# omerbt/Splice

Measured on AMD Instinct MI355X. Metric: opt_steps_per_sec, higher is better.
Workload: dtype bf16

## Files before the change

include/splice_hip.h:

```cpp
#ifndef SPLICE_HIP_H
#define SPLICE_HIP_H
#include <stddef.h>
#include <stdint.h>

#ifdef __cplusplus
extern "C" {
#endif

typedef uint16_t splice_bf16;
typedef void* splice_stream_t;

#define SPLICE_OK 0
#define SPLICE_ERR_ARG -1
#define SPLICE_ERR_HIP -2
#define SPLICE_ERR_STATE -3
#define SPLICE_ERR_NOMEM -4

int splice_version(void);
int splice_dev_switches(void);
const char* splice_last_error(void);

typedef struct splice_gemm_epilogue {
    const float* bias;
    const float* resid;
    int ldr, resid_mod;
    float* out_f32;
    int ldo;
    splice_bf16* out_bf;
    int ldbf;
    splice_bf16* out_bf_t;
    int ldt;
    splice_bf16* out_pre;
    int ldp, pre_row_lo;
    const splice_bf16* aux;
    int ldaux;
    float* out_f32_cols;
    int ld_cols, col_lo, col_hi;
    float alpha;
    int ksplit;
    long long slab_stride;
    const splice_bf16* rd_other;
    int ld_rd, rd_rows;
    float* rowdot;
    const float* row_scale;
    const float* col_scale;
    uint8_t* out_f8;
    int ld8;
    uint8_t* out_f8_t;
    int ldt8;
} splice_gemm_epilogue;

enum {
    SPLICE_EPI_BIAS = 1, SPLICE_EPI_RESID = 2, SPLICE_EPI_OUT_F32 = 4, SPLICE_EPI_OUT_BF = 8,
    SPLICE_EPI_OUT_T = 16, SPLICE_EPI_GELU = 32, SPLICE_EPI_GELU_GRAD = 64,
    SPLICE_EPI_COLS_F32 = 128, SPLICE_EPI_ALPHA = 256, SPLICE_EPI_ROWDOT = 512, SPLICE_EPI_SCALE_RC = 1024, SPLICE_EPI_OUT_F8 = 2048,
    SPLICE_EPI_OUT_F8T = 4096
};

int splice_gemm_nt_bf16(unsigned flags, const splice_bf16* A, int lda, const splice_bf16* B, int ldb,
                        int M, int N, int K, const splice_gemm_epilogue* epi, splice_stream_t stream);

int splice_gemm_nt_fp8(unsigned flags, const uint8_t* A, int lda, const uint8_t* B, int ldb, int M, int N, int K,
                       const splice_gemm_epilogue* epi, splice_stream_t stream);
int splice_quantize_rows_fp8(const float* x, int ldx, uint8_t* q, int ldq, float* scale, int rows, int cols, splice_stream_t stream);
int splice_gemm_splitk_slabs(int M, int ksplit);
int splice_gemm_force_tile(int tile);
int splice_attention_variant(int variant);
int splice_attention_qfold(int on);
int splice_attention_bwd_variant(int variant);

int splice_layernorm_fwd(const float* x, const float* gamma, const float* beta, splice_bf16* y,
                         float* mean, float* rstd, int rows, int D, float eps, splice_stream_t stream);
int splice_layernorm_bwd(const float* dy, const float* x, const float* gamma, const float* mean,
                         const float* rstd, const float* g_in, float* g_out, splice_bf16* g_out_bf,
                         int rows, int D, splice_stream_t stream);

int splice_attention_fwd(const splice_bf16* qkv, const splice_bf16* qkvT, int ldt, int B, int T, int Tld,
                         int D, int H, float scale, splice_bf16* out, float* lse, splice_stream_t stream);
int splice_attention_fwd_fp8(const uint8_t* qkv8, const uint8_t* qkvT8, int ldt8, int B, int T, int Tld, int D, int H, float scale,
                             splice_bf16* out, float* lse, splice_stream_t stream);
int splice_attention_bwd(const splice_bf16* qkv, const splice_bf16* qkvT, int ldt, int B, int T, int Tld,
                         int D, int H, float scale, const splice_bf16* out, const float* lse,
                         const splice_bf16* dout, const splice_bf16* doutT, float* delta,
                         splice_bf16* dqkv, splice_stream_t stream);
int splice_attention_probs(const splice_bf16* qkv, int B, int T, int Tld, int D, int H, float scale,
                           const float* lse, float* probs, splice_stream_t stream);

int splice_augment_structure(const float* img, float* out, float* scratch, int H, int W, int flip, int n_ops, const int* order,
                             const float* factors, float blur_sigma, splice_stream_t stream);

size_t splice_keys_selfsim_ws_bytes(int T, int D);
int splice_keys_selfsim_fwd(const float* K, int ldk, int T, int D, float eps, float* S, void* ws,
                            splice_stream_t stream);
int splice_keys_selfsim_bwd(const float* dS, const float* S, int T, int D, float eps, float* dK, int lddk,
                            int accumulate, void* ws, splice_stream_t stream);

int splice_mse(const float* a, int lda, const float* b, int ldb, int rows, int cols, float weight,
               float* loss_accum, float* grad, int ldg, splice_stream_t stream);

int splice_patchify(const float* img, splice_bf16* patches, int B, int H, int W, int p, int Tld,
                    int normalize, splice_stream_t stream);
int splice_unpatchify(const float* dpatches, float* dimg, int B, int H, int W, int p, int Tld,
                      int normalize, splice_stream_t stream);
int splice_cast_f32_bf16(const float* x, splice_bf16* y, size_t n, splice_stream_t stream);
int splice_cast_bf16_f32(const splice_bf16* x, float* y, size_t n, splice_stream_t stream);
int splice_transpose_f32_bf16(const float* x, splice_bf16* y, int rows, int cols, int ldy, splice_stream_t stream);
int splice_resize_bilinear_fwd(const float* in, float* out, int planes, int h, int w, int oh, int ow, splice_stream_t stream);
int splice_resize_bilinear_bwd(const float* dout, float* din, int planes, int h, int w, int oh, int ow, splice_stream_t stream);

int splice_vit_create(int patch, int dim, int depth, int heads, void** out_handle);
void splice_vit_destroy(void* vit);
int splice_vit_set_param(void* vit, const char* name, const float* data, long long numel, splice_stream_t stream);
float splice_vit_qscale(void* vit);
int splice_vit_params_complete(void* vit);
int splice_vit_enable_fp8(void* vit, splice_stream_t stream);
int splice_vit_ctx_create(void* vit, int B, int H, int W, const float* pos_TD, int need_grad,
                          splice_stream_t stream, void** out_ctx);
void splice_vit_ctx_destroy(void* ctx);
int splice_vit_ctx_info(void* ctx, int* T, int* Tld, int* rows);
int splice_vit_ctx_set_top_cls_only(void* ctx, int on);
int splice_vit_ctx_set_fp8(void* ctx, int mode);
int splice_vit_forward(void* ctx, const float* img, int normalize, splice_stream_t stream);
int splice_vit_forward_ex(void* ctx, const float* img, int normalize, int grad_pass_begin, splice_stream_t stream);
int splice_vit_forward_passes(void* ctx, const float* img, int normalize, int grad_pass_begin, int pass_begin, int pass_end,
                              splice_stream_t stream);
int splice_vit_get_tensor(void* ctx, int kind, int layer, void** out_ptr);
int splice_vit_read_tensor(void* ctx, int kind, int layer, void* dst, size_t bytes, splice_stream_t stream);
int splice_vit_backward(void* ctx, int pass_begin, int pass_end, const float* const* d_block,
                        const float* const* d_qkv, const float* const* d_keys, float* d_img,
                        int normalize, splice_stream_t stream);

int splice_gen_create(void** out_handle);
#define SPLICE_GEN_MAX_SCALES 6
typedef struct splice_gen_arch {
    int n_scales, in_channels, out_channels;
    int down[SPLICE_GEN_MAX_SCALES], up[SPLICE_GEN_MAX_SCALES], skip[SPLICE_GEN_MAX_SCALES];
    int filter_down[SPLICE_GEN_MAX_SCALES], filter_up[SPLICE_GEN_MAX_SCALES];
    int filter_skip;
    int reflect;
} splice_gen_arch;
int splice_gen_create_arch(const splice_gen_arch* arch, void** out_handle);
void splice_gen_destroy(void* gen);
long long splice_gen_param_count(void* gen);
int splice_gen_num_tensors(void* gen);
int splice_gen_tensor_info(void* gen, int i, const char** name, long long* offset, long long* numel);
int splice_gen_plan_create(void* gen, int N, int H, int W, int need_grad, void** out_plan);
void splice_gen_plan_destroy(void* plan);
int splice_gen_forward(void* plan, const float* params, const float* x, float* y, splice_stream_t stream);
int splice_gen_forward_borrowed(void* plan, const float* params, const float* x, float* y, splice_stream_t stream);
int splice_gen_backward(void* plan, const float* params, const float* dy, float* grads, int accumulate,
                        splice_stream_t stream);
long long splice_gen_buffer_count(void* gen);
int splice_gen_num_buffers(void* gen);
int splice_gen_buffer_info(void* gen, int i, const char** name, long long* offset, long long* numel);
int splice_gen_running_stats_update(void* const* plans, int n_plans, float* running, long long running_stride, float momentum,
                                    splice_stream_t stream);
int splice_adam_step(float* params, float* grads, float* m, float* v, long long n, float lr, float beta1,
                     float beta2, float eps, int step, int zero_grad, splice_stream_t stream);
int splice_optim_step(int kind, float* params, float* grads, float* m, float* v, long long n, float lr, float hp0, float hp1,
                      float eps, int step, int zero_grad, splice_stream_t stream);
int splice_optim_step_ex(int kind, float* params, float* grads, const float* g2, float* m, float* v, long long n, float lr,
                         const float* lr_dev, float hp0, float hp1, float eps, int step, int zero_grad, splice_stream_t stream);
int splice_optim_step_pairs(int kind, float* params, float* grads, const float* g2, float* m, float* v, int n_pairs, long long stride,
                            long long n, const float* lr_dev, float hp0, float hp1, float eps, int step, int zero_grad,
                            splice_stream_t stream);
int splice_optim_step_ema(int kind, float* params, float* grads, const float* g2, float* m, float* v, float* ema, long long n, float lr,
                          const float* lr_dev, float hp0, float hp1, float eps, int step, int zero_grad, float ema_decay, int ema_start,
                          splice_stream_t stream);

typedef struct splice_optim_ext {
    float weight_decay;
    float momentum;
    float dampening;
    int nesterov;
    int decoupled;
    int amsgrad;
    int centered;
} splice_optim_ext;
int splice_optim_step_ext(int kind, float* params, float* grads, const float* g2, float* m, float* v, float* w, long long n, float lr,
                          const float* lr_dev, float hp0, float hp1, float eps, int step, int zero_grad, const splice_optim_ext* options,
                          splice_stream_t stream);

int splice_prof_begin(int which);
int splice_prof_end(float* total_ms, int* launches);
int splice_prof_end_ex(float* total_ms, int* calls, int* kernels);
int splice_prof_end_detail(float* total_ms, int* calls, int* kernels, char* detail, int detail_len);
int splice_prof_active(void);
int splice_vit_ctx_dims(void* ctx, int* B, int* H, int* W, int* D, int* depth, int* heads, int* patch);
int splice_gen_plan_dims(void* plan, int* N, int* H, int* W, long long* nparams);
int splice_gen_plan_set_arena_stride(void* plan, long long stride);
int splice_gen_plan_set_batch_stats(void* plan, int on);
int splice_gen_plan_set_groups(void* plan, int images_per_group);
int splice_gen_plan_resize(void* plan, int H, int W);

typedef struct splice_step_config {
    int crop_h, crop_w;
    int vit_h, vit_w;
    int ent_h, ent_w;
    int ent_vit_h, ent_vit_w;
    float lambda_global_cls, lambda_global_ssim, lambda_global_identity, lambda_entire_cls, lambda_entire_ssim;
    int entire_every, cls_warmup;
    float lr, beta1, beta2, eps;
    int pairs;
    long long arena_stride;
    int fp8_selfsim;
    int top_cls_only;
    int n_crops;
    int n_crops_b;
} splice_step_config;
#define SPLICE_STEP_MAX_PAIR_CFGS 32
#define SPLICE_STEP_MAX_GROUP_IMAGES 32
int splice_step_create(const splice_step_config* cfg, void* vit_ctx_global, void* vit_ctx_entire, void* gen_plan_a, void* gen_plan_b,
                       void* gen_plan_entire, void** out_handle);
void splice_step_destroy(void* step);
int splice_step_run(void* step, float* params, float* grads, float* m, float* v, const float* A_crop, const float* B_crop,
                    const float* A_entire, int step_idx, float* losses_out, splice_stream_t stream);
int splice_step_output(void* step, int which, float** out_ptr);
int splice_step_graph_stats(void* step, long long* out);
int splice_step_use_graph(void* step, int on);
int splice_step_use_overlap(void* step, int on);
int splice_step_set_crops(void* step, int a_h, int a_w, int b_h, int b_w);
int splice_step_set_mode(void* step, int skip_adam, int accumulate);
int splice_step_set_optimizer(void* step, int kind, float hp0, float hp1, float eps);
int splice_step_set_lr(void* step, float lr);
int splice_step_set_pair_weights(void* step, const float* lambdas);
int splice_step_set_pair_lr(void* step, const float* lr);
int splice_step_set_phases(void* step, int phases, void* leader);
int splice_step_set_running_stats(void* step, float* running, long long stride);

typedef struct splice_stop_state {
    float sum;
    int count;
    int windows;
    float best;
    int bad;
    int stop_step;
} splice_stop_state;
int splice_step_set_stop_rule(void* step, int window, float rel, int patience, int min_steps);
int splice_step_stop_state(void* step, splice_stop_state* out, splice_stream_t stream);
int splice_step_restore(void* step, int next_step_idx, const splice_stop_state* stop, splice_stream_t stream);
int splice_step_set_input_rows(void* step, int pairs_in, const int* rows);
int splice_plateau_update(splice_stop_state* state, const float* losses8, int pairs, int window, float rel, int patience, int min_steps,
                          int step_idx, int counted, splice_stream_t stream);

int splice_step_set_ema(void* step, float* ema, float decay, int start);
int splice_optim_step_pairs_ema(int kind, float* params, float* grads, const float* g2, float* m, float* v, float* ema, int n_pairs,
                                long long stride, long long n, const float* lr_dev, float hp0, float hp1, float eps, const int* step_dev,
                                const splice_stop_state* stop, int zero_grad, float ema_decay, int ema_start, splice_stream_t stream);

#define SPLICE_CLIP_CHUNK 4096
typedef struct splice_clip_state {
    float sumsq;
    float norm;
    float coef;
    int skip;
    int clipped;
    int skipped;
} splice_clip_state;
int splice_grad_norm_pairs(const float* grads, const float* g2, int n_pairs, long long stride, long long n, float max_norm, float* partials,
                           splice_clip_state* state, const splice_stop_state* stop, const int* step_dev, splice_stream_t stream);
int splice_optim_step_pairs_clip(int kind, float* params, float* grads, const float* g2, float* m, float* v, float* ema, int n_pairs,
                                 long long stride, long long n, const float* lr_dev, float hp0, float hp1, float eps, const int* step_dev,
                                 const splice_stop_state* stop, int zero_grad, float ema_decay, int ema_start, const splice_clip_state* clip,
                                 splice_stream_t stream);
int splice_optim_step_clip(int kind, float* params, float* grads, const float* g2, float* m, float* v, float* ema, long long n, float lr,
                           const float* lr_dev, float hp0, float hp1, float eps, int step, int zero_grad, float ema_decay, int ema_start,
                           const splice_clip_state* clip, splice_stream_t stream);
int splice_step_set_grad_clip(void* step, float max_norm, splice_clip_state* state);

typedef struct splice_clip_auto_state {
    float ref[2];
    int count[2];
    float thr;
    int regime;
} splice_clip_auto_state;
int splice_grad_norm_pairs_auto(const float* grads, const float* g2, int n_pairs, long long stride, long long n, float max_norm, float k,
                                float beta, int warmup, int regime, float* partials, splice_clip_state* state,
                                splice_clip_auto_state* auto_state, const splice_stop_state* stop, const int* step_dev,
                                splice_stream_t stream);
int splice_step_set_grad_clip_auto(void* step, float max_norm, float k, float beta, int warmup, splice_clip_state* state,
                                   splice_clip_auto_state* auto_state);

#define SPLICE_STOP_HISTORY 64
typedef struct splice_best_state {
    int best_step;
    int best_window;
} splice_best_state;
int splice_plateau_update_best(splice_stop_state* state, splice_best_state* best, float* means, const float* losses8, int pairs, int window,
                               float rel, int patience, int min_steps, int step_idx, int counted, splice_stream_t stream);
int splice_optim_step_pairs_best(int kind, float* params, float* grads, const float* g2, float* m, float* v, float* ema, int n_pairs,
                                 long long stride, long long n, const float* lr_dev, float hp0, float hp1, float eps, const int* step_dev,
                                 const splice_stop_state* stop, int zero_grad, float ema_decay, int ema_start, const splice_clip_state* clip,
                                 const splice_best_state* best, float* best_params, float* best_ema, splice_stream_t stream);
int splice_optim_step_pairs_ext(int kind, float* params, float* grads, const float* g2, float* m, float* v, float* w, float* ema, int n_pairs,
                                long long stride, long long n, const float* lr_dev, float hp0, float hp1, float eps, int step,
                                const int* step_dev, const splice_stop_state* stop, int zero_grad, float ema_decay, int ema_start,
                                const splice_clip_state* clip, const splice_best_state* best, float* best_params, float* best_ema,
                                const splice_optim_ext* options, splice_stream_t stream);
int splice_step_set_optimizer_ext(void* step, const splice_optim_ext* options, float* w);
int splice_step_set_keep_best(void* step, float* best_params, float* best_ema, splice_best_state* state, float* means);

int splice_step_set_loss_trace(void* step, float* trace, int capacity);

typedef struct splice_lr_state {
    float scale;
    int bad;
    int cuts;
    int last_cut_step;
} splice_lr_state;
int splice_step_set_lr_plateau(void* step, float factor, int patience, float min_scale, splice_lr_state* state, int* cut_steps);
int splice_plateau_update_lr(splice_stop_state* state, splice_lr_state* lr_state, int* cut_steps, const float* losses8, const float* lr_in,
                             int per_pair, float* lr_eff, int pairs, int window, float rel, int patience, int min_steps, float factor,
                             int lr_patience, float min_scale, int step_idx, int counted, splice_stream_t stream);

size_t splice_selfsim_loss_pairs_ws_bytes(int T, int D, int pairs);
int splice_selfsim_loss_pairs(const splice_bf16* k_tgt, const splice_bf16* k_x, int ldk, size_t k_pstride, const splice_bf16* kT_x, int ldt,
                              size_t kT_pstride, int T, int D, int pairs, float lambda, const float* e_scale_tab, int fp8, float eps,
                              float* loss_part, size_t part_pstride, float* dk, int lddk, size_t dk_pstride, void* ws, splice_stream_t stream);
int splice_mse_pairs(const float* a, int lda, size_t a_ps, const float* b, int ldb, size_t b_ps, int rows, int cols, float loss_weight,
                     float grad_weight, float* part, size_t part_ps, float* grad, int ldg, size_t g_ps, int pairs, const float* grad_tab,
                     splice_stream_t stream);
int splice_total_loss_pairs(float* lbase, size_t lstride, int lp, float w_ssim, float w_essim, float w_ecls, float w_cls, float w_id,
                            float* out8, int pairs, int n_a, int n_b, int n_c, int n_e, const float* wtab, int ssim_on, int entire,
                            splice_stream_t stream);
int splice_step_set_image_terms(void* step, float lambda_tv, float lambda_pix);
#define SPLICE_IMAGE_TERMS_CHUNK 4096
int splice_image_terms_value(const float* x, int n_x, int xh, int xw, const float* y, const float* b, int n_y, int yh, int yw, float* lbase,
                             size_t lstride, int lp, splice_stream_t stream);
int splice_image_terms_grad_add(const float* x, const float* b, float* d, int n_img, int h, int w, float lambda, splice_stream_t stream);
int splice_total_loss_pairs_img(float* lbase, size_t lstride, int lp, float w_ssim, float w_essim, float w_ecls, float w_cls, float w_id,
                                float* out8, int pairs, int n_a, int n_b, int n_c, int n_e, const float* wtab, int ssim_on, int entire,
                                float w_tv, float w_pix, splice_stream_t stream);
int splice_total_loss_pairs_trace(float* lbase, size_t lstride, int lp, float w_ssim, float w_essim, float w_ecls, float w_cls, float w_id,
                                  float* out8, int pairs, int n_a, int n_b, int n_c, int n_e, const float* wtab, int ssim_on, int entire,
                                  splice_stop_state* stop, int window, float rel, int patience, int min_steps, const int* dev_t,
                                  float* trace, int capacity, splice_stream_t stream);

int splice_attn_cls_fwd(const splice_bf16* qkv, const splice_bf16* qkvT, int ldt, int B, int T, int Tld, int D, int H, float scale, splice_bf16* out,
                        float* probs, splice_stream_t stream);
int splice_attn_cls_bwd(const splice_bf16* qkv, const splice_bf16* qkvT, int ldt, int B, int T, int Tld, int D, int H, float scale, const float* probs,
                        const float* dout_slabs, int n_slabs, size_t slab_stride, splice_bf16* dqkv, splice_stream_t stream);
int splice_ln_rows_fwd(float* x, size_t xs, const float* gamma, const float* beta, splice_bf16* y, size_t ys, float* mean, float* rstd, size_t ss,
                       int rows, int D, float eps, const float* slabs, int n_slabs, size_t slab_stride, const float* bias, const float* resid, size_t rs,
                       splice_stream_t stream);
int splice_ln_rows_bwd(float* dy, size_t dys, const float* x, size_t xs, const float* gamma, const float* mean, const float* rstd, size_t ss, float* g,
                       splice_bf16* g_bf, int rows, int D, int n_slabs, size_t slab_stride, splice_stream_t stream);
int splice_rows_finish(int mode, const float* slabs, int n_slabs, size_t slab_stride, int rows, int N, const float* bias, const float* resid, size_t rs,
                       float* out_f32, size_t os, splice_bf16* out_bf, splice_bf16* pre_bf, const splice_bf16* aux, size_t ps, int pre_lo,
                       splice_stream_t stream);

typedef struct splice_gen_conv_args {
    const float* in;
    const float* w;
    const float* bias;
    float* out;
    size_t in_nstride, in_cstride, out_nstride, out_cstride, w_jstride, w_cstride, p_nstride;
    int N, Cin, Hi, Wi, Cout, Ho, Wo, ks, stride, pad;
    int reflect, act, transposed, accumulate;
    float* ws;
    size_t ws_floats;
    int p_group, defer_reduce;
} splice_gen_conv_args;
#define SPLICE_GEN_CONV_FORM_INTS 5
int splice_gen_conv(const splice_gen_conv_args* args, int* form_out, splice_stream_t stream);
int splice_gen_conv_pair(const splice_gen_conv_args* a, const splice_gen_conv_args* b, int* forms_out, splice_stream_t stream);
int splice_gen_conv_reflect_dgrad(const splice_gen_conv_args* args, float* pad_scratch, size_t scratch_floats, splice_stream_t stream);

typedef struct splice_gen_wgrad_args {
    const float* x;
    const float* dy;
    float* ws;
    size_t ws_floats;
// ... 71 lines not shown
```

splice_amd/_lib.py:

```python
import ctypes as C
import os

_HERE = os.path.dirname(os.path.abspath(__file__))
LIB_PATH = os.path.join(_HERE, "libsplice_hip.so")

_lib = None


class GemmEpilogue(C.Structure):
    _fields_ = [
        ("bias", C.c_void_p), ("resid", C.c_void_p), ("ldr", C.c_int), ("resid_mod", C.c_int),
        ("out_f32", C.c_void_p), ("ldo", C.c_int),
        ("out_bf", C.c_void_p), ("ldbf", C.c_int),
        ("out_bf_t", C.c_void_p), ("ldt", C.c_int),
        ("out_pre", C.c_void_p), ("ldp", C.c_int), ("pre_row_lo", C.c_int),
        ("aux", C.c_void_p), ("ldaux", C.c_int),
        ("out_f32_cols", C.c_void_p), ("ld_cols", C.c_int), ("col_lo", C.c_int), ("col_hi", C.c_int),
        ("alpha", C.c_float), ("ksplit", C.c_int), ("slab_stride", C.c_longlong),
        ("rd_other", C.c_void_p), ("ld_rd", C.c_int), ("rd_rows", C.c_int), ("rowdot", C.c_void_p),
        ("row_scale", C.c_void_p), ("col_scale", C.c_void_p),
        ("out_f8", C.c_void_p), ("ld8", C.c_int),
        ("out_f8_t", C.c_void_p), ("ldt8", C.c_int),
    ]


class GenArch(C.Structure):
    _fields_ = [("n_scales", C.c_int), ("in_channels", C.c_int), ("out_channels", C.c_int),
                ("down", C.c_int * 6), ("up", C.c_int * 6), ("skip", C.c_int * 6),
                ("filter_down", C.c_int * 6), ("filter_up", C.c_int * 6), ("filter_skip", C.c_int), ("reflect", C.c_int)]


class StepConfig(C.Structure):
    _fields_ = [
        ("crop_h", C.c_int), ("crop_w", C.c_int), ("vit_h", C.c_int), ("vit_w", C.c_int),
        ("ent_h", C.c_int), ("ent_w", C.c_int), ("ent_vit_h", C.c_int), ("ent_vit_w", C.c_int),
        ("lambda_global_cls", C.c_float), ("lambda_global_ssim", C.c_float), ("lambda_global_identity", C.c_float),
        ("lambda_entire_cls", C.c_float), ("lambda_entire_ssim", C.c_float),
        ("entire_every", C.c_int), ("cls_warmup", C.c_int),
        ("lr", C.c_float), ("beta1", C.c_float), ("beta2", C.c_float), ("eps", C.c_float),
        ("pairs", C.c_int), ("arena_stride", C.c_longlong), ("fp8_selfsim", C.c_int), ("top_cls_only", C.c_int), ("n_crops", C.c_int), ("n_crops_b", C.c_int),
    ]


class StopState(C.Structure):
    _fields_ = [("sum", C.c_float), ("count", C.c_int), ("windows", C.c_int), ("best", C.c_float), ("bad", C.c_int), ("stop_step", C.c_int)]


class ClipState(C.Structure):
    _fields_ = [("sumsq", C.c_float), ("norm", C.c_float), ("coef", C.c_float), ("skip", C.c_int), ("clipped", C.c_int), ("skipped", C.c_int)]


class ClipAutoState(C.Structure):
    _fields_ = [("ref", C.c_float * 2), ("count", C.c_int * 2), ("thr", C.c_float), ("regime", C.c_int)]


class BestState(C.Structure):
    _fields_ = [("best_step", C.c_int), ("best_window", C.c_int)]


class LrState(C.Structure):
    _fields_ = [("scale", C.c_float), ("bad", C.c_int), ("cuts", C.c_int), ("last_cut_step", C.c_int)]


class OptimExt(C.Structure):
    _fields_ = [("weight_decay", C.c_float), ("momentum", C.c_float), ("dampening", C.c_float), ("nesterov", C.c_int), ("decoupled", C.c_int),
                ("amsgrad", C.c_int), ("centered", C.c_int)]


def optim_ext(options):
    if isinstance(options, OptimExt):
        return options
    return OptimExt(float(options.get("weight_decay", 0.0)), float(options.get("momentum", 0.0)), float(options.get("dampening", 0.0)),
                    int(bool(options.get("nesterov", False))), int(bool(options.get("decoupled", False))), int(bool(options.get("amsgrad", False))),
                    int(bool(options.get("centered", False))))


class GenConvArgs(C.Structure):
    _fields_ = [("in", C.c_void_p), ("w", C.c_void_p), ("bias", C.c_void_p), ("out", C.c_void_p)] + \
               [(n, C.c_size_t) for n in ("in_nstride", "in_cstride", "out_nstride", "out_cstride", "w_jstride", "w_cstride", "p_nstride")] + \
               [(n, C.c_int) for n in ("N", "Cin", "Hi", "Wi", "Cout", "Ho", "Wo", "ks", "stride", "pad", "reflect", "act", "transposed", "accumulate")] + \
               [("ws", C.c_void_p), ("ws_floats", C.c_size_t), ("p_group", C.c_int), ("defer_reduce", C.c_int)]


class GenWgradArgs(C.Structure):
    _fields_ = [("x", C.c_void_p), ("dy", C.c_void_p), ("ws", C.c_void_p), ("ws_floats", C.c_size_t)] + \
               [(n, C.c_size_t) for n in ("x_nstride", "x_cstride", "dy_nstride", "dy_cstride")] + \
               [(n, C.c_int) for n in ("N", "Cin", "Hi", "Wi", "Cout", "Ho", "Wo", "ks", "stride", "pad", "reflect")]


class GenBnArgs(C.Structure):
    _fields_ = [("y", C.c_void_p), ("out", C.c_void_p), ("y_nstride", C.c_size_t), ("out_nstride", C.c_size_t),
                ("N", C.c_int), ("C", C.c_int), ("HW", C.c_int), ("batch", C.c_int),
                ("gamma", C.c_void_p), ("beta", C.c_void_p), ("eps", C.c_float), ("slope", C.c_float), ("p_nstride", C.c_size_t),
                ("part", C.c_void_p), ("part_floats", C.c_size_t), ("mean", C.c_void_p), ("rstd", C.c_void_p),
                ("up_src", C.c_void_p), ("up_d_src", C.c_void_p), ("up_src_ns", C.c_size_t), ("up_d_src_ns", C.c_size_t),
                ("up_c0", C.c_int), ("up_h", C.c_int), ("up_w", C.c_int), ("up_Ho", C.c_int), ("up_Wo", C.c_int),
                ("slabs", C.c_void_p), ("bias", C.c_void_p), ("ksplit", C.c_int),
                ("da", C.c_void_p), ("dy", C.c_void_p), ("da_nstride", C.c_size_t), ("dy_nstride", C.c_size_t),
                ("dgamma", C.c_void_p), ("dbeta", C.c_void_p), ("accumulate", C.c_int),
                ("da_slabs", C.c_void_p), ("da_ksplit", C.c_int), ("da_accumulate", C.c_int),
                ("pre_y", C.c_void_p), ("pre_y_ns", C.c_size_t), ("pre_slabs", C.c_void_p), ("pre_bias", C.c_void_p),
                ("pre_ksplit", C.c_int), ("pre_C", C.c_int), ("pre_gamma", C.c_void_p), ("pre_beta", C.c_void_p),
                ("pre_mean", C.c_void_p), ("pre_rstd", C.c_void_p), ("pre_slope", C.c_float),
                ("pre_dy", C.c_void_p), ("pre_dgamma", C.c_void_p), ("pre_dbeta", C.c_void_p)]


GEN_CONV_FORM_INTS, GEN_WGRAD_FORM_INTS, GEN_BN_FORM_INTS = 5, 6, 7

STOP_HISTORY = 64

EPI_BIAS, EPI_RESID, EPI_OUT_F32, EPI_OUT_BF, EPI_OUT_T = 1, 2, 4, 8, 16
EPI_GELU, EPI_GELU_GRAD, EPI_COLS_F32, EPI_ALPHA, EPI_ROWDOT, EPI_SCALE_RC, EPI_OUT_F8, EPI_OUT_F8T = 32, 64, 128, 256, 512, 1024, 2048, 4096

_vp, _i, _f, _sz, _u = C.c_void_p, C.c_int, C.c_float, C.c_size_t, C.c_uint

_SIGNATURES = {
    "splice_version": ([], C.c_int),
    "splice_dev_switches": ([], C.c_int),
    "splice_last_error": ([], C.c_char_p),
    "splice_gemm_nt_bf16": ([_u, _vp, _i, _vp, _i, _i, _i, _i, C.POINTER(GemmEpilogue), _vp], _i),
    "splice_gemm_nt_fp8": ([_u, _vp, _i, _vp, _i, _i, _i, _i, C.POINTER(GemmEpilogue), _vp], _i),
    "splice_quantize_rows_fp8": ([_vp, _i, _vp, _i, _vp, _i, _i, _vp], _i),
    "splice_gemm_splitk_slabs": ([_i, _i], _i),
    "splice_gemm_force_tile": ([_i], _i),
    "splice_attention_variant": ([_i], _i),
    "splice_attention_qfold": ([_i], _i),
    "splice_attention_bwd_variant": ([_i], _i),
    "splice_layernorm_fwd": ([_vp, _vp, _vp, _vp, _vp, _vp, _i, _i, _f, _vp], _i),
    "splice_layernorm_bwd": ([_vp, _vp, _vp, _vp, _vp, _vp, _vp, _vp, _i, _i, _vp], _i),
    "splice_attention_fwd": ([_vp, _vp, _i, _i, _i, _i, _i, _i, _f, _vp, _vp, _vp], _i),
    "splice_attention_fwd_fp8": ([_vp, _vp, _i, _i, _i, _i, _i, _i, _f, _vp, _vp, _vp], _i),
    "splice_attention_bwd": ([_vp, _vp, _i, _i, _i, _i, _i, _i, _f, _vp, _vp, _vp, _vp, _vp, _vp, _vp], _i),
    "splice_attention_probs": ([_vp, _i, _i, _i, _i, _i, _f, _vp, _vp, _vp], _i),
    "splice_augment_structure": ([_vp, _vp, _vp, _i, _i, _i, _i, C.POINTER(C.c_int), C.POINTER(C.c_float), _f, _vp], _i),
    "splice_keys_selfsim_ws_bytes": ([_i, _i], _sz),
    "splice_keys_selfsim_fwd": ([_vp, _i, _i, _i, _f, _vp, _vp, _vp], _i),
    "splice_keys_selfsim_bwd": ([_vp, _vp, _i, _i, _f, _vp, _i, _i, _vp, _vp], _i),
    "splice_mse": ([_vp, _i, _vp, _i, _i, _i, _f, _vp, _vp, _i, _vp], _i),
    "splice_selfsim_loss_pairs_ws_bytes": ([_i, _i, _i], _sz),
    "splice_selfsim_loss_pairs": ([_vp, _vp, _i, _sz, _vp, _i, _sz, _i, _i, _i, _f, _vp, _i, _f, _vp, _sz, _vp, _i, _sz, _vp, _vp], _i),
    "splice_mse_pairs": ([_vp, _i, _sz, _vp, _i, _sz, _i, _i, _f, _f, _vp, _sz, _vp, _i, _sz, _i, _vp, _vp], _i),
    "splice_total_loss_pairs": ([_vp, _sz, _i, _f, _f, _f, _f, _f, _vp, _i, _i, _i, _i, _i, _vp, _i, _i, _vp], _i),
    "splice_attn_cls_fwd": ([_vp, _vp, _i, _i, _i, _i, _i, _i, _f, _vp, _vp, _vp], _i),
    "splice_attn_cls_bwd": ([_vp, _vp, _i, _i, _i, _i, _i, _i, _f, _vp, _vp, _i, _sz, _vp, _vp], _i),
    "splice_ln_rows_fwd": ([_vp, _sz, _vp, _vp, _vp, _sz, _vp, _vp, _sz, _i, _i, _f, _vp, _i, _sz, _vp, _vp, _sz, _vp], _i),
    "splice_ln_rows_bwd": ([_vp, _sz, _vp, _sz, _vp, _vp, _vp, _sz, _vp, _vp, _i, _i, _i, _sz, _vp], _i),
    "splice_rows_finish": ([_i, _vp, _i, _sz, _i, _i, _vp, _vp, _sz, _vp, _sz, _vp, _vp, _vp, _sz, _i, _vp], _i),
    "splice_gen_conv": ([C.POINTER(GenConvArgs), C.POINTER(_i), _vp], _i),
    "splice_gen_conv_pair": ([C.POINTER(GenConvArgs), C.POINTER(GenConvArgs), C.POINTER(_i), _vp], _i),
    "splice_gen_conv_reflect_dgrad": ([C.POINTER(GenConvArgs), _vp, _sz, _vp], _i),
    "splice_gen_conv_wgrad_ws_floats": ([_i, _i, _i, _i, _i, _i], _sz),
    "splice_gen_conv_wgrad": ([C.POINTER(GenWgradArgs), _vp, _i, _i, _sz, C.POINTER(_i), _vp], _i),
    "splice_gen_wgrad_reduce": ([_vp, _i, _i, _vp, _i, _i, _sz, _vp], _i),
    "splice_gen_bn_small_instance": ([_i], _i),
    "splice_gen_bn_form": ([_i, _i, _sz, _i, C.POINTER(_i)], _i),
    "splice_gen_bn_part_floats": ([_i, _i], _sz),
    "splice_gen_bn_fwd": ([C.POINTER(GenBnArgs), _vp], _i),
    "splice_gen_bn_bwd": ([C.POINTER(GenBnArgs), _vp], _i),
    "splice_gen_upsample2x_fwd": ([_vp, _sz, _vp, _sz, _i, _i, _i, _i, _i, _i, _vp], _i),
    "splice_gen_upsample2x_bwd": ([_vp, _sz, _vp, _sz, _i, _i, _i, _i, _i, _i, _vp], _i),
    "splice_gen_sigmoid_bias_part_floats": ([_i, _i], _sz),
    "splice_gen_sigmoid_bwd_bias": ([_vp, _vp, _vp, _i, _i, _i, _vp, _sz, _sz, _i, C.POINTER(_i), _vp], _i),
    "splice_patchify": ([_vp, _vp, _i, _i, _i, _i, _i, _i, _vp], _i),
    "splice_unpatchify": ([_vp, _vp, _i, _i, _i, _i, _i, _i, _vp], _i),
    "splice_cast_f32_bf16": ([_vp, _vp, _sz, _vp], _i),
    "splice_cast_bf16_f32": ([_vp, _vp, _sz, _vp], _i),
    "splice_transpose_f32_bf16": ([_vp, _vp, _i, _i, _i, _vp], _i),
    "splice_resize_bilinear_fwd": ([_vp, _vp, _i, _i, _i, _i, _i, _vp], _i),
    "splice_resize_bilinear_bwd": ([_vp, _vp, _i, _i, _i, _i, _i, _vp], _i),
    "splice_vit_create": ([_i, _i, _i, _i, C.POINTER(_vp)], _i),
    "splice_vit_destroy": ([_vp], None),
    "splice_vit_set_param": ([_vp, C.c_char_p, _vp, C.c_longlong, _vp], _i),
    "splice_vit_params_complete": ([_vp], _i),
    "splice_vit_enable_fp8": ([_vp, _vp], _i),
    "splice_vit_ctx_create": ([_vp, _i, _i, _i, _vp, _i, _vp, C.POINTER(_vp)], _i),
    "splice_vit_ctx_destroy": ([_vp], None),
    "splice_vit_ctx_info": ([_vp, C.POINTER(_i), C.POINTER(_i), C.POINTER(_i)], _i),
    "splice_vit_ctx_set_top_cls_only": ([_vp, _i], _i),
    "splice_vit_ctx_set_fp8": ([_vp, _i], _i),
    "splice_vit_forward": ([_vp, _vp, _i, _vp], _i),
    "splice_vit_forward_ex": ([_vp, _vp, _i, _i, _vp], _i),
    "splice_vit_forward_passes": ([_vp, _vp, _i, _i, _i, _i, _vp], _i),
    "splice_vit_get_tensor": ([_vp, _i, _i, C.POINTER(_vp)], _i),
    "splice_vit_qscale": ([_vp], C.c_float),
    "splice_vit_read_tensor": ([_vp, _i, _i, _vp, _sz, _vp], _i),
    "splice_vit_backward": ([_vp, _i, _i, C.POINTER(_vp), C.POINTER(_vp), C.POINTER(_vp), _vp, _i, _vp], _i),
    "splice_gen_create": ([C.POINTER(_vp)], _i),
    "splice_gen_create_arch": ([C.POINTER(GenArch), C.POINTER(_vp)], _i),
    "splice_gen_destroy": ([_vp], None),
    "splice_gen_param_count": ([_vp], C.c_longlong),
    "splice_gen_num_tensors": ([_vp], _i),
    "splice_gen_tensor_info": ([_vp, _i, C.POINTER(C.c_char_p), C.POINTER(C.c_longlong), C.POINTER(C.c_longlong)], _i),
    "splice_gen_plan_create": ([_vp, _i, _i, _i, _i, C.POINTER(_vp)], _i),
    "splice_gen_plan_destroy": ([_vp], None),
    "splice_gen_forward": ([_vp, _vp, _vp, _vp, _vp], _i),
    "splice_gen_forward_borrowed": ([_vp, _vp, _vp, _vp, _vp], _i),
    "splice_gen_backward": ([_vp, _vp, _vp, _vp, _i, _vp], _i),
    "splice_adam_step": ([_vp, _vp, _vp, _vp, C.c_longlong, _f, _f, _f, _f, _i, _i, _vp], _i),
    "splice_optim_step": ([_i, _vp, _vp, _vp, _vp, C.c_longlong, _f, _f, _f, _f, _i, _i, _vp], _i),
    "splice_optim_step_ex": ([_i, _vp, _vp, _vp, _vp, _vp, C.c_longlong, _f, _vp, _f, _f, _f, _i, _i, _vp], _i),
    "splice_optim_step_pairs": ([_i, _vp, _vp, _vp, _vp, _vp, _i, C.c_longlong, C.c_longlong, _vp, _f, _f, _f, _i, _i, _vp], _i),
    "splice_optim_step_ema": ([_i, _vp, _vp, _vp, _vp, _vp, _vp, C.c_longlong, _f, _vp, _f, _f, _f, _i, _i, _f, _i, _vp], _i),
    "splice_optim_step_pairs_ema": ([_i, _vp, _vp, _vp, _vp, _vp, _vp, _i, C.c_longlong, C.c_longlong, _vp, _f, _f, _f, _vp, _vp, _i, _f, _i, _vp], _i),
    "splice_step_set_ema": ([_vp, _vp, _f, _i], _i),
    "splice_grad_norm_pairs": ([_vp, _vp, _i, C.c_longlong, C.c_longlong, _f, _vp, _vp, _vp, _vp, _vp], _i),
    "splice_optim_step_pairs_clip": ([_i, _vp, _vp, _vp, _vp, _vp, _vp, _i, C.c_longlong, C.c_longlong, _vp, _f, _f, _f, _vp, _vp, _i, _f, _i, _vp, _vp], _i),
    "splice_optim_step_clip": ([_i, _vp, _vp, _vp, _vp, _vp, _vp, C.c_longlong, _f, _vp, _f, _f, _f, _i, _i, _f, _i, _vp, _vp], _i),
    "splice_step_set_grad_clip": ([_vp, _f, _vp], _i),
    "splice_grad_norm_pairs_auto": ([_vp, _vp, _i, C.c_longlong, C.c_longlong, _f, _f, _f, _i, _i, _vp, _vp, _vp, _vp, _vp, _vp], _i),
    "splice_step_set_grad_clip_auto": ([_vp, _f, _f, _f, _i, _vp, _vp], _i),
    "splice_plateau_update_best": ([_vp, _vp, _vp, _vp, _i, _i, _f, _i, _i, _i, _i, _vp], _i),
    "splice_optim_step_pairs_best": ([_i, _vp, _vp, _vp, _vp, _vp, _vp, _i, C.c_longlong, C.c_longlong, _vp, _f, _f, _f, _vp, _vp, _i, _f, _i, _vp, _vp, _vp, _vp, _vp], _i),
    "splice_step_set_keep_best": ([_vp, _vp, _vp, _vp, _vp], _i),
    "splice_step_set_loss_trace": ([_vp, _vp, _i], _i),
    "splice_total_loss_pairs_trace": ([_vp, _sz, _i, _f, _f, _f, _f, _f, _vp, _i, _i, _i, _i, _i, _vp, _i, _i, _vp, _i, _f, _i, _i, _vp, _vp, _i, _vp], _i),
    "splice_step_set_lr_plateau": ([_vp, _f, _i, _f, _vp, _vp], _i),
    "splice_plateau_update_lr": ([_vp, _vp, _vp, _vp, _vp, _i, _vp, _i, _i, _f, _i, _i, _f, _i, _f, _i, _i, _vp], _i),
    "splice_optim_step_ext": ([_i, _vp, _vp, _vp, _vp, _vp, _vp, C.c_longlong, _f, _vp, _f, _f, _f, _i, _i, C.POINTER(OptimExt), _vp], _i),
    "splice_optim_step_pairs_ext": ([_i, _vp, _vp, _vp, _vp, _vp, _vp, _vp, _i, C.c_longlong, C.c_longlong, _vp, _f, _f, _f, _i, _vp, _vp, _i, _f, _i, _vp, _vp,
                                     _vp, _vp, C.POINTER(OptimExt), _vp], _i),
    "splice_step_set_optimizer_ext": ([_vp, C.POINTER(OptimExt), _vp], _i),
    "splice_step_set_image_terms": ([_vp, _f, _f], _i),
    "splice_image_terms_value": ([_vp, _i, _i, _i, _vp, _vp, _i, _i, _i, _vp, _sz, _i, _vp], _i),
    "splice_image_terms_grad_add": ([_vp, _vp, _vp, _i, _i, _i, _f, _vp], _i),
    "splice_total_loss_pairs_img": ([_vp, _sz, _i, _f, _f, _f, _f, _f, _vp, _i, _i, _i, _i, _i, _vp, _i, _i, _f, _f, _vp], _i),
    "splice_prof_begin": ([_i], _i),
    "splice_prof_end": ([C.POINTER(_f), C.POINTER(_i)], _i),
    "splice_prof_end_ex": ([C.POINTER(_f), C.POINTER(_i), C.POINTER(_i)], _i),
    "splice_prof_end_detail": ([C.POINTER(_f), C.POINTER(_i), C.POINTER(_i), C.c_char_p, _i], _i),
    "splice_prof_active": ([], _i),
    "splice_step_use_graph": ([_vp, _i], _i),
    "splice_step_graph_stats": ([_vp, C.POINTER(C.c_longlong)], _i),
    "splice_step_use_overlap": ([_vp, _i], _i),
    "splice_vit_ctx_dims": ([_vp] + [C.POINTER(_i)] * 7, _i),
    "splice_gen_plan_dims": ([_vp, C.POINTER(_i), C.POINTER(_i), C.POINTER(_i), C.POINTER(C.c_longlong)], _i),
    "splice_step_create": ([C.POINTER(StepConfig), _vp, _vp, _vp, _vp, _vp, C.POINTER(_vp)], _i),
    "splice_step_destroy": ([_vp], None),
    "splice_step_run": ([_vp, _vp, _vp, _vp, _vp, _vp, _vp, _vp, _i, _vp, _vp], _i),
    "splice_step_output": ([_vp, _i, C.POINTER(_vp)], _i),
    "splice_step_set_crops": ([_vp, _i, _i, _i, _i], _i),
    "splice_step_set_running_stats": ([_vp, _vp, C.c_longlong], _i),
    "splice_step_set_mode": ([_vp, _i, _i], _i),
    "splice_step_set_optimizer": ([_vp, _i, _f, _f, _f], _i),
    "splice_step_set_lr": ([_vp, _f], _i),
    "splice_step_set_pair_weights": ([_vp, _vp], _i),
    "splice_step_set_pair_lr": ([_vp, _vp], _i),
    "splice_step_set_phases": ([_vp, _i, _vp], _i),
    "splice_step_set_stop_rule": ([_vp, _i, _f, _i, _i], _i),
    "splice_step_stop_state": ([_vp, _vp, _vp], _i),
    "splice_plateau_update": ([_vp, _vp, _i, _i, _f, _i, _i, _i, _i, _vp], _i),
    "splice_step_restore": ([_vp, _i, _vp, _vp], _i),
    "splice_step_set_input_rows": ([_vp, _i, _vp], _i),
    "splice_gen_buffer_count": ([_vp], C.c_longlong),
    "splice_gen_num_buffers": ([_vp], _i),
    "splice_gen_buffer_info": ([_vp, _i, C.POINTER(C.c_char_p), C.POINTER(C.c_longlong), C.POINTER(C.c_longlong)], _i),
    "splice_gen_running_stats_update": ([C.POINTER(_vp), _i, _vp, C.c_longlong, _f, _vp], _i),
    "splice_gen_plan_resize": ([_vp, _i, _i], _i),
    "splice_gen_plan_set_arena_stride": ([_vp, C.c_longlong], _i),
    "splice_gen_plan_set_batch_stats": ([_vp, _i], _i),
    "splice_gen_plan_set_groups": ([_vp, _i], _i),
}


def exported_symbols():
    return sorted(_SIGNATURES)


def register(name, argtypes, restype):
    _SIGNATURES[name] = (argtypes, restype)


def lib():
    global _lib
    if _lib is None:
        if not os.path.exists(LIB_PATH):
            raise RuntimeError(
                f"{LIB_PATH} not found: the HIP extension is not built "
                "(run __graft_entry__.build() or `make -C splice_amd/csrc`). There is no CPU fallback.")
        _lib = C.CDLL(LIB_PATH)
        for name, (argtypes, restype) in _SIGNATURES.items():
            fn = getattr(_lib, name)
            fn.argtypes = argtypes
            fn.restype = restype
    return _lib


def check(rc, what=""):
    if rc != 0:
        msg = lib().splice_last_error().decode(errors="replace")
        raise RuntimeError(f"libsplice_hip {what} failed (rc={rc}): {msg}")


def ptr(t):
    return None if t is None else C.c_void_p(t.data_ptr())


def current_stream():
    import torch
    return C.c_void_p(torch.cuda.current_stream().cuda_stream)
```

splice_amd/csrc/attention.hip:

```cpp
#include "kernels.h"
#include <cstdlib>


#define NEG_BIG (-1.0e30f)
#define LOG2E 1.4426950408889634f
#define LN2 0.6931471805599453f

__device__ __forceinline__ u32x4 ld16v(const bf16_t* p) { return *reinterpret_cast<const u32x4*>(p); }
__device__ __forceinline__ u32x4 pack8v(const f32x4& a, const f32x4& b) {
    return u32x4{pack2bf(a[0], a[1]), pack2bf(a[2], a[3]), pack2bf(b[0], b[1]), pack2bf(b[2], b[3])};
}
__device__ __forceinline__ void st4bf(bf16_t* p, const f32x4& v, float s) {
    *reinterpret_cast<uint2*>(p) = uint2{pack2bf(v[0] * s, v[1] * s), pack2bf(v[2] * s, v[3] * s)};
}
__device__ __forceinline__ float group4_max(float v) {
    v = fmaxf(v, __shfl_xor(v, 16, 64));
    return fmaxf(v, __shfl_xor(v, 32, 64));
}
__device__ __forceinline__ float group4_sum(float v) {
    v += __shfl_xor(v, 16, 64);
    return v + __shfl_xor(v, 32, 64);
}

typedef __attribute__((address_space(3))) void lds_void;
// ... 320 lines not shown
        }
        __syncthreads();
        if (grp == 1) return;
#pragma unroll
        for (int qb = 0; qb < QB; ++qb) {
            const float* e = ex + ((dma.wave * QB + qb) * 18) * 64 + lane;
            const float m1 = e[0], l1 = e[64];
            const float mn = fmaxf(m[qb], m1);
            const float a0 = __builtin_amdgcn_exp2f(m[qb] - mn), a1 = __builtin_amdgcn_exp2f(m1 - mn);
            m[qb] = mn;
            l[qb] = merge2(l[qb], a0, l1, a1);
#pragma unroll
            for (int nd = 0; nd < 4; ++nd)
#pragma unroll
                for (int r = 0; r < 4; ++r) o[qb][nd][r] = merge2(o[qb][nd][r], a0, e[(2 + nd * 4 + r) * 64], a1);
        }
    }
    if (!active) return;
#pragma unroll
    for (int qb = 0; qb < QB; ++qb) {
        const float lt = group4_sum(l[qb]);
        const int q = qidx[qb];
        if (q < a.Tld) {
            const float inv = 1.0f / lt;
            bf16_t* op = a.out + ((size_t)b * a.Tld + q) * a.D + h * 64 + g * 4;
#pragma unroll
            for (int nd = 0; nd < 4; ++nd) st4bf(op + nd * 16, o[qb][nd], inv);
            if (g == 0) a.lse[((size_t)b * a.H + h) * a.Tld + q] = m[qb] + __builtin_amdgcn_logf(lt);
        }
    }
}

template <int NSUB, bool MASK>
__device__ __forceinline__ void attn_bwd_q_tile(const bf16_t* Ks, const bf16_t* Vs, const FragAddr& fa,
                                                const u32x4 (&qf)[2], const u32x4 (&dof)[2], float lse_q, float del_q, f32x4 (&dq)[4],
                                                float c2, int kt, int T, int g) {
    f32x4 s[NSUB * 2], dp[NSUB * 2];
#pragma unroll
    for (int nb = 0; nb < NSUB * 2; ++nb) {
        const int off = (nb >> 1) * 2048 + (nb & 1) * 256;
        s[nb] = mfma16(lds16(Ks + fa.tok[0] + off), qf[0], f32x4{0.f, 0.f, 0.f, 0.f});
        dp[nb] = mfma16(lds16(Vs + fa.tok[0] + off), dof[0], f32x4{0.f, 0.f, 0.f, 0.f});
        s[nb] = mfma16(lds16(Ks + fa.tok[1] + off), qf[1], s[nb]);
        dp[nb] = mfma16(lds16(Vs + fa.tok[1] + off), dof[1], dp[nb]);
    }
#pragma unroll
    for (int nb = 0; nb < NSUB * 2; ++nb)
#pragma unroll
        for (int r = 0; r < 4; ++r) {
            float p = __builtin_amdgcn_exp2f(__builtin_fmaf(s[nb][r], c2, -lse_q));
            if (MASK) p = kt + (nb >> 1) * 32 + g * 8 + (nb & 1) * 4 + r < T ? p : 0.f;
            dp[nb][r] = p * (dp[nb][r] - del_q);
        }
#pragma unroll
    for (int sub = 0; sub < NSUB; ++sub) {
        const u32x4 dsb = pack8v(dp[sub * 2], dp[sub * 2 + 1]);
#pragma unroll
        for (int nd = 0; nd < 4; ++nd) dq[nd] = mfma16(lds_tr16(Ks, fa.tr[nd] + sub * 2048), dsb, dq[nd]);
    }
}

__device__ __forceinline__ float dot8bf(const u32x4& x, const u32x4& y) {
    float acc = 0.f;
#pragma unroll
    for (int j = 0; j < 4; ++j) {
        acc = __builtin_fmaf(__uint_as_float(x[j] << 16), __uint_as_float(y[j] << 16), acc);
        acc = __builtin_fmaf(__uint_as_float(x[j] & 0xFFFF0000u), __uint_as_float(y[j] & 0xFFFF0000u), acc);
    }
    return acc;
}

constexpr int Q_STAGE = 2 * 4096;
template <int NW = 4>
__device__ __forceinline__ void attn_bwd_q_body(const AttnArgs& a, int xb, int h, int b, bf16_t* smem ) {
    const int lane = threadIdx.x & 63;
    const int g = lane >> 4, c = lane & 15;
    const int ld = 3 * a.D;
    const TileDmaT<NW> dma;
    const FragAddr fa(g, c);
    const int qbase = xb * (16 * NW) + dma.wave * 16;
    const bool active = qbase < a.Tld;
    const int q = qbase + c;
    const int qc = q < a.Tld ? q : a.Tld - 1;
    const bf16_t* qkv_b = a.qkv + (size_t)b * a.Tld * ld;
    u32x4 qf[2], dof[2];
    {
        const bf16_t* pq = qkv_b + (size_t)qc * ld + h * 64 + g * 8;
        const bf16_t* pd = a.dout + ((size_t)b * a.Tld + qc) * a.D + h * 64 + g * 8;
        qf[0] = ld16v(pq); qf[1] = ld16v(pq + 32);
        dof[0] = ld16v(pd); dof[1] = ld16v(pd + 32);
    }
    const float lse_q = a.lse[((size_t)b * a.H + h) * a.Tld + qc];
    const float del_q = a.delta[((size_t)b * a.H + h) * a.Tld + qc];
    const bf16_t* krow = qkv_b + a.D + h * 64;
    const bf16_t* vrow = qkv_b + 2 * a.D + h * 64;
    const uint32_t koff = dma.token_off(ld);
    auto issue = [&](int kt, bf16_t* st) {
        if (kt + 64 <= a.Tld) {
            dma.fast_tile(krow + (size_t)kt * ld, koff, ld, st);
            dma.fast_tile(vrow + (size_t)kt * ld, koff, ld, st + 4096);
        } else {
            dma.token_tile(krow, ld, kt, a.Tld - 1, st);
            dma.token_tile(vrow, ld, kt, a.Tld - 1, st + 4096);
        }
    };
    issue(0, smem);
    f32x4 dq[4];
#pragma unroll
    for (int nd = 0; nd < 4; ++nd) dq[nd] = f32x4{0.f, 0.f, 0.f, 0.f};
    const float c2 = a.scale * LOG2E;
    const int nfull = a.T / 64;
    for (int it = 0; it < nfull; ++it) {
        dma_wait_barrier();
        const int kn = it * 64 + 64;
        if (kn < a.Tld) issue(kn, smem + ((it + 1) & 1) * Q_STAGE);
        if (active) {
            const bf16_t* cur = smem + (it & 1) * Q_STAGE;
            attn_bwd_q_tile<2, false>(cur, cur + 4096, fa, qf, dof, lse_q, del_q, dq, c2, it * 64, a.T, g);
        }
    }
    if (nfull * 64 < a.T) {
        dma_wait_barrier();
        const int kt = nfull * 64;
        if (active) {
            const bf16_t* cur = smem + (nfull & 1) * Q_STAGE;
            if (kt + 32 < a.T) attn_bwd_q_tile<2, true>(cur, cur + 4096, fa, qf, dof, lse_q, del_q, dq, c2, kt, a.T, g);
            else attn_bwd_q_tile<1, true>(cur, cur + 4096, fa, qf, dof, lse_q, del_q, dq, c2, kt, a.T, g);
        }
    }
    if (active && q < a.Tld) {
        bf16_t* p = a.dqkv + ((size_t)b * a.Tld + q) * ld + h * 64 + g * 4;
#pragma unroll
        for (int nd = 0; nd < 4; ++nd) st4bf(p + nd * 16, dq[nd], a.scale);
    }
}

#define KV_STAGE (2 * 4096 + 256)
template <int NSUB>
__device__ __forceinline__ void attn_bwd_kv_tile(const bf16_t* st, const FragAddr& fa, const u32x4 (&kf)[2], const u32x4 (&vf)[2],
                                                 f32x4 (&dk)[4], f32x4 (&dv)[4], float c2, int g) {
    const bf16_t *Qs = st, *Ds = st + 4096;
    const float* Ls = reinterpret_cast<const float*>(st + 8192);
    const float* Es = Ls + 64;
    f32x4 s[NSUB * 2], dp[NSUB * 2];
#pragma unroll
    for (int nb = 0; nb < NSUB * 2; ++nb) {
        const int off = (nb >> 1) * 2048 + (nb & 1) * 256;
        s[nb] = mfma16(lds16(Qs + fa.tok[0] + off), kf[0], f32x4{0.f, 0.f, 0.f, 0.f});
        dp[nb] = mfma16(lds16(Ds + fa.tok[0] + off), vf[0], f32x4{0.f, 0.f, 0.f, 0.f});
        s[nb] = mfma16(lds16(Qs + fa.tok[1] + off), kf[1], s[nb]);
        dp[nb] = mfma16(lds16(Ds + fa.tok[1] + off), vf[1], dp[nb]);
    }
#pragma unroll
    for (int nb = 0; nb < NSUB * 2; ++nb) {
        const f32x4 ls = *reinterpret_cast<const f32x4*>(Ls + (nb >> 1) * 32 + g * 8 + (nb & 1) * 4);
        const f32x4 de = *reinterpret_cast<const f32x4*>(Es + (nb >> 1) * 32 + g * 8 + (nb & 1) * 4);
#pragma unroll
        for (int r = 0; r < 4; ++r) {
            const float p = __builtin_amdgcn_exp2f(__builtin_fmaf(s[nb][r], c2, -ls[r]));
            s[nb][r] = p;
            dp[nb][r] = p * (dp[nb][r] - de[r]);
        }
    }
#pragma unroll
    for (int sub = 0; sub < NSUB; ++sub) {
        const u32x4 pb = pack8v(s[sub * 2], s[sub * 2 + 1]), dsb = pack8v(dp[sub * 2], dp[sub * 2 + 1]);
#pragma unroll
        for (int nd = 0; nd < 4; ++nd) {
            dv[nd] = mfma16(lds_tr16(Ds, fa.tr[nd] + sub * 2048), pb, dv[nd]);
            dk[nd] = mfma16(lds_tr16(Qs, fa.tr[nd] + sub * 2048), dsb, dk[nd]);
        }
    }
}

template <int NW = 4>
__device__ __forceinline__ void attn_bwd_kv_body(const AttnArgs& a, int xb, int h, int b, bf16_t* smem ) {
    const int lane = threadIdx.x & 63;
    const int g = lane >> 4, c = lane & 15;
    const int ld = 3 * a.D;
    const TileDmaT<NW> dma;
    const FragAddr fa(g, c);
    const int kbase = xb * (16 * NW) + dma.wave * 16;
    const bool active = kbase < a.Tld;
    const int key = kbase + c;
    const int keyc = key < a.Tld ? key : a.Tld - 1;
    const bf16_t* qkv_b = a.qkv + (size_t)b * a.Tld * ld;
    u32x4 kf[2], vf[2];
    {
        const bf16_t* pk = qkv_b + (size_t)keyc * ld + a.D + h * 64 + g * 8;
        const bf16_t* pv = qkv_b + (size_t)keyc * ld + 2 * a.D + h * 64 + g * 8;
        kf[0] = ld16v(pk); kf[1] = ld16v(pk + 32);
        vf[0] = ld16v(pv); vf[1] = ld16v(pv + 32);
    }
    const bf16_t* qrow = qkv_b + h * 64;
    const bf16_t* dorow = a.dout + (size_t)b * a.Tld * a.D + h * 64;
    const float* lse = a.lse + ((size_t)b * a.H + h) * a.Tld;
    const float* dl = a.delta + ((size_t)b * a.H + h) * a.Tld;
    const uint32_t qoff = dma.token_off(ld), dooff = dma.token_off(a.D);
    auto issue = [&](int qt, bf16_t* st) {
        if (qt + 64 <= a.Tld) {
            dma.fast_tile(qrow + (size_t)qt * ld, qoff, ld, st);
            dma.fast_tile(dorow + (size_t)qt * a.D, dooff, a.D, st + 4096);
        } else {
            dma.token_tile(qrow, ld, qt, a.Tld - 1, st);
            dma.token_tile(dorow, a.D, qt, a.Tld - 1, st + 4096);
        }
        if (dma.wave < 2) {
            const int qq = qt + lane < a.Tld ? qt + lane : a.Tld - 1;
            const float* src = (dma.wave == 0 ? lse : dl) + qq;
            __builtin_amdgcn_global_load_lds((glb_void*)src, (lds_void*)(st + 8192 + dma.wave * 128), 4, 0, 0);
        }
    };
    issue(0, smem);
    f32x4 dk[4], dv[4];
#pragma unroll
    for (int nd = 0; nd < 4; ++nd) { dk[nd] = f32x4{0.f, 0.f, 0.f, 0.f}; dv[nd] = f32x4{0.f, 0.f, 0.f, 0.f}; }
    const float c2 = a.scale * LOG2E;
    const int nfull = a.Tld / 64;
    for (int it = 0; it < nfull; ++it) {
        dma_wait_barrier();
        const int qn = it * 64 + 64;
        if (qn < a.Tld) issue(qn, smem + ((it + 1) & 1) * KV_STAGE);
        if (active) attn_bwd_kv_tile<2>(smem + (it & 1) * KV_STAGE, fa, kf, vf, dk, dv, c2, g);
    }
    if (nfull * 64 < a.Tld) {
        dma_wait_barrier();
        if (active) attn_bwd_kv_tile<1>(smem + (nfull & 1) * KV_STAGE, fa, kf, vf, dk, dv, c2, g);
    }
    if (active && key < a.Tld) {
        const float sk = key < a.T ? a.scale : 0.f, sv = key < a.T ? 1.0f : 0.f;
        bf16_t* pk = a.dqkv + ((size_t)b * a.Tld + key) * ld + a.D + h * 64 + g * 4;
        bf16_t* pv = a.dqkv + ((size_t)b * a.Tld + key) * ld + 2 * a.D + h * 64 + g * 4;
#pragma unroll
        for (int nd = 0; nd < 4; ++nd) {
            st4bf(pk + nd * 16, dk[nd], sk);
            st4bf(pv + nd * 16, dv[nd], sv);
        }
    }
}

__global__ __launch_bounds__(256) void attn_bwd_kernel(AttnArgs a, int nx) {
    __shared__ __attribute__((aligned(16))) bf16_t smem[2 * KV_STAGE];
    const int n = nx * a.H * a.B;
    const int lid = xcd_remap(blockIdx.x, 2 * n);
    const int pair = lid >> 1;
    const int xb = pair % nx, bh = pair / nx;
    const int h = bh % a.H, b = bh / a.H;
    if (lid & 1) attn_bwd_kv_body(a, xb, h, b, smem);
    else attn_bwd_q_body(a, xb, h, b, smem);
}

template <int NW>
__global__ __launch_bounds__(64 * NW) void attn_bwd_q_kernel(AttnArgs a, int nx) {
    __shared__ __attribute__((aligned(16))) bf16_t smem[2 * Q_STAGE];
    int xb, h, b;
    attn_block_coords(nx, a.H, a.B, xb, h, b);
    attn_bwd_q_body<NW>(a, xb, h, b, smem);
}
template <int NW>
__global__ __launch_bounds__(64 * NW) void attn_bwd_kv_kernel(AttnArgs a, int nx) {
    __shared__ __attribute__((aligned(16))) bf16_t smem[2 * KV_STAGE];
    int xb, h, b;
    attn_block_coords(nx, a.H, a.B, xb, h, b);
    attn_bwd_kv_body<NW>(a, xb, h, b, smem);
}

__global__ void attn_delta_kernel(AttnArgs a) {
    const int idx = blockIdx.x * blockDim.x + threadIdx.x;
    if (idx >= a.B * a.Tld * a.H) return;
    const int h = idx % a.H, row = idx / a.H;
    const int b = row / a.Tld, q = row % a.Tld;
    const bf16_t* po = a.out + (size_t)row * a.D + h * 64;
    const bf16_t* pd = a.dout + (size_t)row * a.D + h * 64;
    float acc = 0.f;
#pragma unroll
    for (int i = 0; i < 8; ++i) acc += dot8bf(ld16v(po + i * 8), ld16v(pd + i * 8));
    a.delta[((size_t)b * a.H + h) * a.Tld + q] = acc;
}

__global__ void attn_probs_kernel(AttnArgs a, float* probs) {
    const int q = blockIdx.x, h = blockIdx.y, b = blockIdx.z;
    const int ld = 3 * a.D;
    const bf16_t* qkv_b = a.qkv + (size_t)b * a.Tld * ld;
    const bf16_t* pq = qkv_b + (size_t)q * ld + h * 64;
    const float lse = a.lse[((size_t)b * a.H + h) * a.Tld + q];
    float qv[64];
#pragma unroll
    for (int d = 0; d < 64; ++d) qv[d] = bf2f(pq[d]);
    float* out = probs + (((size_t)b * a.H + h) * a.T + q) * a.T;
    for (int key = threadIdx.x; key < a.T; key += blockDim.x) {
        const bf16_t* pk = qkv_b + (size_t)key * ld + a.D + h * 64;
        float s = 0.f;
#pragma unroll
        for (int d = 0; d < 64; ++d) s += qv[d] * bf2f(pk[d]);
        out[key] = __builtin_amdgcn_exp2f(s * a.scale * LOG2E - lse);
    }
}

static int g_attn_variant = 0;
void attn_set_variant(int v) { g_attn_variant = v; }
static int g_attn_qfold = 0;
void attn_set_qfold(int on) { g_attn_qfold = on; }
int attn_qfold_hook() { return g_attn_qfold; }

struct AttrOnce {
    bool done[64] = {};
    void set(const void* fn, int bytes) {
        int dev = 0;
        (void)hipGetDevice(&dev);
        if (dev < 0 || dev >= 64) { (void)hipFuncSetAttribute(fn, hipFuncAttributeMaxDynamicSharedMemorySize, bytes); return; }
        if (!done[dev]) { (void)hipFuncSetAttribute(fn, hipFuncAttributeMaxDynamicSharedMemorySize, bytes); done[dev] = true; }
    }
};

template <int NW, bool FOLD>
static void attn_fwd_x32_go(const AttnArgs* a, hipStream_t s) {
    static AttrOnce attr;
    attr.set((const void*)attn_fwd_x32_kernel<NW, FOLD>, X32<NW>::LDS_BYTES);
    const int nx = cdiv(a->Tld, 32 * NW);
    SPLICE_LAUNCH((attn_fwd_x32_kernel<NW, FOLD>), dim3(nx * a->H * a->B), dim3(64 * NW), X32<NW>::LDS_BYTES, s, *a, nx);
}

int attn_fwd_launch(const AttnArgs* a, hipStream_t s) {
    if (a->Tld % 32 || a->D % 64 || a->D / 64 != a->H) return SPLICE_ERR_ARG;
    if (!a->qkv8) {
        const int nwv = g_attn_variant / 10 == 4 ? g_attn_variant % 10 : 4;
        if (a->qfold) { if (nwv == 2) attn_fwd_x32_go<2, true>(a, s); else if (nwv == 8) attn_fwd_x32_go<8, true>(a, s); else attn_fwd_x32_go<4, true>(a, s); }
        else { if (nwv == 2) attn_fwd_x32_go<2, false>(a, s); else if (nwv == 8) attn_fwd_x32_go<8, false>(a, s); else attn_fwd_x32_go<4, false>(a, s); }
        return SPLICE_OK;
    }
    if (!a->qkvT8 || a->ldt8 % 16 || a->D % 16) return SPLICE_ERR_ARG;
    const long tasks = (long)a->B * a->H * cdiv(a->Tld, 16);
    const int qb = g_attn_variant ? g_attn_variant % 10 : (tasks > 60000 ? 2 : 1);
    const long wgs = (long)cdiv(a->Tld, 64 * qb) * a->H * a->B;
    const int ks = g_attn_variant ? (g_attn_variant / 10 == 1 ? 2 : 1) : ((wgs > 512 && a->T <= 2048) ? 1 : 2);
    const int nx = cdiv(a->Tld, 64 * qb);
    const dim3 grid(nx * a->H * a->B);
    if (ks == 2) {
        if (qb == 2) SPLICE_LAUNCH((attn_fwd8_kernel<2, 2>), grid, dim3(512), 0, s, *a, nx);
        else SPLICE_LAUNCH((attn_fwd8_kernel<1, 2>), grid, dim3(512), 0, s, *a, nx);
    } else {
        if (qb == 2) SPLICE_LAUNCH((attn_fwd8_kernel<2, 1>), grid, dim3(256), 0, s, *a, nx);
        else SPLICE_LAUNCH((attn_fwd8_kernel<1, 1>), grid, dim3(256), 0, s, *a, nx);
    }
    return SPLICE_OK;
}

static int g_attn_bwd_variant = 0;
void attn_set_bwd_variant(int v) { g_attn_bwd_variant = v; }
static const int kAttnBwdMergeMaxX32 = 1400;
static const int kAttnBwdMergeMax16 = 768;

int attn_bwd_launch(const AttnArgs* a, hipStream_t s) {
    if (a->Tld % 32 || a->D % 64 || a->D / 64 != a->H) return SPLICE_ERR_ARG;
    const int nx = cdiv(a->Tld, 64);
    if (!a->delta_ready) SPLICE_LAUNCH(attn_delta_kernel, dim3(cdiv(a->B * a->Tld * a->H, 256)), dim3(256), 0, s, *a);
    if (a->qfold && g_attn_bwd_variant != 1) {
        static AttrOnce at_m, at_q, at_kv, at_m2;
        at_m.set((const void*)attn_bwd_x32_kernel<4>, BX_KV_LDS);
        at_q.set((const void*)attn_bwd_q_x32_kernel<4>, BX_Q_LDS);
        at_kv.set((const void*)attn_bwd_kv_x32_kernel<4>, BX_KV_LDS);
        if (g_attn_bwd_variant == 4) {
            at_m2.set((const void*)attn_bwd_x32_kernel<2>, BX_KV_LDS);
            const int nx2 = cdiv(a->Tld, 64), n2 = nx2 * a->H * a->B;
            SPLICE_LAUNCH((attn_bwd_x32_kernel<2>), dim3(2 * n2), dim3(128), BX_KV_LDS, s, *a, nx2);
            return SPLICE_OK;
        }
        const int nx4 = cdiv(a->Tld, 128), n4 = nx4 * a->H * a->B;
        if (g_attn_bwd_variant == 3 || (g_attn_bwd_variant != 2 && 2 * n4 > kAttnBwdMergeMaxX32)) {
            SPLICE_LAUNCH((attn_bwd_q_x32_kernel<4>), dim3(n4), dim3(256), BX_Q_LDS, s, *a, nx4);
            SPLICE_LAUNCH((attn_bwd_kv_x32_kernel<4>), dim3(n4), dim3(256), BX_KV_LDS, s, *a, nx4);
        } else SPLICE_LAUNCH((attn_bwd_x32_kernel<4>), dim3(2 * n4), dim3(256), BX_KV_LDS, s, *a, nx4);
        return SPLICE_OK;
    }
    const int n = nx * a->H * a->B;
    if (2 * n <= kAttnBwdMergeMax16) {
        SPLICE_LAUNCH(attn_bwd_kernel, dim3(2 * n), dim3(256), 0, s, *a, nx);
    } else {
        SPLICE_LAUNCH(attn_bwd_q_kernel<4>, dim3(n), dim3(256), 0, s, *a, nx);
        SPLICE_LAUNCH(attn_bwd_kv_kernel<4>, dim3(n), dim3(256), 0, s, *a, nx);
    }
    return SPLICE_OK;
}

int attn_probs_launch(const AttnArgs* a, float* probs, hipStream_t s) {
    dim3 grid(a->T, a->H, a->B);
    SPLICE_LAUNCH(attn_probs_kernel, grid, dim3(128), 0, s, *a, probs);
    return SPLICE_OK;
}
```

splice_amd/csrc/attn_bwd_x32.h:

```cpp
#pragma once

constexpr int BX_SLOTS = 4;
constexpr int BX_Q_LDS = BX_SLOTS * 2 * 8192;
constexpr int BX_KV_LDS = BX_SLOTS * (2 * 8192 + 512);

__device__ __forceinline__ int bx_swz(int row) { return (((row >> 1) & 1) << 2) | (((row >> 3) & 1) << 1) | ((row >> 2) & 1); }

struct BxFrag {
    int rowa[4];
    int tra[2][2];
    __device__ __forceinline__ BxFrag(int lane) {
        const int q32 = lane & 31, hi = lane >> 5;
#pragma unroll
        for (int ks = 0; ks < 4; ++ks) rowa[ks] = q32 * 64 + (((2 * ks + hi) ^ bx_swz(q32)) << 3);
        const int m = lane & 15, dg = (lane >> 4) & 1;
#pragma unroll
        for (int db = 0; db < 2; ++db)
#pragma unroll
            for (int sec = 0; sec < 2; ++sec) {
                const int row = 8 * sec + 4 * hi + (m >> 2);
                tra[db][sec] = row * 64 + (((4 * db + 2 * dg + ((m >> 1) & 1)) ^ bx_swz(row)) << 3) + (m & 1) * 4;
            }
    }
};
__device__ __forceinline__ u32x4 bx_tr(const bf16_t* tile, const BxFrag& f, int db, int off) {
    typedef __attribute__((address_space(3))) tr_v4s lds_v4s;
    const tr_v4s lo = __builtin_amdgcn_ds_read_tr16_b64_v4i16((lds_v4s*)(tile + f.tra[db][0] + off));
    const tr_v4s hh = __builtin_amdgcn_ds_read_tr16_b64_v4i16((lds_v4s*)(tile + f.tra[db][1] + off));
    const uint2 x = __builtin_bit_cast(uint2, lo), y = __builtin_bit_cast(uint2, hh);
    return u32x4{x.x, x.y, y.x, y.y};
}
__device__ __forceinline__ void bx_mfma_seed(f32x16_t& d, const u32x4& a, const u32x4& b, const f32x16_t& c) {
    asm volatile("v_mfma_f32_32x32x16_bf16 %0, %1, %2, %3" : "=&v"(d) : "v"(a), "v"(b), "v"(c));
}
#define BX_SB __builtin_amdgcn_sched_barrier(0)

template <int NW>
struct BxDma {
    static constexpr int PIECES = 8 / NW;
    int wave, lr, chunk;
    uint32_t off[PIECES];
    __device__ __forceinline__ BxDma(int lane, int wave_, int ld, int coldelta) : wave(wave_) {
        lr = lane >> 3;
        const int pos = lane & 7;
        chunk = pos ^ ((((lr >> 1) & 1) << 2) | ((wave & 1) << 1) | ((lr >> 2) & 1));
#pragma unroll
        for (int i = 0; i < PIECES; ++i) off[i] = (uint32_t)((((wave + NW * i) * 8 + lr) * ld + chunk * 8 + coldelta) * 2);
    }
    __device__ __forceinline__ void tile(const bf16_t* base, int ld, int coldelta, int row0, int rows_total, uint32_t dst) const {
        if (row0 + 64 <= rows_total) {
            const bf16_t* tb = base + (size_t)row0 * ld;
#pragma unroll
            for (int i = 0; i < PIECES; ++i) pp_dma16(dst + i * (NW * 1024), off[i], tb);
        } else {
#pragma unroll
            for (int i = 0; i < PIECES; ++i) {
                int t = row0 + (wave + NW * i) * 8 + lr;
                t = t < rows_total ? t : rows_total - 1;
                pp_dma16(dst + i * (NW * 1024), (uint32_t)((t * ld + chunk * 8 + coldelta) * 2), base);
            }
        }
    }
};

template <int NW, bool FOLD>
__device__ __forceinline__ void attn_bwd_q_x32_body(const AttnArgs& a, int xb, int h, int b, bf16_t* bx_smem ) {
    constexpr int NL = 2 * (8 / NW);
    const int lane = threadIdx.x & 63, q32 = lane & 31, hi = lane >> 5;
    const int wave = __builtin_amdgcn_readfirstlane(threadIdx.x >> 6);
    const int ld = 3 * a.D;
    const int qbase = xb * (32 * NW) + wave * 32;
    const bool active = qbase < a.Tld;
    const bf16_t* pbase = a.qkv + (size_t)b * a.Tld * ld + h * 64;
    const int nt = (a.T + 63) / 64;
    const BxDma<NW> dk_(lane, wave, ld, a.D), dv_(lane, wave, ld, 2 * a.D);
    const BxFrag fr(lane);
    const uint32_t lds0 = (uint32_t)(size_t)(__attribute__((address_space(3))) bf16_t*)bx_smem + (uint32_t)wave * 1024u;
    auto issue = [&](int tile, int slot) __attribute__((always_inline)) {
        const uint32_t dst = __builtin_amdgcn_readfirstlane(lds0 + (uint32_t)slot * 16384u);
        dk_.tile(pbase, ld, a.D, tile * 64, a.Tld, dst);
        dv_.tile(pbase, ld, 2 * a.D, tile * 64, a.Tld, dst + 8192u);
    };
    issue(0, 0);
    if (nt > 1) issue(1, 1);
    if (nt > 2) issue(2, 2);

    const int qidx = qbase + q32;
    const int qc = qidx < a.Tld ? qidx : a.Tld - 1;
    u32x4 qf[4], dof[4];
    {
        const bf16_t* pq = pbase + (size_t)qc * ld + hi * 8;
        const bf16_t* pd = a.dout + ((size_t)b * a.Tld + qc) * a.D + h * 64 + hi * 8;
#pragma unroll
        for (int ks = 0; ks < 4; ++ks) { qf[ks] = ld16v(pq + ks * 16); dof[ks] = ld16v(pd + ks * 16); }
    }
    const float lse_q = a.lse[((size_t)b * a.H + h) * a.Tld + qc];
    const float del_q = a.delta[((size_t)b * a.H + h) * a.Tld + qc];
    const float c2 = a.scale * LOG2E;
    f32x16_t negl, negd, dq[2], s[2], dp[2];
    const f32x16_t zero16 = {0.f, 0.f, 0.f, 0.f, 0.f, 0.f, 0.f, 0.f, 0.f, 0.f, 0.f, 0.f, 0.f, 0.f, 0.f, 0.f};
#pragma unroll
    for (int r = 0; r < 16; ++r) { negl[r] = -lse_q; negd[r] = -del_q; dq[0][r] = dq[1][r] = 0.f; s[0][r] = s[1][r] = dp[0][r] = dp[1][r] = 0.f; }
    u32x4 kf[4], vf[4];
    auto read_rows = [&](const bf16_t* K, int blk) __attribute__((always_inline)) {
#pragma unroll
        for (int ks = 0; ks < 4; ++ks) { kf[ks] = lds16(K + fr.rowa[ks] + blk * 2048); vf[ks] = lds16(K + 4096 + fr.rowa[ks] + blk * 2048); }
    };
    auto sdp = [&](f32x16_t& sx, f32x16_t& dx, int ks) __attribute__((always_inline)) {
        if (ks == 0) {
            if (FOLD) bx_mfma_seed(sx, kf[0], qf[0], negl); else sx = mfma32(kf[0], qf[0], zero16);
            bx_mfma_seed(dx, vf[0], dof[0], negd);
        } else { sx = mfma32(kf[ks], qf[ks], sx); dx = mfma32(vf[ks], dof[ks], dx); }
    };
    pp_wait_dma<0>();
    asm volatile("" : "+v"(qf[0]), "+v"(qf[1]), "+v"(qf[2]), "+v"(qf[3]), "+v"(dof[0]), "+v"(dof[1]), "+v"(dof[2]), "+v"(dof[3]));
    pp_barrier();
    if (active) {
        read_rows(bx_smem, 0);
#pragma unroll
        for (int ks = 0; ks < 4; ++ks) sdp(s[0], dp[0], ks);
        read_rows(bx_smem, 1);
    }
    int slot = 0;
    auto body = [&](auto TAILC, int t) __attribute__((always_inline)) {
        constexpr bool TAIL = decltype(TAILC)::value;
        const int s1 = (slot + 1) & 3, s3 = (slot + 3) & 3;
        if (!TAIL || t + 2 < nt) pp_wait_dma<NL>(); else pp_wait_dma<0>();
        asm volatile("s_waitcnt lgkmcnt(0)" ::: "memory");
        pp_barrier();
        if (!TAIL || t + 3 < nt) issue(t + 3, s3);
        if (active) {
            const bf16_t* Kt = bx_smem + slot * 8192;
            const bf16_t* Kn = bx_smem + s1 * 8192;
#pragma unroll
            for (int blk = 0; blk < 2; ++blk) {
                f32x16_t& sc = s[blk];
                f32x16_t& dc = dp[blk];
                f32x16_t& sn = s[blk ^ 1];
                f32x16_t& dn = dp[blk ^ 1];
                if (TAIL && t * 64 + 64 > a.T) {
#pragma unroll
                    for (int r = 0; r < 16; ++r) sc[r] = t * 64 + 32 * blk + 8 * (r >> 2) + 4 * hi + (r & 3) < a.T ? sc[r] : NEG_BIG;
                }
                float g[16];
                u32x4 dsb[2], ktf[2][2];
                auto va = [&](int r0, int n) __attribute__((always_inline)) {
#pragma unroll
                    for (int r = r0; r < r0 + n; ++r) {
                        const float p = FOLD ? __builtin_amdgcn_exp2f(sc[r]) : __builtin_amdgcn_exp2f(__builtin_fmaf(sc[r], c2, -lse_q));
                        g[r] = p * dc[r];
                    }
                    asm volatile("" : "+v"(g[r0]), "+v"(g[r0 + n - 1]));
                };
                auto cv = [&](int kk) __attribute__((always_inline)) {
                    const float* pp = &g[kk * 8];
                    dsb[kk] = u32x4{pack2bf(pp[0], pp[1]), pack2bf(pp[2], pp[3]), pack2bf(pp[4], pp[5]), pack2bf(pp[6], pp[7])};
                    pp_opaque(dsb[kk]);
                };
                auto rt = [&](int kk, int db) __attribute__((always_inline)) {
                    ktf[kk][db] = bx_tr(Kt, fr, db, blk * 2048 + kk * 1024);
                };
                BX_SB;
                sdp(sn, dn, 0); BX_SB; va(0, 4); rt(0, 0); BX_SB;
                sdp(sn, dn, 1); BX_SB; va(4, 4); cv(0); rt(0, 1); BX_SB;
                sdp(sn, dn, 2); BX_SB; va(8, 4); rt(1, 0); BX_SB;
                sdp(sn, dn, 3); BX_SB; va(12, 4); cv(1); rt(1, 1); BX_SB;
                const bf16_t* Kr = blk == 0 ? Kn : Kn;
#pragma unroll
                for (int kk = 0; kk < 2; ++kk)
#pragma unroll
                    for (int db = 0; db < 2; ++db) {
                        dq[db] = mfma32(ktf[kk][db], dsb[kk], dq[db]);
                        BX_SB;
                        const int ks = kk * 2 + db;
                        kf[ks] = lds16(Kr + fr.rowa[ks] + blk * 2048); vf[ks] = lds16(Kr + 4096 + fr.rowa[ks] + blk * 2048);
                        BX_SB;
                    }
            }
        }
        slot = s1;
    };
    {
        std::false_type MAIN; std::true_type TAILT;
        int t = 0;
        for (; t + 4 < nt; ++t) body(MAIN, t);
        for (; t < nt; ++t) body(TAILT, t);
    }
    if (!active || qidx >= a.Tld) return;
    bf16_t* op = a.dqkv + ((size_t)b * a.Tld + qidx) * ld + h * 64 + hi * 4;
#pragma unroll
    for (int db = 0; db < 2; ++db)
#pragma unroll
        for (int j = 0; j < 4; ++j)
            *reinterpret_cast<uint2*>(op + db * 32 + j * 8) = uint2{pack2bf(dq[db][4 * j] * a.scale, dq[db][4 * j + 1] * a.scale),
                                                                    pack2bf(dq[db][4 * j + 2] * a.scale, dq[db][4 * j + 3] * a.scale)};
}

template <int NW>
__device__ __forceinline__ void attn_bwd_kv_x32_body(const AttnArgs& a, int xb, int h, int b, bf16_t* bx_smem ) {
    constexpr int SLOT = 2 * 4096 + 256;
    static_assert(NW >= 2, "waves 0 and 1 move the lse / delta rows");
    const int lane = threadIdx.x & 63, k32 = lane & 31, hi = lane >> 5;
    const int wave = __builtin_amdgcn_readfirstlane(threadIdx.x >> 6);
    const int ld = 3 * a.D;
    const int kbase = xb * (32 * NW) + wave * 32;
    const bool active = kbase < a.Tld;
    const bf16_t* pbase = a.qkv + (size_t)b * a.Tld * ld + h * 64;
    const bf16_t* dobase = a.dout + (size_t)b * a.Tld * a.D + h * 64;
    const float* lse = a.lse + ((size_t)b * a.H + h) * a.Tld;
    const float* dl = a.delta + ((size_t)b * a.H + h) * a.Tld;
    const int nblk = a.Tld / 32, nt = (nblk + 1) / 2;
    const BxDma<NW> dq_(lane, wave, ld, 0), dd_(lane, wave, a.D, 0);
    const BxFrag fr(lane);
    const uint32_t ldsb = (uint32_t)(size_t)(__attribute__((address_space(3))) bf16_t*)bx_smem;
    const uint32_t lds0 = ldsb + (uint32_t)wave * 1024u;
    auto issue = [&](int tile, int slot) __attribute__((always_inline)) {
        const uint32_t dst = __builtin_amdgcn_readfirstlane(lds0 + (uint32_t)slot * (SLOT * 2));
        dq_.tile(pbase, ld, 0, tile * 64, a.Tld, dst);
        dd_.tile(dobase, a.D, 0, tile * 64, a.Tld, dst + 8192u);
        if (wave < 2) {
            const int r = tile * 64 + lane;
            const uint32_t voff = (uint32_t)((r < a.Tld ? r : a.Tld - 1) * 4);
            const uint32_t d2 = __builtin_amdgcn_readfirstlane(ldsb + (uint32_t)slot * (SLOT * 2) + 16384u + (uint32_t)wave * 256u);
            const float* src = wave == 0 ? lse : dl;
            asm volatile("s_mov_b32 m0, %0\n\ts_nop 0\n\tglobal_load_lds_dword %1, %2" ::"s"(d2), "v"(voff), "s"(src) : "memory");
        }
    };
    issue(0, 0);
    if (nt > 1) issue(1, 1);
    if (nt > 2) issue(2, 2);

    const int kidx = kbase + k32;
    const int kc = kidx < a.Tld ? kidx : a.Tld - 1;
    u32x4 kn[4], vn[4];
    {
        const bf16_t* pk = pbase + (size_t)kc * ld + a.D + hi * 8;
        const bf16_t* pv = pbase + (size_t)kc * ld + 2 * a.D + hi * 8;
#pragma unroll
        for (int ks = 0; ks < 4; ++ks) {
            kn[ks] = ld16v(pk + ks * 16); vn[ks] = ld16v(pv + ks * 16);
#pragma unroll
            for (int j = 0; j < 4; ++j) { kn[ks][j] ^= 0x80008000u; vn[ks][j] ^= 0x80008000u; }
        }
    }
    f32x16_t dkn[2], dv[2];
#pragma unroll
    for (int r = 0; r < 16; ++r) { dkn[0][r] = dkn[1][r] = dv[0][r] = dv[1][r] = 0.f; }
    u32x4 qr[4], dr[4];
    f32x16_t sx, dx;
    auto seeds = [&](const bf16_t* st, int blk) __attribute__((always_inline)) {
        const float* Ls = reinterpret_cast<const float*>(st + 8192);
#pragma unroll
        for (int j = 0; j < 4; ++j) {
            const f32x4 lv = *reinterpret_cast<const f32x4*>(Ls + 32 * blk + 8 * j + 4 * hi);
            const f32x4 ev = *reinterpret_cast<const f32x4*>(Ls + 64 + 32 * blk + 8 * j + 4 * hi);
#pragma unroll
            for (int i = 0; i < 4; ++i) { sx[4 * j + i] = lv[i]; dx[4 * j + i] = ev[i]; }
        }
    };
    auto rows = [&](const bf16_t* st, int blk) __attribute__((always_inline)) {
#pragma unroll
        for (int ks = 0; ks < 4; ++ks) { qr[ks] = lds16(st + fr.rowa[ks] + blk * 2048); dr[ks] = lds16(st + 4096 + fr.rowa[ks] + blk * 2048); }
    };
    pp_wait_dma<0>();
    asm volatile("" : "+v"(kn[0]), "+v"(kn[1]), "+v"(kn[2]), "+v"(kn[3]), "+v"(vn[0]), "+v"(vn[1]), "+v"(vn[2]), "+v"(vn[3]));
    pp_barrier();
    if (active) { rows(bx_smem, 0); seeds(bx_smem, 0); }
    int slot = 0;
    auto body = [&](auto TAILC, int t) __attribute__((always_inline)) {
        constexpr bool TAIL = decltype(TAILC)::value;
        const int s1 = (slot + 1) & 3, s3 = (slot + 3) & 3;
        if (!TAIL || t + 2 < nt) { if (wave < 2) pp_wait_dma<2 * (8 / NW) + 1>(); else pp_wait_dma<2 * (8 / NW)>(); } else pp_wait_dma<0>();
        asm volatile("s_waitcnt lgkmcnt(0)" ::: "memory");
        pp_barrier();
        if (!TAIL || t + 3 < nt) issue(t + 3, s3);
        if (active) {
            const bf16_t* st = bx_smem + slot * SLOT;
            const bf16_t* sn = bx_smem + s1 * SLOT;
#pragma unroll
            for (int blk = 0; blk < 2; ++blk) {
                if (TAIL && 2 * t + blk >= nblk) break;
                u32x4 dot[2][2], qt[2][2], pb[2], gb[2];
                float p[16], g[16];
#pragma unroll
                for (int ks = 0; ks < 4; ++ks) {
                    sx = mfma32(qr[ks], kn[ks], sx);
                    BX_SB;
                    {
                        if (ks < 2) { dot[ks][0] = bx_tr(st + 4096, fr, 0, blk * 2048 + ks * 1024); dot[ks][1] = bx_tr(st + 4096, fr, 1, blk * 2048 + ks * 1024); }
                        else { qt[ks - 2][0] = bx_tr(st, fr, 0, blk * 2048 + (ks - 2) * 1024); qt[ks - 2][1] = bx_tr(st, fr, 1, blk * 2048 + (ks - 2) * 1024); }
                    }
                    BX_SB;
                }
#pragma unroll
                for (int ks = 0; ks < 4; ++ks) {
                    dx = mfma32(dr[ks], vn[ks], dx);
                    BX_SB;
                    {
#pragma unroll
                        for (int r = 4 * ks; r < 4 * ks + 4; ++r) p[r] = __builtin_amdgcn_exp2f(-sx[r]);
                        if (ks & 1) {
                            const float* pp = &p[(ks >> 1) * 8];
                            pb[ks >> 1] = u32x4{pack2bf(pp[0], pp[1]), pack2bf(pp[2], pp[3]), pack2bf(pp[4], pp[5]), pack2bf(pp[6], pp[7])};
                            pp_opaque(pb[ks >> 1]);
                        } else asm volatile("" : "+v"(p[4 * ks]), "+v"(p[4 * ks + 3]));
                    }
                    BX_SB;
                }
#pragma unroll
                for (int i4 = 0; i4 < 4; ++i4) {
                    const int kk = i4 >> 1, db = i4 & 1;
                    dv[db] = mfma32(dot[kk][db], pb[kk], dv[db]);
                    BX_SB;
                    {
#pragma unroll
                        for (int r = 4 * i4; r < 4 * i4 + 4; ++r) g[r] = p[r] * dx[r];
                        if (i4 & 1) {
                            const float* pp = &g[(i4 >> 1) * 8];
                            gb[i4 >> 1] = u32x4{pack2bf(pp[0], pp[1]), pack2bf(pp[2], pp[3]), pack2bf(pp[4], pp[5]), pack2bf(pp[6], pp[7])};
                            pp_opaque(gb[i4 >> 1]);
                        } else asm volatile("" : "+v"(g[4 * i4]), "+v"(g[4 * i4 + 3]));
                    }
                    BX_SB;
                }
                const bf16_t* nx_st = blk == 0 ? st : sn;
                const int nx_blk = blk ^ 1;
#pragma unroll
                for (int i4 = 0; i4 < 4; ++i4) {
                    const int kk = i4 >> 1, db = i4 & 1;
                    dkn[db] = mfma32(qt[kk][db], gb[kk], dkn[db]);
                    BX_SB;
                    {
                        const float* Ls = reinterpret_cast<const float*>(nx_st + 8192);
                        qr[i4] = lds16(nx_st + fr.rowa[i4] + nx_blk * 2048);
                        dr[i4] = lds16(nx_st + 4096 + fr.rowa[i4] + nx_blk * 2048);
                        const f32x4 lv = *reinterpret_cast<const f32x4*>(Ls + 32 * nx_blk + 8 * i4 + 4 * hi);
                        const f32x4 ev = *reinterpret_cast<const f32x4*>(Ls + 64 + 32 * nx_blk + 8 * i4 + 4 * hi);
#pragma unroll
                        for (int i = 0; i < 4; ++i) { sx[4 * i4 + i] = lv[i]; dx[4 * i4 + i] = ev[i]; }
                    }
                    BX_SB;
                }
            }
        }
        slot = s1;
    };
    {
        std::false_type MAIN; std::true_type TAILT;
        int t = 0;
        for (; t + 4 < nt; ++t) body(MAIN, t);
        for (; t < nt; ++t) body(TAILT, t);
    }
    if (!active || kidx >= a.Tld) return;
    const float sk = kidx < a.T ? -a.scale : 0.f, sv = kidx < a.T ? 1.0f : 0.f;
    bf16_t* pk = a.dqkv + ((size_t)b * a.Tld + kidx) * ld + a.D + h * 64 + hi * 4;
    bf16_t* pv = a.dqkv + ((size_t)b * a.Tld + kidx) * ld + 2 * a.D + h * 64 + hi * 4;
#pragma unroll
    for (int db = 0; db < 2; ++db)
#pragma unroll
        for (int j = 0; j < 4; ++j) {
            *reinterpret_cast<uint2*>(pk + db * 32 + j * 8) = uint2{pack2bf(dkn[db][4 * j] * sk, dkn[db][4 * j + 1] * sk), pack2bf(dkn[db][4 * j + 2] * sk, dkn[db][4 * j + 3] * sk)};
            *reinterpret_cast<uint2*>(pv + db * 32 + j * 8) = uint2{pack2bf(dv[db][4 * j] * sv, dv[db][4 * j + 1] * sv), pack2bf(dv[db][4 * j + 2] * sv, dv[db][4 * j + 3] * sv)};
        }
}
#undef BX_SB

template <int NW>
__global__ __launch_bounds__(64 * NW) void attn_bwd_x32_kernel(AttnArgs a, int nx) {
    extern __shared__ __attribute__((aligned(16))) bf16_t bx_smem[];
    const int n = nx * a.H * a.B;
    const int lid = xcd_remap(blockIdx.x, 2 * n);
    const int pair = lid >> 1;
    const int xb = pair % nx, bh = pair / nx;
    const int h = bh % a.H, b = bh / a.H;
    if (lid & 1) attn_bwd_kv_x32_body<NW>(a, xb, h, b, bx_smem);
    else attn_bwd_q_x32_body<NW, true>(a, xb, h, b, bx_smem);
}
template <int NW>
__global__ __launch_bounds__(64 * NW) void attn_bwd_q_x32_kernel(AttnArgs a, int nx) {
    extern __shared__ __attribute__((aligned(16))) bf16_t bx_smem[];
    int xb, h, b;
    attn_block_coords(nx, a.H, a.B, xb, h, b);
    attn_bwd_q_x32_body<NW, true>(a, xb, h, b, bx_smem);
}
template <int NW>
__global__ __launch_bounds__(64 * NW) void attn_bwd_kv_x32_kernel(AttnArgs a, int nx) {
    extern __shared__ __attribute__((aligned(16))) bf16_t bx_smem[];
    int xb, h, b;
    attn_block_coords(nx, a.H, a.B, xb, h, b);
    attn_bwd_kv_x32_body<NW>(a, xb, h, b, bx_smem);
}
```

splice_amd/csrc/attn_x32.h:

```cpp
#pragma once
#include <type_traits>

template <int NW>
struct X32 {
    static constexpr int PIECES = 8 / NW;
    static constexpr int NL = 2 * PIECES;
    static constexpr int LDS_BYTES = 6 * 8192;
};

__device__ __forceinline__ void pp_dma16(uint32_t lds_byte, uint32_t voff, const void* sbase) {
    asm volatile("s_mov_b32 m0, %0\n\ts_nop 0\n\tglobal_load_lds_dwordx4 %1, %2" ::"s"(lds_byte), "v"(voff), "s"(sbase) : "memory");
}
template <int N>
__device__ __forceinline__ void pp_wait_dma() { asm volatile("s_waitcnt vmcnt(%0)" ::"n"(N) : "memory"); }
__device__ __forceinline__ void pp_barrier() {
    __builtin_amdgcn_sched_barrier(0);
    __builtin_amdgcn_s_barrier();
    __builtin_amdgcn_sched_barrier(0);
}
template <class V> __device__ __forceinline__ void pp_opaque(V& v) { asm volatile("" : "+v"(v)); }

typedef __attribute__((ext_vector_type(16))) float f32x16_t;
__device__ __forceinline__ f32x16_t mfma32(const u32x4& a, const u32x4& b, const f32x16_t& c) {
    return __builtin_amdgcn_mfma_f32_32x32x16_bf16(__builtin_bit_cast(bf16x8, a), __builtin_bit_cast(bf16x8, b), c, 0, 0, 0);
}
__device__ __forceinline__ float half2_max(float v) { return fmaxf(v, __shfl_xor(v, 32, 64)); }

__device__ __forceinline__ void x32_exact_rows(const AttnArgs& a, const bf16_t* pbase, int b, int h, int qidx, int hi, float c2) {
    const int ld = 3 * a.D;
    const int qc = qidx < a.Tld ? qidx : a.Tld - 1;
    float q[64], o[64];
    {
        const bf16_t* p = pbase + (size_t)qc * ld;
#pragma unroll
        for (int i = 0; i < 8; ++i) {
            const u32x4 v = ld16v(p + i * 8);
#pragma unroll
            for (int j = 0; j < 4; ++j) { q[i * 8 + 2 * j] = __uint_as_float(v[j] << 16) * c2; q[i * 8 + 2 * j + 1] = __uint_as_float(v[j] & 0xFFFF0000u) * c2; }
        }
    }
#pragma unroll
    for (int d = 0; d < 64; ++d) o[d] = 0.f;
    float m = NEG_BIG, l = 0.f;
    for (int key = hi; key < a.T; key += 2) {
        const bf16_t* kp = pbase + (size_t)key * ld + a.D;
        float sc = 0.f;
#pragma unroll
        for (int i = 0; i < 8; ++i) {
            const u32x4 v = ld16v(kp + i * 8);
#pragma unroll
            for (int j = 0; j < 4; ++j) {
                sc = __builtin_fmaf(q[i * 8 + 2 * j], __uint_as_float(v[j] << 16), sc);
                sc = __builtin_fmaf(q[i * 8 + 2 * j + 1], __uint_as_float(v[j] & 0xFFFF0000u), sc);
            }
        }
        const float mn = fmaxf(m, sc);
        const float alpha = __builtin_amdgcn_exp2f(m - mn), pk = __builtin_amdgcn_exp2f(sc - mn);
        m = mn;
        l = l * alpha + pk;
        const bf16_t* vp = pbase + (size_t)key * ld + 2 * a.D;
#pragma unroll
        for (int i = 0; i < 8; ++i) {
            const u32x4 v = ld16v(vp + i * 8);
#pragma unroll
            for (int j = 0; j < 4; ++j) {
                o[i * 8 + 2 * j] = __builtin_fmaf(pk, __uint_as_float(v[j] << 16), o[i * 8 + 2 * j] * alpha);
                o[i * 8 + 2 * j + 1] = __builtin_fmaf(pk, __uint_as_float(v[j] & 0xFFFF0000u), o[i * 8 + 2 * j + 1] * alpha);
            }
        }
    }
    const float m1 = __shfl_xor(m, 32, 64), l1 = __shfl_xor(l, 32, 64);
    const float mn = fmaxf(m, m1);
    const float a0 = __builtin_amdgcn_exp2f(m - mn), a1 = __builtin_amdgcn_exp2f(m1 - mn);
    const float lt = l * a0 + l1 * a1, inv = 1.0f / lt;
    bf16_t* op = a.out + ((size_t)b * a.Tld + qc) * a.D + h * 64;
#pragma unroll
    for (int d = 0; d < 64; ++d) {
        const float od = (o[d] * a0 + __shfl_xor(o[d], 32, 64) * a1) * inv;
        if (hi == (d >> 5) && qidx < a.Tld) op[d] = f2bf(od);
    }
    if (hi == 0 && qidx < a.Tld) a.lse[((size_t)b * a.H + h) * a.Tld + qidx] = mn + __builtin_amdgcn_logf(lt);
}

template <int NW, bool FOLD>
__global__ __launch_bounds__(64 * NW) void attn_fwd_x32_kernel(AttnArgs a, int nx) {
    extern __shared__ __attribute__((aligned(16))) bf16_t x32_smem[];
    constexpr int PIECES = X32<NW>::PIECES, NL = X32<NW>::NL;
    const int lane = threadIdx.x & 63;
    const int q32 = lane & 31, hi = lane >> 5;
    const int wave = __builtin_amdgcn_readfirstlane(threadIdx.x >> 6);
    int xb, h, b;
    attn_block_coords(nx, a.H, a.B, xb, h, b);
    const int ld = 3 * a.D;
    const int qbase = xb * (32 * NW) + wave * 32;
    const bool active = qbase < a.Tld;
    const bf16_t* pbase = a.qkv + (size_t)b * a.Tld * ld + h * 64;
    const int nt = (a.T + 63) / 64;

    const int lr = lane >> 3, pos = lane & 7;
    const int kchunk = pos ^ (((wave & 1) << 2) | (lr >> 1));
    const int vchunk = pos ^ (((lr >> 1) & 1) << 2);
    uint32_t koffs[PIECES], voffs[PIECES];
#pragma unroll
    for (int i = 0; i < PIECES; ++i) {
        const int row = (wave + NW * i) * 8 + lr;
        koffs[i] = (uint32_t)((row * ld + kchunk * 8 + a.D) * 2);
        voffs[i] = (uint32_t)((row * ld + vchunk * 8 + 2 * a.D) * 2);
    }
    const uint32_t lds0 = (uint32_t)(size_t)(__attribute__((address_space(3))) bf16_t*)x32_smem + (uint32_t)wave * 1024u;
    auto issue_tile = [&](const uint32_t (&offs)[PIECES], int chunk, int coldelta, int tile, uint32_t dst) __attribute__((always_inline)) {
        const int kt = tile * 64;
        if (kt + 64 <= a.Tld) {
            const bf16_t* tb = pbase + (size_t)kt * ld;
#pragma unroll
            for (int i = 0; i < PIECES; ++i) pp_dma16(dst + i * (NW * 1024), offs[i], tb);
        } else {
#pragma unroll
            for (int i = 0; i < PIECES; ++i) {
                int t = kt + (wave + NW * i) * 8 + lr;
                t = t < a.Tld ? t : a.Tld - 1;
                pp_dma16(dst + i * (NW * 1024), (uint32_t)((t * ld + chunk * 8 + coldelta) * 2), pbase);
            }
        }
    };
    auto issue_k = [&](int tile, int slot) __attribute__((always_inline)) { issue_tile(koffs, kchunk, a.D, tile, __builtin_amdgcn_readfirstlane(lds0 + (uint32_t)slot * 8192u)); };
    auto issue_v = [&](int tile, int slot) __attribute__((always_inline)) { issue_tile(voffs, vchunk, 2 * a.D, tile, __builtin_amdgcn_readfirstlane(lds0 + 3 * 8192u + (uint32_t)slot * 8192u)); };
    const char* kptr = reinterpret_cast<const char*>(pbase) + (size_t)4 * 64 * ld * 2;
    const char* vptr = reinterpret_cast<const char*>(pbase) + (size_t)2 * 64 * ld * 2;
    const size_t tile_bytes = (size_t)64 * ld * 2;
    auto issue_fast = [&](int s1, int s2) __attribute__((always_inline)) {
        const uint32_t kd = __builtin_amdgcn_readfirstlane(lds0 + (uint32_t)s1 * 8192u), vd = __builtin_amdgcn_readfirstlane(lds0 + 3 * 8192u + (uint32_t)s2 * 8192u);
#pragma unroll
        for (int i = 0; i < PIECES; ++i) pp_dma16(kd + i * (NW * 1024), koffs[i], kptr);
#pragma unroll
        for (int i = 0; i < PIECES; ++i) pp_dma16(vd + i * (NW * 1024), voffs[i], vptr);
    };
    issue_k(0, 0);
    issue_v(0, 0);
    if (nt > 1) { issue_k(1, 1); issue_v(1, 1); }
    if (nt > 2) issue_k(2, 2);

    u32x4 qf[4];
    const int qidx = qbase + q32;
    {
        const int qc = qidx < a.Tld ? qidx : a.Tld - 1;
        const bf16_t* p = pbase + (size_t)qc * ld + hi * 8;
#pragma unroll
        for (int ks = 0; ks < 4; ++ks) qf[ks] = ld16v(p + ks * 16);
    }
    int ka[4];
#pragma unroll
    for (int ks = 0; ks < 4; ++ks) ka[ks] = q32 * 64 + (((2 * ks + hi) ^ ((q32 >> 1) & 7)) << 3);
    int va[2];
    {
        const int m = lane & 15, dg = (lane >> 4) & 1;
#pragma unroll
        for (int db = 0; db < 2; ++db)
            va[db] = (4 * hi + (m >> 2)) * 64 + (((4 * db + 2 * dg + ((m >> 1) & 1)) ^ (((m >> 3) & 1) << 2)) << 3) + (m & 1) * 4;
    }
    float m_ref = 0.f, l = 0.f;
    f32x16_t o[2], sb[2][2], negm;
#pragma unroll
    for (int r = 0; r < 16; ++r) { o[0][r] = 0.f; o[1][r] = 0.f; sb[0][0][r] = sb[0][1][r] = sb[1][0][r] = sb[1][1][r] = 0.f; negm[r] = 0.f; }
    const float c2 = a.scale * LOG2E;
    const f32x16_t zero16 = {0.f, 0.f, 0.f, 0.f, 0.f, 0.f, 0.f, 0.f, 0.f, 0.f, 0.f, 0.f, 0.f, 0.f, 0.f, 0.f};
    u32x4 kf[2][4];
    auto read_k = [&](const bf16_t* Ks) __attribute__((always_inline)) {
#pragma unroll
        for (int kb = 0; kb < 2; ++kb)
#pragma unroll
            for (int ks = 0; ks < 4; ++ks) kf[kb][ks] = lds16(Ks + ka[ks] + kb * 2048);
    };
    auto scores = [&](f32x16_t (&s)[2], const f32x16_t& seed) __attribute__((always_inline)) {
#pragma unroll
        for (int kb = 0; kb < 2; ++kb) s[kb] = mfma32(kf[kb][0], qf[0], seed);
#pragma unroll
        for (int ks = 1; ks < 4; ++ks)
#pragma unroll
            for (int kb = 0; kb < 2; ++kb) s[kb] = mfma32(kf[kb][ks], qf[ks], s[kb]);
    };
    const bf16_t* Kring = x32_smem;
    const bf16_t* Vring = x32_smem + 3 * 4096;

    pp_wait_dma<0>();
    asm volatile("" : "+v"(qf[0]), "+v"(qf[1]), "+v"(qf[2]), "+v"(qf[3]));
    pp_barrier();
    if (active) {
        read_k(Kring);
        scores(sb[0], zero16);
        float mx = NEG_BIG;
#pragma unroll
        for (int kb = 0; kb < 2; ++kb)
#pragma unroll
            for (int r = 0; r < 16; ++r) {
                const bool valid = 32 * kb + 8 * (r >> 2) + 4 * hi + (r & 3) < a.T;
                mx = fmaxf(mx, valid ? sb[0][kb][r] : NEG_BIG);
            }
        m_ref = half2_max(mx) * (FOLD ? 1.0f : c2);
#pragma unroll
        for (int r = 0; r < 16; ++r) negm[r] = -m_ref;
        if (FOLD) scores(sb[0], negm);
        if (nt > 1) read_k(Kring + 4096);
    }
    asm volatile("s_waitcnt lgkmcnt(0)" ::: "memory");
    pp_barrier();
    if (nt > 3) issue_k(3, 0);

    int slot = 0;
#define X32_SB __builtin_amdgcn_sched_barrier(0)
    auto body = [&](auto PARC, auto TAILC, int t) __attribute__((always_inline)) {
        constexpr int PAR = decltype(PARC)::value;
        constexpr bool TAIL = decltype(TAILC)::value;
        f32x16_t (&s)[2] = sb[PAR];
        f32x16_t (&sn)[2] = sb[PAR ^ 1];
        const int s1 = slot == 2 ? 0 : slot + 1, s2 = slot == 0 ? 2 : slot - 1;
        if (!TAIL || t + 3 < nt) pp_wait_dma<NL>(); else pp_wait_dma<0>();
        asm volatile("s_waitcnt lgkmcnt(0)" ::: "memory");
        pp_barrier();
        if (!TAIL) issue_fast(s1, s2);
        else {
            if (t + 4 < nt) issue_k(t + 4, s1);
            if (t + 2 < nt) issue_v(t + 2, s2);
        }
        kptr += tile_bytes;
        vptr += tile_bytes;
        if (active) {
            const bf16_t* Vs = Vring + slot * 4096;
            const bf16_t* Kn = Kring + s2 * 4096;
            u32x4 vf[4][2], pb[4];
            float p[2][16];
            float pa[4] = {0.f, 0.f, 0.f, 0.f};
            const int kt = t * 64;
            if (TAIL && kt + 64 > a.T) {
#pragma unroll
                for (int kb = 0; kb < 2; ++kb)
#pragma unroll
                    for (int r = 0; r < 16; ++r) s[kb][r] = kt + 32 * kb + 8 * (r >> 2) + 4 * hi + (r & 3) < a.T ? s[kb][r] : NEG_BIG;
            }
            auto ex = [&](int kb, int r0, int n) __attribute__((always_inline)) {
#pragma unroll
                for (int r = r0; r < r0 + n; ++r) {
                    p[kb][r] = FOLD ? __builtin_amdgcn_exp2f(s[kb][r]) : __builtin_amdgcn_exp2f(__builtin_fmaf(s[kb][r], c2, -m_ref));
                    pa[r & 3] += p[kb][r];
                }
                asm volatile("" : "+v"(pa[0]), "+v"(pa[1]), "+v"(pa[2]), "+v"(pa[3]));
            };
            auto cv = [&](int kk) __attribute__((always_inline)) {
                const float* pp = &p[kk >> 1][(kk & 1) * 8];
                pb[kk] = u32x4{pack2bf(pp[0], pp[1]), pack2bf(pp[2], pp[3]), pack2bf(pp[4], pp[5]), pack2bf(pp[6], pp[7])};
                pp_opaque(pb[kk]);
            };
            auto rv = [&](int kk, int db) __attribute__((always_inline)) {
                typedef __attribute__((address_space(3))) tr_v4s lds_v4s;
                const tr_v4s lo = __builtin_amdgcn_ds_read_tr16_b64_v4i16((lds_v4s*)(Vs + va[db] + kk * 1024));
                const tr_v4s hh = __builtin_amdgcn_ds_read_tr16_b64_v4i16((lds_v4s*)(Vs + va[db] + kk * 1024 + 512));
                const uint2 x = __builtin_bit_cast(uint2, lo), y = __builtin_bit_cast(uint2, hh);
                vf[kk][db] = u32x4{x.x, x.y, y.x, y.y};
            };
            auto rk = [&](int kb, int ks) __attribute__((always_inline)) {
                kf[kb][ks] = lds16(Kn + ka[ks] + kb * 2048);
            };
            auto qk = [&](int kb, int ks) __attribute__((always_inline)) {
                if (ks == 0 && FOLD) asm volatile("v_mfma_f32_32x32x16_bf16 %0, %1, %2, %3" : "=&v"(sn[kb]) : "v"(kf[kb][0]), "v"(qf[0]), "v"(negm));
                else sn[kb] = mfma32(kf[kb][ks], qf[ks], ks == 0 ? zero16 : sn[kb]);
            };
            auto pv = [&](int kk, int db) __attribute__((always_inline)) {
                o[db] = mfma32(vf[kk][db], pb[kk], o[db]);
            };
            X32_SB;
            qk(0, 0); X32_SB; ex(0, 0, 3); rv(0, 0); X32_SB;
            qk(1, 0); X32_SB; ex(0, 3, 3); rv(0, 1); X32_SB;
            qk(0, 1); X32_SB; ex(0, 6, 2); cv(0); rv(1, 0); X32_SB;
            qk(1, 1); X32_SB; ex(0, 8, 3); rv(1, 1); X32_SB;
            qk(0, 2); X32_SB; ex(0, 11, 3); rv(2, 0); X32_SB;
            qk(1, 2); X32_SB; ex(0, 14, 2); cv(1); rv(2, 1); X32_SB;
            qk(0, 3); X32_SB; ex(1, 0, 3); rv(3, 0); X32_SB;
            qk(1, 3); X32_SB; ex(1, 3, 3); rv(3, 1); X32_SB;
            pv(0, 0); X32_SB; ex(1, 6, 2); cv(2); rk(0, 0); X32_SB;
            pv(0, 1); X32_SB; ex(1, 8, 3); rk(1, 0); X32_SB;
            pv(1, 0); X32_SB; ex(1, 11, 3); rk(0, 1); X32_SB;
            pv(1, 1); X32_SB; ex(1, 14, 2); cv(3); rk(1, 1); X32_SB;
            pv(2, 0); X32_SB; rk(0, 2); X32_SB;
            pv(2, 1); X32_SB; rk(1, 2); X32_SB;
            pv(3, 0); X32_SB; rk(0, 3); X32_SB;
            pv(3, 1); X32_SB; rk(1, 3); X32_SB;
            const float ps = (pa[0] + pa[1]) + (pa[2] + pa[3]);
            l += ps;
            if (__builtin_expect(__any(!(ps < ATTN_RESCALE_LIMIT)), 0)) {
                const bool mine = half2_max(!(ps < ATTN_RESCALE_LIMIT) ? 1.0f : 0.0f) > 0.f;
                const float lq = l + __shfl_xor(l, 32, 64);
                const float shift = mine ? __builtin_amdgcn_logf(lq) : 0.f;
                const float alpha = __builtin_amdgcn_exp2f(-shift);
                m_ref += shift;
                l *= alpha;
#pragma unroll
                for (int r = 0; r < 16; ++r) {
                    negm[r] = -m_ref; o[0][r] *= alpha; o[1][r] *= alpha;
                    if (FOLD) { sn[0][r] -= shift; sn[1][r] -= shift; }
                }
            }
        }
        slot = s1;
    };
    {
        std::integral_constant<int, 0> P0; std::integral_constant<int, 1> P1;
        std::false_type MAIN; std::true_type TAILT;
        int t = 0;
        for (; t + 6 < nt; t += 2) {
            body(P0, MAIN, t);
            body(P1, MAIN, t + 1);
        }
        for (; t < nt; t += 2) {
            body(P0, TAILT, t);
            if (t + 1 < nt) body(P1, TAILT, t + 1);
        }
    }
#undef X32_SB
    if (!active) return;
    const float lt = l + __shfl_xor(l, 32, 64);
    if (__builtin_expect(__any(!(lt > 0.25f && lt < 1.0e37f)), 0)) {
        x32_exact_rows(a, pbase, b, h, qidx, hi, FOLD ? 1.0f : c2);
        return;
    }
    if (qidx < a.Tld) {
        const float inv = 1.0f / lt;
        bf16_t* op = a.out + ((size_t)b * a.Tld + qidx) * a.D + h * 64 + hi * 4;
#pragma unroll
        for (int db = 0; db < 2; ++db)
#pragma unroll
            for (int j = 0; j < 4; ++j)
                *reinterpret_cast<uint2*>(op + db * 32 + j * 8) =
                    uint2{pack2bf(o[db][4 * j] * inv, o[db][4 * j + 1] * inv), pack2bf(o[db][4 * j + 2] * inv, o[db][4 * j + 3] * inv)};
        if (hi == 0) a.lse[((size_t)b * a.H + h) * a.Tld + qidx] = m_ref + __builtin_amdgcn_logf(lt);
    }
}
```

splice_amd/csrc/capi.hip:

```cpp
#include <stdarg.h>
#include <stdio.h>

#include "gen_kernels.h"
#include "kernels.h"

static thread_local char g_err[512] = "";

void splice_set_error(const char* fmt, ...) {
    va_list ap;
    va_start(ap, fmt);
    vsnprintf(g_err, sizeof(g_err), fmt, ap);
    va_end(ap);
}

static int finish(int rc, const char* what) {
    if (rc != SPLICE_OK) {
        splice_set_error("%s: invalid argument", what);
        return rc;
    }
    const hipError_t e = hipGetLastError();
    if (e != hipSuccess) {
        splice_set_error("%s: HIP error %d (%s)", what, (int)e, hipGetErrorString(e));
        return SPLICE_ERR_HIP;
    }
    return SPLICE_OK;
}

#define ST(s) ((hipStream_t)(s))

extern "C" {

int splice_version(void) { return 100; }
int splice_dev_switches(void) {
#ifdef SPLICE_DEV_SWITCHES
    return 1;
#else
    return 0;
#endif
}
const char* splice_last_error(void) { return g_err; }

int splice_gemm_nt_bf16(unsigned flags, const splice_bf16* A, int lda, const splice_bf16* B, int ldb, int M, int N, int K,
                        const splice_gemm_epilogue* epi, splice_stream_t stream) {
    if (!A || !B || !epi) return finish(SPLICE_ERR_ARG, "splice_gemm_nt_bf16");
    return finish(gemm_nt_launch(flags, A, lda, B, ldb, M, N, K, *epi, ST(stream)), "splice_gemm_nt_bf16");
}

int splice_gemm_nt_fp8(unsigned flags, const uint8_t* A, int lda, const uint8_t* B, int ldb, int M, int N, int K,
                       const splice_gemm_epilogue* epi, splice_stream_t stream) {
    if (!A || !B || !epi) return finish(SPLICE_ERR_ARG, "splice_gemm_nt_fp8");
    return finish(gemm_nt_fp8_launch(flags, A, lda, B, ldb, M, N, K, *epi, ST(stream)), "splice_gemm_nt_fp8");
}
int splice_quantize_rows_fp8(const float* x, int ldx, uint8_t* q, int ldq, float* scale, int rows, int cols, splice_stream_t stream) {
    if (!x || !q || !scale) return finish(SPLICE_ERR_ARG, "splice_quantize_rows_fp8");
    return finish(quantize_rows_fp8_launch(x, ldx, q, ldq, scale, rows, cols, ST(stream)), "splice_quantize_rows_fp8");
}

int splice_gemm_splitk_slabs(int M, int ksplit) { return gemm_splitk_slabs(M, ksplit); }

int splice_gemm_force_tile(int tile) { gemm_force_tile(tile); return SPLICE_OK; }
int splice_attention_variant(int variant) { attn_set_variant(variant); return SPLICE_OK; }
int splice_attention_qfold(int on) { attn_set_qfold(on); return SPLICE_OK; }
int splice_attention_bwd_variant(int variant) { attn_set_bwd_variant(variant); return SPLICE_OK; }

int splice_layernorm_fwd(const float* x, const float* gamma, const float* beta, splice_bf16* y, float* mean, float* rstd,
                         int rows, int D, float eps, splice_stream_t stream) {
    return finish(layernorm_fwd_launch(x, gamma, beta, y, mean, rstd, rows, D, eps, ST(stream)), "splice_layernorm_fwd");
}
int splice_layernorm_bwd(const float* dy, const float* x, const float* gamma, const float* mean, const float* rstd,
                         const float* g_in, float* g_out, splice_bf16* g_out_bf, int rows, int D, splice_stream_t stream) {
    return finish(layernorm_bwd_launch(dy, x, gamma, mean, rstd, g_in, g_out, g_out_bf, rows, D, ST(stream)), "splice_layernorm_bwd");
}

int splice_attention_fwd(const splice_bf16* qkv, const splice_bf16* qkvT, int ldt, int B, int T, int Tld, int D, int H,
                         float scale, splice_bf16* out, float* lse, splice_stream_t stream) {
    AttnArgs a = {};
    a.qkv = qkv; a.qkvT = qkvT; a.ldt = ldt; a.B = B; a.T = T; a.Tld = Tld; a.D = D; a.H = H; a.scale = scale;
    a.out = out; a.lse = lse; a.qfold = attn_qfold_hook();
    return finish(attn_fwd_launch(&a, ST(stream)), "splice_attention_fwd");
}
int splice_attention_fwd_fp8(const uint8_t* qkv8, const uint8_t* qkvT8, int ldt8, int B, int T, int Tld, int D, int H, float scale,
                             splice_bf16* out, float* lse, splice_stream_t stream) {
    if (!qkv8 || !qkvT8 || !out || !lse) return finish(SPLICE_ERR_ARG, "splice_attention_fwd_fp8");
    AttnArgs a = {};
    a.qkv8 = qkv8; a.qkvT8 = qkvT8; a.ldt8 = ldt8; a.ldt = 4; a.B = B; a.T = T; a.Tld = Tld; a.D = D; a.H = H; a.scale = scale;
    a.out = out; a.lse = lse;
    return finish(attn_fwd_launch(&a, ST(stream)), "splice_attention_fwd_fp8");
}
int splice_attention_bwd(const splice_bf16* qkv, const splice_bf16* qkvT, int ldt, int B, int T, int Tld, int D, int H,
                         float scale, const splice_bf16* out, const float* lse, const splice_bf16* dout,
                         const splice_bf16* doutT, float* delta, splice_bf16* dqkv, splice_stream_t stream) {
    AttnArgs a = {};
    a.qkv = qkv; a.qkvT = qkvT; a.ldt = ldt; a.B = B; a.T = T; a.Tld = Tld; a.D = D; a.H = H; a.scale = scale;
    a.out = const_cast<splice_bf16*>(out); a.lse = const_cast<float*>(lse);
    a.dout = dout; a.doutT = doutT; a.delta = delta; a.dqkv = dqkv; a.qfold = attn_qfold_hook();
    return finish(attn_bwd_launch(&a, ST(stream)), "splice_attention_bwd");
}
int splice_attention_probs(const splice_bf16* qkv, int B, int T, int Tld, int D, int H, float scale, const float* lse,
                           float* probs, splice_stream_t stream) {
    AttnArgs a = {};
    a.qkv = qkv; a.B = B; a.T = T; a.Tld = Tld; a.D = D; a.H = H; a.scale = scale; a.lse = const_cast<float*>(lse);
    return finish(attn_probs_launch(&a, probs, ST(stream)), "splice_attention_probs");
}

int splice_augment_structure(const float* img, float* out, float* scratch, int H, int W, int flip, int n_ops, const int* order,
                             const float* factors, float blur_sigma, splice_stream_t stream) {
    return finish(augment_structure_launch(img, out, scratch, H, W, flip, n_ops, order, factors, blur_sigma, ST(stream)), "splice_augment_structure");
}

size_t splice_keys_selfsim_ws_bytes(int T, int D) { return selfsim_ws_bytes(T, D); }
int splice_keys_selfsim_fwd(const float* K, int ldk, int T, int D, float eps, float* S, void* ws, splice_stream_t stream) {
    SelfSimWs w;
    selfsim_ws_carve(ws, T, D, &w);
    return finish(selfsim_fwd_launch(K, ldk, T, D, eps, S, w, ST(stream)), "splice_keys_selfsim_fwd");
}
int splice_keys_selfsim_bwd(const float* dS, const float* S, int T, int D, float eps, float* dK, int lddk, int accumulate,
                            void* ws, splice_stream_t stream) {
    SelfSimWs w;
    selfsim_ws_carve(ws, T, D, &w);
    return finish(selfsim_bwd_launch(dS, S, T, D, eps, dK, lddk, accumulate, w, ST(stream)), "splice_keys_selfsim_bwd");
}
int splice_mse(const float* a, int lda, const float* b, int ldb, int rows, int cols, float weight, float* loss_accum,
               float* grad, int ldg, splice_stream_t stream) {
    return finish(mse_launch(a, lda, b, ldb, rows, cols, weight, loss_accum, grad, ldg, ST(stream)), "splice_mse");
}

size_t splice_selfsim_loss_pairs_ws_bytes(int T, int D, int pairs) { return selfsim_batch_ws_bytes(T, D, pairs); }
int splice_selfsim_loss_pairs(const splice_bf16* k_tgt, const splice_bf16* k_x, int ldk, size_t k_pstride, const splice_bf16* kT_x, int ldt,
                              size_t kT_pstride, int T, int D, int pairs, float lambda, const float* e_scale_tab, int fp8, float eps,
                              float* loss_part, size_t part_pstride, float* dk, int lddk, size_t dk_pstride, void* ws, splice_stream_t stream) {
    const char* who = "splice_selfsim_loss_pairs";
    if (!k_tgt || !k_x || !kT_x || !loss_part || !dk || !ws || T < 1 || pairs < 1 || D < 64 || D % 64 || ldk < D || ldk % 8 || ldt % 8 ||
        k_pstride % 8 || kT_pstride % 8 || lddk < D)
        return finish(SPLICE_ERR_ARG, who);
    const int nt = (T + 63) / 64;
    if ((fp8 && D % 128) || (size_t)(nt * (nt + 1) / 2) > part_pstride) return finish(SPLICE_ERR_ARG, who);
    SelfSimBatch b = {};
    selfsim_batch_carve(ws, T, D, pairs, &b);
    b.ldk = ldk; b.ldt = ldt; b.k_pstride = k_pstride; b.kT_pstride = kT_pstride;
    b.k_tgt = k_tgt; b.k_x = k_x; b.kT_x = kT_x;
    b.loss_part = loss_part; b.part_pstride = part_pstride;
    b.dk = dk; b.dk_pstride = dk_pstride; b.lddk = lddk;
    b.eps = eps;
    b.fp8 = fp8 != 0;
    b.loss_scale = 1.0f / ((float)T * (float)T);
    b.e_scale = 4.0f * lambda * b.loss_scale;
    b.e_scale_tab = e_scale_tab;
    const int rc = selfsim_target_launch(b, ST(stream));
    if (rc != SPLICE_OK) return finish(rc, who);
    return finish(selfsim_loss_launch(b, ST(stream)), who);
}
int splice_mse_pairs(const float* a, int lda, size_t a_ps, const float* b, int ldb, size_t b_ps, int rows, int cols, float loss_weight,
                     float grad_weight, float* part, size_t part_ps, float* grad, int ldg, size_t g_ps, int pairs, const float* grad_tab,
                     splice_stream_t stream) {
    if (!a || !b || rows < 1 || cols < 1) return finish(SPLICE_ERR_ARG, "splice_mse_pairs");
    return finish(mse_batched_launch(a, lda, a_ps, b, ldb, b_ps, rows, cols, loss_weight, grad_weight, part, part_ps, grad, ldg, g_ps, pairs,
                                     ST(stream), grad_tab),
                  "splice_mse_pairs");
}

static_assert(SPLICE_IMAGE_TERMS_CHUNK == IMAGE_TERMS_CHUNK, "the header states the value kernel's chunk");
int splice_image_terms_value(const float* x, int n_x, int xh, int xw, const float* y, const float* b, int n_y, int yh, int yw, float* lbase,
                             size_t lstride, int lp, splice_stream_t stream) {
    const char* who = "splice_image_terms_value";
    if (!lbase || lp < 1 || lstride < 8 + (size_t)8 * lp || (!x && !y) || (y && !b)) return finish(SPLICE_ERR_ARG, who);
    const int rc = image_terms_value_launch(x, n_x, xh, xw, lbase + 8 + (size_t)6 * lp, y, b, n_y, yh, yw, lbase + 8 + (size_t)7 * lp, lstride, (size_t)lp,
                                            ST(stream));
    if (rc != SPLICE_OK) return rc;
    return finish(rc, who);
}
int splice_image_terms_grad_add(const float* x, const float* b, float* d, int n_img, int h, int w, float lambda, splice_stream_t stream) {
    if (!(lambda <= 3.402823466e+38f)) return finish(SPLICE_ERR_ARG, "splice_image_terms_grad_add");
    const int rc = b ? image_pix_grad_add_launch(x, b, d, n_img, h, w, lambda, ST(stream)) : image_tv_grad_add_launch(x, d, n_img, h, w, lambda, ST(stream));
    if (rc != SPLICE_OK) return rc;
    return finish(rc, "splice_image_terms_grad_add");
}

static bool attn_cls_args_ok(const void* qkv, const void* qkvT, int ldt, int B, int T, int Tld, int D, int H, size_t lds) {
    if (!qkv || !qkvT || B < 1 || T < 1 || T > Tld || Tld % 32 || ldt % 8 || (long long)ldt < (long long)B * Tld || D < 64 || D % 64 || H != D / 64)
        return false;
    int dev = 0, lim = 0;
    if (hipGetDevice(&dev) != hipSuccess || hipDeviceGetAttribute(&lim, hipDeviceAttributeMaxSharedMemoryPerBlock, dev) != hipSuccess) return false;
    return lds <= (size_t)(lim < 65536 ? lim : 65536);
}
int splice_attn_cls_fwd(const splice_bf16* qkv, const splice_bf16* qkvT, int ldt, int B, int T, int Tld, int D, int H, float scale, splice_bf16* out,
                        float* probs, splice_stream_t stream) {
    const char* who = "splice_attn_cls_fwd";
    if (!out || !probs || !attn_cls_args_ok(qkv, qkvT, ldt, B, T, Tld, D, H, ((size_t)Tld + Tld / 2 + 256 + 8) * sizeof(float)))
        return finish(SPLICE_ERR_ARG, who);
    return finish(attn_cls_fwd_launch(qkv, qkvT, ldt, B, T, Tld, D, H, scale, out, probs, ST(stream)), who);
}
int splice_attn_cls_bwd(const splice_bf16* qkv, const splice_bf16* qkvT, int ldt, int B, int T, int Tld, int D, int H, float scale, const float* probs,
                        const float* dout_slabs, int n_slabs, size_t slab_stride, splice_bf16* dqkv, splice_stream_t stream) {
    const char* who = "splice_attn_cls_bwd";
    if (!probs || !dout_slabs || !dqkv || n_slabs < 1 || n_slabs > 16 ||
        !attn_cls_args_ok(qkv, qkvT, ldt, B, T, Tld, D, H, ((size_t)Tld + Tld / 2 + 64 + 64 + 32 + 256 + 8) * sizeof(float)))
        return finish(SPLICE_ERR_ARG, who);
    return finish(attn_cls_bwd_launch(qkv, qkvT, ldt, B, T, Tld, D, H, scale, probs, dout_slabs, n_slabs, slab_stride, dqkv, ST(stream)), who);
}
int splice_ln_rows_fwd(float* x, size_t xs, const float* gamma, const float* beta, splice_bf16* y, size_t ys, float* mean, float* rstd, size_t ss,
                       int rows, int D, float eps, const float* slabs, int n_slabs, size_t slab_stride, const float* bias, const float* resid, size_t rs,
                       splice_stream_t stream) {
    const char* who = "splice_ln_rows_fwd";
    if (!x || !gamma || !beta || !y || !mean || !rstd || (slabs && (n_slabs < 1 || !bias || !resid))) return finish(SPLICE_ERR_ARG, who);
    return finish(ln_rows_fwd_launch(x, xs, gamma, beta, y, ys, mean, rstd, ss, rows, D, eps, slabs, n_slabs, slab_stride, bias, resid, rs, ST(stream)), who);
}
int splice_ln_rows_bwd(float* dy, size_t dys, const float* x, size_t xs, const float* gamma, const float* mean, const float* rstd, size_t ss, float* g,
                       splice_bf16* g_bf, int rows, int D, int n_slabs, size_t slab_stride, splice_stream_t stream) {
    const char* who = "splice_ln_rows_bwd";
    if (!dy || !x || !gamma || !mean || !rstd || !g || !g_bf) return finish(SPLICE_ERR_ARG, who);
    return finish(ln_rows_bwd_launch(dy, dys, x, xs, gamma, mean, rstd, ss, g, g_bf, rows, D, n_slabs, slab_stride, ST(stream)), who);
}
int splice_rows_finish(int mode, const float* slabs, int n_slabs, size_t slab_stride, int rows, int N, const float* bias, const float* resid, size_t rs,
                       float* out_f32, size_t os, splice_bf16* out_bf, splice_bf16* pre_bf, const splice_bf16* aux, size_t ps, int pre_lo,
                       splice_stream_t stream) {
    const char* who = "splice_rows_finish";
    if (mode < 0 || mode > 2 || !slabs || n_slabs < 1 || rows < 1 || N < 1 || (long long)rows * N > 0x7fffffffLL) return finish(SPLICE_ERR_ARG, who);
    if ((mode == 0 && (!out_f32 || !resid)) || (mode != 0 && !out_bf) || (mode == 2 && !aux)) return finish(SPLICE_ERR_ARG, who);
    return finish(rows_finish_launch(mode, slabs, n_slabs, slab_stride, rows, N, bias, resid, rs, out_f32, os, out_bf, pre_bf, aux, ps, pre_lo, ST(stream)), who);
}

static bool gen_conv_args_ok(const splice_gen_conv_args* g, bool reflect_dgrad) {
    if (!g || !g->in || !g->w || !g->out) return false;
    if (g->N < 1 || g->Cin < 1 || g->Hi < 1 || g->Wi < 1 || g->Cout < 1 || g->Ho < 1 || g->Wo < 1 || g->pad < 0) return false;
    if (g->ks != 1 && g->ks != 3 && g->ks != 5 && g->ks != 7) return false;
    if (g->stride != 1 && g->stride != 2) return false;
    if ((g->act != 0 && g->act != 1) || (g->reflect && g->transposed && !reflect_dgrad)) return false;
    const long long HWi = (long long)g->Hi * g->Wi, HWo = (long long)g->Ho * g->Wo;
    if (HWi > 0x1fffffffLL || HWo > 0x1fffffffLL) return false;
    if (g->in_cstride < (size_t)HWi || g->out_cstride < (size_t)HWo) return false;
    if (g->N > 1 && (g->in_nstride < (size_t)g->Cin * g->in_cstride || g->out_nstride < (size_t)g->Cout * g->out_cstride)) return false;
    if ((size_t)g->Cin * g->in_cstride > 0x1fffffffULL) return false;
    if ((size_t)g->Cout * g->w_jstride + (size_t)g->Cin * g->w_cstride + (size_t)g->ks * g->ks > 0x1fffffffULL) return false;
    if ((size_t)g->Cout * g->out_cstride > 0x7fffffffULL) return false;
    if (g->w_jstride < 1 || g->w_cstride < 1) return false;
    if (g->p_group < 0 || (g->p_group > 1 && (!g->p_nstride || g->N % g->p_group))) return false;
    if (g->reflect && !reflect_dgrad && (g->pad >= g->Hi || g->pad >= g->Wi)) return false;
    if (reflect_dgrad && (g->pad >= g->Ho || g->pad >= g->Wo || g->act)) return false;
    if (g->ws && g->ws_floats < 1) return false;
    if (g->defer_reduce && !g->ws) return false;
    return true;
}
static ConvArgs gen_conv_fill(const splice_gen_conv_args* g) {
    ConvArgs a = {};
    a.in = g->in; a.w = g->w; a.bias = g->bias; a.out = g->out;
    a.in_nstride = g->in_nstride; a.in_cstride = g->in_cstride; a.out_nstride = g->out_nstride; a.out_cstride = g->out_cstride;
    a.w_jstride = g->w_jstride; a.w_cstride = g->w_cstride; a.p_nstride = g->p_nstride;
    a.N = g->N; a.Cin = g->Cin; a.Hi = g->Hi; a.Wi = g->Wi; a.Cout = g->Cout; a.Ho = g->Ho; a.Wo = g->Wo;
    a.ks = g->ks; a.stride = g->stride; a.pad = g->pad;
    a.reflect = g->reflect; a.act = g->act; a.transposed = g->transposed; a.accumulate = g->accumulate;
    a.ws = g->ws; a.ws_floats = g->ws_floats; a.p_group = g->p_group; a.defer_reduce = g->defer_reduce;
    return a;
}
int splice_gen_conv(const splice_gen_conv_args* args, int* form_out, splice_stream_t stream) {
    const char* who = "splice_gen_conv";
    if (!gen_conv_args_ok(args, false)) return finish(SPLICE_ERR_ARG, who);
    const ConvArgs a = gen_conv_fill(args);
    if (form_out) conv_form_report(a, form_out);
    return finish(conv_launch(a, ST(stream)), who);
}
int splice_gen_conv_pair(const splice_gen_conv_args* a_args, const splice_gen_conv_args* b_args, int* forms_out, splice_stream_t stream) {
    const char* who = "splice_gen_conv_pair";
    if (!gen_conv_args_ok(a_args, false) || !gen_conv_args_ok(b_args, false)) return finish(SPLICE_ERR_ARG, who);
    const ConvArgs a = gen_conv_fill(a_args), b = gen_conv_fill(b_args);
    if (forms_out) { conv_form_report(a, forms_out); conv_form_report(b, forms_out + SPLICE_GEN_CONV_FORM_INTS); }
    return finish(conv_pair_launch(a, b, ST(stream)), who);
}
int splice_gen_conv_reflect_dgrad(const splice_gen_conv_args* args, float* pad_scratch, size_t scratch_floats, splice_stream_t stream) {
    const char* who = "splice_gen_conv_reflect_dgrad";
    if (!gen_conv_args_ok(args, true) || !pad_scratch) return finish(SPLICE_ERR_ARG, who);
    const size_t Hp = (size_t)args->Ho + 2 * args->pad, Wp = (size_t)args->Wo + 2 * args->pad;
    if (scratch_floats < (size_t)args->N * args->Cout * Hp * Wp || (size_t)args->Cout * Hp * Wp > 0x7fffffffULL) return finish(SPLICE_ERR_ARG, who);
    return finish(conv_reflect_dgrad_launch(gen_conv_fill(args), pad_scratch, ST(stream)), who);
}

static bool gen_wgrad_args_ok(const splice_gen_wgrad_args* g) {
    if (!g || !g->x || !g->dy) return false;
    if (g->N < 1 || g->Cin < 1 || g->Hi < 1 || g->Wi < 1 || g->Cout < 1 || g->Ho < 1 || g->Wo < 1 || g->pad < 0 || g->pad > 255) return false;
    if (g->ks != 1 && g->ks != 3 && g->ks != 5 && g->ks != 7) return false;
    if ((g->stride != 1 && g->stride != 2) || g->Cout > 128) return false;
    if (g->Hi > 65535 || g->Wi > 65535 || g->Ho > 65535 || g->Wo > 65535 || g->Cin > 65535) return false;
    const long long HWi = (long long)g->Hi * g->Wi, HWo = (long long)g->Ho * g->Wo;
    if (HWo > (1LL << 22)) return false;
    if (g->x_cstride < (size_t)HWi || g->dy_cstride < (size_t)HWo) return false;
    if (g->N > 1 && (g->x_nstride < (size_t)g->Cin * g->x_cstride || g->dy_nstride < (size_t)g->Cout * g->dy_cstride)) return false;
    if ((size_t)g->Cin * g->x_cstride > 0x1fffffffULL || (size_t)g->Cout * g->dy_cstride > 0x1fffffffULL) return false;
    if (g->x_nstride > 0xffffffffULL || g->dy_nstride > 0xffffffffULL) return false;
    if (g->reflect && (g->pad >= g->Hi || g->pad >= g->Wi)) return false;
    return true;
}
size_t splice_gen_conv_wgrad_ws_floats(int N, int Cin, int Cout, int ks, int Ho, int Wo) {
    if (N < 1 || Cin < 1 || Cout < 1 || ks < 1 || Ho < 1 || Wo < 1) return 0;
    int ppc = 0, cpi = 0;
    return (size_t)wgrad_chunks(N, Ho, Wo, &ppc, &cpi) * Cout * Cin * ks * ks;
}
int splice_gen_conv_wgrad(const splice_gen_wgrad_args* args, float* dw, int accumulate, int n_img, size_t p_nstride, int* form_out, splice_stream_t stream) {
    const char* who = "splice_gen_conv_wgrad";
    if (!gen_wgrad_args_ok(args) || !dw || !args->ws) return finish(SPLICE_ERR_ARG, who);
    const size_t n = (size_t)args->Cout * args->Cin * args->ks * args->ks;
    if (n > 0x7fffffffULL || args->ws_floats < splice_gen_conv_wgrad_ws_floats(args->N, args->Cin, args->Cout, args->ks, args->Ho, args->Wo))
        return finish(SPLICE_ERR_ARG, who);
    if (p_nstride ? (n_img != args->N || p_nstride < n) : n_img != 1) return finish(SPLICE_ERR_ARG, who);
    WgradArgs a = {};
    a.x = args->x; a.dy = args->dy; a.ws = args->ws;
    a.x_nstride = args->x_nstride; a.x_cstride = args->x_cstride; a.dy_nstride = args->dy_nstride; a.dy_cstride = args->dy_cstride;
    a.N = args->N; a.Cin = args->Cin; a.Hi = args->Hi; a.Wi = args->Wi; a.Cout = args->Cout; a.Ho = args->Ho; a.Wo = args->Wo;
    a.ks = args->ks; a.stride = args->stride; a.pad = args->pad; a.reflect = args->reflect;
    WgradBatchPair pair = {};
    int chunks = 0;
    int rc = conv_wgrad_add(&pair, a, &chunks);
    if (rc != SPLICE_OK) return finish(rc, who);
    WgradReduceAll r = {};
    r.count = 1; r.n[0] = (int)n; r.chunks[0] = chunks; r.ws_off[0] = 0; r.dw_off[0] = 0;
    if (form_out) {
        const WgradBatch& b = pair.tile.count ? pair.tile : pair.big.count ? pair.big : pair.small;
        form_out[0] = pair.tile.count ? 2 : pair.big.count ? 1 : 0;
        form_out[1] = b.d[0].variant;
        form_out[2] = b.d[0].pix_per_chunk;
        form_out[3] = chunks;
        form_out[4] = !((reinterpret_cast<size_t>(args->ws) | reinterpret_cast<size_t>(dw)) & 15) && p_nstride % 4 == 0 && n % 4 == 0;
        form_out[5] = b.total_wgs;
    }
    rc = conv_wgrad_batched_launch(pair, ST(stream));
    if (rc != SPLICE_OK) return finish(rc, who);
    return finish(wgrad_reduce_all_launch(r, args->ws, dw, accumulate, ST(stream), n_img, p_nstride), who);
}

int splice_gen_wgrad_reduce(const float* partials, int n, int chunks, float* dw, int accumulate, int n_img, size_t p_nstride, splice_stream_t stream) {
    const char* who = "splice_gen_wgrad_reduce";
    if (!partials || !dw || n < 1 || chunks < 0 || n_img < 1 || n_img > 65535 || (long long)n * (chunks > 0 ? chunks : 1) > 0x7fffffffLL) return finish(SPLICE_ERR_ARG, who);
    if (p_nstride ? (chunks % n_img || p_nstride < (size_t)n) : n_img != 1) return finish(SPLICE_ERR_ARG, who);
    WgradReduceAll r = {};
    r.count = 1; r.n[0] = n; r.chunks[0] = chunks; r.ws_off[0] = 0; r.dw_off[0] = 0;
    return finish(wgrad_reduce_all_launch(r, partials, dw, accumulate, ST(stream), n_img, p_nstride), who);
}

int splice_gen_bn_small_instance(int mask) { return finish(bn_small_force_instance(mask), "splice_gen_bn_small_instance"); }
int splice_gen_bn_form(int HW, int N, size_t p_nstride, int batch, int* out) {
    if (HW < 1 || N < 1 || batch < 0 || !out) return finish(SPLICE_ERR_ARG, "splice_gen_bn_form");
    const BnForm f = bn_form(HW, N, p_nstride, batch);
    out[0] = (int)f.kind; out[1] = f.hosts_pre; out[2] = f.fwd_takes_slabs; out[3] = f.bwd_takes_slabs;
    out[4] = f.fwd_fuses_upsample; out[5] = f.bwd_fuses_upsample; out[6] = f.sign_from_y;
    return SPLICE_OK;
}
size_t splice_gen_bn_part_floats(int N, int C) { return N < 1 || C < 1 ? 0 : (size_t)bn_part_floats(N, C); }
static bool gen_bn_fill(const splice_gen_bn_args* g, bool bwd, BnArgs* a, BnUpsample* up, BnPre* pre, BnSlabs* sl) {
    if (!g || !g->y || !g->out || !g->gamma || !g->mean || !g->rstd) return false;
    if (g->N < 1 || g->C < 1 || g->HW < 1 || g->N > 65535 || g->C > 65535 || g->batch < 0 || g->batch > 8) return false;
    if (g->batch && (g->N % g->batch || (g->N != g->batch && !g->p_nstride))) return false;
    if (g->N > 1 && (g->y_nstride < (size_t)g->C * g->HW || g->out_nstride < (size_t)g->C * g->HW)) return false;
    const BnForm f = bn_form(g->HW, g->N, g->p_nstride, g->batch);
    const bool two_stage = f.kind == BnForm::TWO_STAGE || f.kind == BnForm::TWO_STAGE_VEC;
    if (two_stage && (!g->part || g->part_floats < (size_t)bn_part_floats(g->N, g->C))) return false;
    if (!bwd && !g->beta) return false;
    if (bwd && ((f.sign_from_y && !g->beta) || !g->da || !g->dy || !g->dgamma || !g->dbeta)) return false;
    if (bwd && g->N > 1 && (g->da_nstride < (size_t)g->C * g->HW || g->dy_nstride < (size_t)g->C * g->HW)) return false;
    a->y = g->y; a->y_nstride = g->y_nstride; a->out = g->out; a->out_nstride = g->out_nstride;
    a->N = g->N; a->C = g->C; a->HW = g->HW; a->gamma = g->gamma; a->beta = g->beta; a->eps = g->eps; a->slope = g->slope;
    a->p_nstride = g->p_nstride; a->batch = g->batch; a->part = g->part; a->mean = g->mean; a->rstd = g->rstd;
    if (g->up_src || g->up_d_src) {
        if (bwd ? !g->up_d_src : !g->up_src) return false;
        if (g->up_c0 < 0 || g->up_c0 >= g->C || g->up_h < 1 || g->up_w < 1 || g->up_Ho < 1 || g->up_Wo < 1) return false;
        if (g->up_Ho > 2 * g->up_h || g->up_Wo > 2 * g->up_w || (long long)g->up_Ho * g->up_Wo != g->HW) return false;
        const size_t src = (size_t)(g->C - g->up_c0) * g->up_h * g->up_w;
        if (g->N > 1 && (bwd ? g->up_d_src_ns : g->up_src_ns) < src) return false;
        up->src = g->up_src; up->src_ns = g->up_src_ns; up->d_src = g->up_d_src; up->d_src_ns = g->up_d_src_ns;
// ... 88 lines not shown
```

splice_amd/csrc/common.h:

```cpp
#pragma once
#include <hip/hip_runtime.h>
#include <hip/hip_ext.h>
#include <stdint.h>
#include "splice_hip.h"

typedef uint16_t bf16_t;

void splice_set_error(const char* fmt, ...);
#define RC(x)                                                                                     \
    do {                                                                                          \
        int rc_ = (x);                                                                            \
        if (rc_ != SPLICE_OK) {                                                                   \
            splice_set_error("%s:%d %s failed (%d)", __FILE__, __LINE__, #x, rc_);                \
            return rc_;                                                                           \
        }                                                                                         \
    } while (0)
#define HIPCHK(x)                                                                                 \
    do {                                                                                          \
        hipError_t e_ = (x);                                                                      \
        if (e_ != hipSuccess) {                                                                   \
            splice_set_error("%s:%d %s -> %s", __FILE__, __LINE__, #x, hipGetErrorString(e_));    \
            return SPLICE_ERR_HIP;                                                                \
        }                                                                                         \
    } while (0)

bool splice_prof_take(hipEvent_t* start, hipEvent_t* stop, const char* kernel_name);
void splice_prof_note(double flops, double bytes);
extern int g_splice_prof_open;
struct SpliceProfScope {
    bool on;
    explicit SpliceProfScope(int which);
    ~SpliceProfScope();
};
#ifdef SPLICE_DEV_SWITCHES
extern unsigned long long g_splice_dev_skip;
extern int g_splice_dev_region, g_splice_dev_steps;
struct SpliceDevRegion {
    int prev;
    explicit SpliceDevRegion(int id) : prev(g_splice_dev_region) { g_splice_dev_region = id; }
    ~SpliceDevRegion() { g_splice_dev_region = prev; }
};
#define SPLICE_DEV_REGION(id) SpliceDevRegion splice_dev_region_##id(id)
#define SPLICE_DEV_SKIPPED() (g_splice_dev_steps > 2 && ((g_splice_dev_skip >> g_splice_dev_region) & 1ull))
#else
#define SPLICE_DEV_REGION(id) do { } while (0)
#define SPLICE_DEV_SKIPPED() false
#endif
#define SPLICE_LAUNCH(kernel, grid, block, lds, stream, ...)                                                       \
    do {                                                                                                           \
        if (SPLICE_DEV_SKIPPED()) break;                                                                           \
        hipEvent_t pa_, pb_;                                                                                       \
        if (g_splice_prof_open > 0 && splice_prof_take(&pa_, &pb_, #kernel))                                             \
            hipExtLaunchKernelGGL(kernel, grid, block, lds, stream, pa_, pb_, 0, __VA_ARGS__);                     \
        else                                                                                                       \
            hipLaunchKernelGGL(kernel, grid, block, lds, stream, __VA_ARGS__);                                     \
    } while (0)
typedef __attribute__((ext_vector_type(8))) __bf16 bf16x8;
typedef __attribute__((ext_vector_type(4))) float f32x4;
typedef __attribute__((ext_vector_type(4))) unsigned int u32x4;
typedef __attribute__((ext_vector_type(16))) float f32x16;
typedef __attribute__((ext_vector_type(2))) unsigned int u32x2;

#ifndef WT_STORES
#define WT_STORES 1
#endif
template <class V>
__device__ __forceinline__ void st_out(V* p, const V& v) {
    static_assert(sizeof(V) == 16 || sizeof(V) == 8 || sizeof(V) == 4, "4-, 8- or 16-byte values");
#if WT_STORES
    if constexpr (sizeof(V) == 16) asm volatile("global_store_dwordx4 %0, %1, off sc0 sc1" ::"v"(p), "v"(__builtin_bit_cast(u32x4, v)) : "memory");
    else if constexpr (sizeof(V) == 8) asm volatile("global_store_dwordx2 %0, %1, off sc0 sc1" ::"v"(p), "v"(__builtin_bit_cast(u32x2, v)) : "memory");
    else asm volatile("global_store_dword %0, %1, off sc0 sc1" ::"v"(p), "v"(__builtin_bit_cast(unsigned int, v)) : "memory");
#else
    *p = v;
#endif
}


typedef __bf16 bf16x2_t __attribute__((ext_vector_type(2)));
__device__ __forceinline__ bf16_t f2bf(float f) {
    const __bf16 h = (__bf16)f;
    return __builtin_bit_cast(bf16_t, h);
}
__device__ __forceinline__ float bf2f(bf16_t h) { return __uint_as_float(((uint32_t)h) << 16); }
__device__ __forceinline__ uint32_t pack2bf(float lo, float hi) {
    const bf16x2_t v = {(__bf16)lo, (__bf16)hi};
    return __builtin_bit_cast(uint32_t, v);
}

__device__ __forceinline__ float wave_sum(float v) {
#pragma unroll
    for (int o = 32; o > 0; o >>= 1) v += __shfl_xor(v, o, 64);
    return v;
}
__device__ __forceinline__ float wave_max(float v) {
#pragma unroll
    for (int o = 32; o > 0; o >>= 1) v = fmaxf(v, __shfl_xor(v, o, 64));
    return v;
}

__device__ __forceinline__ float gelu_cdf_poly(float xc) {
    const float u = xc * xc;
    float p = 7.804400182e-11f;
    p = __builtin_fmaf(p, u, -6.827484800e-09f);
    p = __builtin_fmaf(p, u, 2.666929504e-07f);
    p = __builtin_fmaf(p, u, -6.221946023e-06f);
    p = __builtin_fmaf(p, u, 9.829076589e-05f);
    p = __builtin_fmaf(p, u, -1.130963792e-03f);
    p = __builtin_fmaf(p, u, 9.869961999e-03f);
    p = __builtin_fmaf(p, u, -6.640202552e-02f);
    p = __builtin_fmaf(p, u, 3.989198506e-01f);
    return __builtin_fmaf(xc, p, 0.5f);
}
__device__ __forceinline__ float gelu_f(float x) {
    const float m = fmaxf(x, -4.0f);
    return m * gelu_cdf_poly(fminf(m, 4.0f));
}
__device__ __forceinline__ float gelu_grad_f(float x) {
    const float xc = fminf(fmaxf(x, -4.0f), 4.0f), u = xc * xc;
    float p = -5.066447262e-11f;
    p = __builtin_fmaf(p, u, 4.789254326e-09f);
    p = __builtin_fmaf(p, u, -2.026289394e-07f);
    p = __builtin_fmaf(p, u, 5.107016932e-06f);
    p = __builtin_fmaf(p, u, -8.623141184e-05f);
    p = __builtin_fmaf(p, u, 1.038558665e-03f);
    p = __builtin_fmaf(p, u, -9.190188721e-03f);
    p = __builtin_fmaf(p, u, 5.937872082e-02f);
    p = __builtin_fmaf(p, u, -2.656380534e-01f);
    p = __builtin_fmaf(p, u, 7.978171706e-01f);
    const float d = __builtin_fmaf(xc, p, 0.5f);
    return x < -4.0f ? 0.0f : (x > 4.0f ? 0.99997f : d);
}

__device__ __forceinline__ f32x4 mfma16(const uint4& a, const uint4& b, f32x4 c) {
    return __builtin_amdgcn_mfma_f32_16x16x32_bf16(__builtin_bit_cast(bf16x8, a), __builtin_bit_cast(bf16x8, b), c, 0, 0, 0);
}
__device__ __forceinline__ f32x4 mfma16(const u32x4& a, const u32x4& b, f32x4 c) {
    return __builtin_amdgcn_mfma_f32_16x16x32_bf16(__builtin_bit_cast(bf16x8, a), __builtin_bit_cast(bf16x8, b), c, 0, 0, 0);
}

__device__ __forceinline__ int xcd_remap(int bid, int nwg) {
    const int q = nwg >> 3, r = nwg & 7, xcd = bid & 7, idx = bid >> 3;
    const int base = (xcd < r) ? xcd * (q + 1) : r * (q + 1) + (xcd - r) * q;
    return base + idx;
}

__device__ __forceinline__ void grouped_tile(int t, int tiles_m, int tiles_n, int gm, int& tm, int& tn) {
    const int width = gm * tiles_n;
    const int gid = t / width, first = gid * gm;
    const int gsz = (tiles_m - first) < gm ? (tiles_m - first) : gm;
    const int r = t - gid * width;
    tm = first + r % gsz;
    tn = r / gsz;
}

static inline int cdiv(int a, int b) { return (a + b - 1) / b; }
```

splice_amd/csrc/gen_conv.hip:

```cpp
#include "gen_device.h"
#ifndef CONV_KB
#define CONV_KB 6
#endif
#include <cstdlib>

template <int KS, int FN, int CK>
struct ConvTile {
    static constexpr int T = KS * KS, KT = CK * T, BM = 64;
    static constexpr int LDA = KS == 7 ? BM + 1 : BM + 16;
    static constexpr int LDW = KT + 2;
    static constexpr int A_FLOATS = KT * LDA, W_FLOATS = 16 * FN * LDW;
};
__device__ __forceinline__ size_t conv_arena(const ConvArgs& a, int img) { return (size_t)(a.p_group > 1 ? img / a.p_group : img) * a.p_nstride; }
template <int KS, bool TRANSPOSED, int FN, int CK, int NG>
__device__ __forceinline__ void conv_igemm_body(const ConvArgs& a, int bx, int by, int bz, float* As, float* Ws) {
    constexpr int T = KS * KS;
    constexpr int KT = CK * T;
    constexpr int BM = 64;
    constexpr int LDA = ConvTile<KS, FN, CK>::LDA;
    constexpr int LDW = ConvTile<KS, FN, CK>::LDW;
    constexpr int BN = 16 * FN;
    constexpr int NTH = 256 * NG;
    constexpr int NWV = 4 * NG;
    constexpr int NA = KT / NWV;
    constexpr int NW = (BN * KT + NTH - 1) / NTH;
    constexpr int KSTEPS = KT / 4 / NG;
    static_assert(KT % (4 * NG) == 0 && ((LDW / 2) & 1) == 1, "tile shape");
    static_assert(NG == 1 || KT * LDA >= FN * 4 * 256, "accumulator exchange reuses the A tile");
    const int tid = threadIdx.x, lane = tid & 63, wave = __builtin_amdgcn_readfirstlane(tid >> 6);
    const int pw = wave & 3, grp = wave >> 2;
    const int img = bz;
    const int m0 = bx * BM;
    const int HWo = a.Ho * a.Wo;
    const float* in = a.in + (size_t)img * a.in_nstride;
    const float* wgt = a.w + conv_arena(a, img);
    const float* bias = a.bias ? a.bias + conv_arena(a, img) : nullptr;
    const int pl = tid & 63;
    const int p = m0 + pl;
    const bool pvalid = p < HWo;
    const int oy = pvalid ? p / a.Wo : 0, ox = pvalid ? p % a.Wo : 0;
    const int ksplit = a.ksplit > 1 ? a.ksplit : 1;
    const int kslice = by % ksplit;
    const int n0 = (by / ksplit) * BN;
    const int cper = ((a.Cin + ksplit - 1) / ksplit + CK - 1) / CK * CK;
    const int cbeg = kslice * cper;
    const int Kc = min(a.Cin, cbeg + cper);
    int a_off[NA], a_cl[NA];
    unsigned long long a_ok = 0;
    static_assert(NA <= 64, "gather mask");
#pragma unroll
    for (int i = 0; i < NA; ++i) {
        const int k = wave + NWV * i;
        const int cl = k / T, tap = k % T;
        const int ky = tap / KS, kx = tap % KS;
        int sy, sx;
        bool ok;
        if (!TRANSPOSED) {
            sy = oy * a.stride + ky - a.pad;
            sx = ox * a.stride + kx - a.pad;
            if (a.reflect) {
                sy = sy < 0 ? -sy : (sy >= a.Hi ? 2 * (a.Hi - 1) - sy : sy);
                sx = sx < 0 ? -sx : (sx >= a.Wi ? 2 * (a.Wi - 1) - sx : sx);
            }
            ok = sy >= 0 && sy < a.Hi && sx >= 0 && sx < a.Wi;
        } else {
            const int ty = oy + a.pad - ky, tx = ox + a.pad - kx;
            ok = ty >= 0 && tx >= 0;
            if (a.stride == 2) {
                ok = ok && !(ty & 1) && !(tx & 1);
                sy = ty >> 1; sx = tx >> 1;
            } else {
                sy = ty; sx = tx;
            }
            ok = ok && sy < a.Hi && sx < a.Wi;
        }
        ok = ok && pvalid;
        a_cl[i] = cl;
        a_off[i] = ok ? (int)(cl * a.in_cstride) + sy * a.Wi + sx : 0;
        if (ok) a_ok |= 1ull << i;
    }
    static_assert(NW <= 64, "weight mask");
    int w_off[NW], w_cl[NW], w_lds[NW];
    unsigned long long w_ok = 0;
#pragma unroll
    for (int t = 0; t < NW; ++t) {
        const int e = tid + NTH * t;
        const int j = e / KT, k = e % KT;
        const int cl = k / T, tap = k % T;
        const bool ok = e < BN * KT && (n0 + j) < a.Cout;
        w_cl[t] = cl;
        w_off[t] = ok ? (int)((size_t)(n0 + j) * a.w_jstride + (size_t)cl * a.w_cstride + tap) : 0;
        w_lds[t] = e < BN * KT ? j * LDW + k : -1;
        if (ok) w_ok |= 1ull << t;
    }
    float av[NA], wv[NW];
    const __amdgpu_buffer_rsrc_t rin = __builtin_amdgcn_make_buffer_rsrc(const_cast<float*>(in), 0, 0x7FFFFFFF, 0x00020000);
    const __amdgpu_buffer_rsrc_t rw = __builtin_amdgcn_make_buffer_rsrc(const_cast<float*>(wgt), 0, 0x7FFFFFFF, 0x00020000);
    int a_vo[NA], w_vo[NW];
#pragma unroll
    for (int i = 0; i < NA; ++i) a_vo[i] = ((a_ok >> i) & 1ull) ? a_off[i] * 4 : (int)0x80000000;
#pragma unroll
    for (int t = 0; t < NW; ++t) w_vo[t] = ((w_ok >> t) & 1ull) ? w_off[t] * 4 : (int)0x80000000;
    auto fetch = [&](int c0) {
        if (c0 + CK <= Kc) {
            const int so_a = __builtin_amdgcn_readfirstlane(c0 * (int)a.in_cstride * 4), so_w = __builtin_amdgcn_readfirstlane(c0 * (int)a.w_cstride * 4);
#pragma unroll
            for (int i = 0; i < NA; ++i) av[i] = __builtin_bit_cast(float, __builtin_amdgcn_raw_buffer_load_b32(rin, a_vo[i], so_a, 0));
#pragma unroll
            for (int t = 0; t < NW; ++t) wv[t] = __builtin_bit_cast(float, __builtin_amdgcn_raw_buffer_load_b32(rw, w_vo[t], so_w, 0));
            return;
        }
        const float* inc = in + (size_t)c0 * a.in_cstride;
        const float* wc = wgt + (size_t)c0 * a.w_cstride;
#pragma unroll
        for (int i = 0; i < NA; ++i) av[i] = a_vo[i] >= 0 && (c0 + a_cl[i] < Kc) ? inc[a_vo[i] >> 2] : 0.f;
#pragma unroll
        for (int t = 0; t < NW; ++t) wv[t] = w_vo[t] >= 0 && (c0 + w_cl[t] < Kc) ? wc[w_vo[t] >> 2] : 0.f;
    };
    f32x4 acc[FN];
#pragma unroll
    for (int j = 0; j < FN; ++j) acc[j] = f32x4{0.f, 0.f, 0.f, 0.f};
    fetch(cbeg);
    int a_wr = wave * LDA + pl;
    int a_rd = (grp * KSTEPS * 4 + (lane >> 4)) * LDA + pw * 16 + (lane & 15);
    int w_rd = (lane & 15) * LDW + grp * KSTEPS * 4 + (lane >> 4);
    for (int c0 = cbeg; c0 < Kc; c0 += CK) {
        asm volatile("" : "+v"(a_wr), "+v"(a_rd), "+v"(w_rd));
        __syncthreads();
#pragma unroll
        for (int i = 0; i < NA; ++i) As[a_wr + NWV * i * LDA] = av[i];
#pragma unroll
        for (int t = 0; t < NW; ++t)
            if (w_lds[t] >= 0) Ws[w_lds[t]] = wv[t];
        __syncthreads();
        if (c0 + CK < Kc) fetch(c0 + CK);
        constexpr int KB0 = FN == 1 ? CONV_KB : 3;
        constexpr int KB = KB0 > 0 ? (KB0 < KSTEPS ? KB0 : KSTEPS) : KSTEPS;
        float af[2][KB], bf[2][FN][KB];
        auto frag = [&](int buf, int k0) __attribute__((always_inline)) {
#pragma unroll
            for (int t = 0; t < KB; ++t) {
                if (k0 + t >= KSTEPS) break;
                af[buf][t] = As[a_rd + (k0 + t) * 4 * LDA];
#pragma unroll
                for (int j = 0; j < FN; ++j) bf[buf][j][t] = Ws[w_rd + j * 16 * LDW + (k0 + t) * 4];
            }
        };
        frag(0, 0);
#pragma unroll
        for (int k0 = 0, cur = 0; k0 < KSTEPS; k0 += KB, cur ^= 1) {
            if (k0 + KB < KSTEPS) frag(cur ^ 1, k0 + KB);
            __builtin_amdgcn_sched_barrier(0);
#pragma unroll
            for (int t = 0; t < KB; ++t) {
                if (k0 + t >= KSTEPS) break;
#pragma unroll
                for (int j = 0; j < FN; ++j) {
                    acc[j] = mfma4(af[cur][t], bf[cur][j][t], acc[j]);
                }
            }
            __builtin_amdgcn_sched_barrier(0);
        }
    }
    if (NG == 2) {
        __syncthreads();
        if (grp == 1) {
#pragma unroll
            for (int j = 0; j < FN; ++j)
#pragma unroll
                for (int r = 0; r < 4; ++r) As[(j * 4 + r) * 256 + (tid & 255)] = acc[j][r];
        }
        __syncthreads();
        if (grp == 1) return;
#pragma unroll
        for (int j = 0; j < FN; ++j)
#pragma unroll
            for (int r = 0; r < 4; ++r) acc[j][r] += As[(j * 4 + r) * 256 + tid];
    }
    if (ksplit > 1) {
        float* wsp = a.ws + (((size_t)kslice * a.N + img) * a.Cout) * HWo;
#pragma unroll
        for (int j = 0; j < FN; ++j) {
            const int n = n0 + j * 16 + (lane & 15);
            if (n >= a.Cout) continue;
#pragma unroll
            for (int r = 0; r < 4; ++r) {
                const int pp = m0 + pw * 16 + (lane >> 4) * 4 + r;
                if (pp < HWo) wsp[(size_t)n * HWo + pp] = acc[j][r];
            }
        }
        return;
    }
    float* out = a.out + (size_t)img * a.out_nstride;
    float bj[FN], prev[FN][4];
#pragma unroll
    for (int j = 0; j < FN; ++j) {
        const int nc = min(n0 + j * 16 + (lane & 15), a.Cout - 1);
        bj[j] = bias ? bias[nc] : 0.f;
        if (a.accumulate) {
#pragma unroll
            for (int r = 0; r < 4; ++r) prev[j][r] = out[(size_t)nc * a.out_cstride + min(m0 + pw * 16 + (lane >> 4) * 4 + r, HWo - 1)];
        }
    }
#pragma unroll
    for (int j = 0; j < FN; ++j) {
        const int n = n0 + j * 16 + (lane & 15);
        if (n >= a.Cout) continue;
        const float b = bj[j];
#pragma unroll
        for (int r = 0; r < 4; ++r) {
            const int pp = m0 + pw * 16 + (lane >> 4) * 4 + r;
            if (pp < HWo) {
                float v = acc[j][r] + b;
                if (a.act == 1) v = 1.0f / (1.0f + __expf(-v));
                out[(size_t)n * a.out_cstride + pp] = a.accumulate ? prev[j][r] + v : v;
            }
        }
    }
}

template <int KS, bool TRANSPOSED, int FN, int CK, int NG>
__global__ __launch_bounds__(256 * NG) void conv_igemm_kernel(ConvArgs a) {
    __shared__ float As[ConvTile<KS, FN, CK>::A_FLOATS];
    __shared__ float Ws[ConvTile<KS, FN, CK>::W_FLOATS];
    conv_igemm_body<KS, TRANSPOSED, FN, CK, NG>(a, blockIdx.x, blockIdx.y, blockIdx.z, As, Ws);
}
template <int KSA, bool TRA, int FNA, int CKA, int NGA, int KSB, bool TRB, int FNB, int CKB, int NGB>
__global__ __launch_bounds__(256 * (NGA > NGB ? NGA : NGB)) void conv_pair_kernel(ConvArgs a, ConvArgs b, int na, int gxa, int gxb) {
    using TA = ConvTile<KSA, FNA, CKA>;
    using TB = ConvTile<KSB, FNB, CKB>;
    constexpr int AF = TA::A_FLOATS > TB::A_FLOATS ? TA::A_FLOATS : TB::A_FLOATS;
    constexpr int WF = TA::W_FLOATS > TB::W_FLOATS ? TA::W_FLOATS : TB::W_FLOATS;
    __shared__ float As[AF];
    __shared__ float Ws[WF];
    const int bid = blockIdx.x;
    if (bid < na) {
        if (NGA < NGB && threadIdx.x >= 256 * NGA) return;
        conv_igemm_body<KSA, TRA, FNA, CKA, NGA>(a, bid % gxa, bid / gxa, blockIdx.z, As, Ws);
    } else {
        if (NGB < NGA && threadIdx.x >= 256 * NGB) return;
        conv_igemm_body<KSB, TRB, FNB, CKB, NGB>(b, (bid - na) % gxb, (bid - na) / gxb, blockIdx.z, As, Ws);
    }
}

__global__ void conv_splitk_reduce_kernel(ConvArgs a, int ksplit) {
    const int HWo = a.Ho * a.Wo;
    const size_t per = (size_t)a.N * a.Cout * HWo;
    for (size_t i = (size_t)blockIdx.x * 256 + threadIdx.x; i < per; i += (size_t)gridDim.x * 256) {
        const int pp = i % HWo;
        const int n = (i / HWo) % a.Cout;
        const int img = i / ((size_t)HWo * a.Cout);
        float v = a.bias ? a.bias[conv_arena(a, img) + n] : 0.f;
        float* q = a.out + (size_t)img * a.out_nstride + (size_t)n * a.out_cstride + pp;
        const float prev = a.accumulate ? *q : 0.f;
        int k = 0;
        for (; k + 3 < ksplit; k += 4) {
            const float t0 = a.ws[(size_t)k * per + i], t1 = a.ws[(size_t)(k + 1) * per + i], t2 = a.ws[(size_t)(k + 2) * per + i],
                        t3 = a.ws[(size_t)(k + 3) * per + i];
            v += t0; v += t1; v += t2; v += t3;
        }
        for (; k < ksplit; ++k) v += a.ws[(size_t)k * per + i];
        if (a.act == 1) v = 1.0f / (1.0f + __expf(-v));
        *q = a.accumulate ? prev + v : v;
    }
}

struct ConvPolicy { int fn_run, ng, ksplit, mt, ny; };
static ConvPolicy conv_policy(const ConvArgs& a, int KS, int CK) {
    const int HWo = a.Ho * a.Wo;
    const int mt = cdiv(HWo, 64);
    const int fn = (KS < 5 && a.Cout > 16 && a.Cout <= 32) ? 2 : 1;
    const int nt = cdiv(a.Cout, 16 * fn);
    constexpr int batch_fn = 2;
    constexpr int batch_min = 4;
    int fn_run = (KS < 5 && fn == 1 && a.Cout >= 64 && a.N >= batch_min && (batch_fn == 2 || batch_fn == 4)) ? batch_fn : fn;
    static const int big_fn = getenv("SPLICE_CONV_BIG_FN") ? atoi(getenv("SPLICE_CONV_BIG_FN")) : 4;
    constexpr int big_mt = 512;
    if (KS < 5 && (big_fn == 2 || big_fn == 4) && mt >= big_mt && a.Cout > 16) {
        const int want = a.Cout > 32 ? big_fn : 2;
        if (want > fn_run) fn_run = want;
    }
    const int nt_run = cdiv(a.Cout, 16 * fn_run);
    const int npol = a.p_nstride ? (a.p_group > 1 ? a.p_group : 1) : a.N;
    const int wgs = mt * nt * npol;
    int ksplit = 1;
    const int ktiles = cdiv(a.Cin, CK);
    if (a.ws && wgs < 128 && ktiles >= 4 && (size_t)a.N * a.Cout * HWo * 16 <= a.ws_floats) {
        ksplit = cdiv(256, wgs);
        if (ksplit > ktiles) ksplit = ktiles;
        if (ksplit > 16) ksplit = 16;
        if (ksplit < 2) ksplit = 1;
    }
    const bool can8 = KS == 3 && CK == 8;
    const bool ng2 = can8 && (long)mt * nt * ksplit * npol <= 2048 && cdiv(a.Cin, CK) >= 2;
    ConvPolicy p;
    p.fn_run = KS >= 5 ? 1 : fn_run;
    p.ng = ng2 ? 2 : 1;
    p.ksplit = ksplit;
    p.mt = mt;
    p.ny = (KS >= 5 ? cdiv(a.Cout, 16) : nt_run) * ksplit;
    return p;
}
static void conv_splitk_reduce_launch(const ConvArgs& a, int ksplit, hipStream_t s) {
    const size_t per = (size_t)a.N * a.Cout * a.Ho * a.Wo;
    size_t g = (per + 255) / 256;
    if (g > 1024) g = 1024;
    SPLICE_LAUNCH(conv_splitk_reduce_kernel, dim3((unsigned)g), dim3(256), 0, s, a, ksplit);
}

static inline void conv_note_work(const ConvArgs& a) {
    if (g_splice_prof_open <= 0) return;
    const double outs = (double)a.N * a.Cout * a.Ho * a.Wo, red = (double)a.Cin * a.ks * a.ks;
    splice_prof_note(2.0 * outs * red, 4.0 * (outs + (double)a.N * a.Cin * a.Hi * a.Wi + (double)a.Cout * red * (a.p_nstride ? a.N / (a.p_group > 1 ? a.p_group : 1) : 1)));
}
template <int KS, bool TR, int CK>
static void conv_launch_fn(ConvArgs a, hipStream_t s, int* ksplit_out) {
    const ConvPolicy pol = conv_policy(a, KS, CK);
    conv_note_work(a);
    a.ksplit = pol.ksplit;
    const dim3 grid(pol.mt, pol.ny, a.N);
    constexpr bool CAN8 = KS == 3 && CK == 8;
    if constexpr (KS >= 5) {
        SPLICE_LAUNCH((conv_igemm_kernel<KS, TR, 1, CK, 1>), grid, dim3(256), 0, s, a);
    } else {
        if (pol.ng == 2) {
            if constexpr (CAN8) {
                if (pol.fn_run == 1) SPLICE_LAUNCH((conv_igemm_kernel<KS, TR, 1, CK, 2>), grid, dim3(512), 0, s, a);
                else if (pol.fn_run == 2) SPLICE_LAUNCH((conv_igemm_kernel<KS, TR, 2, CK, 2>), grid, dim3(512), 0, s, a);
                else SPLICE_LAUNCH((conv_igemm_kernel<KS, TR, 4, CK, 2>), grid, dim3(512), 0, s, a);
            }
        } else {
            if (pol.fn_run == 1) SPLICE_LAUNCH((conv_igemm_kernel<KS, TR, 1, CK, 1>), grid, dim3(256), 0, s, a);
            else if (pol.fn_run == 2) SPLICE_LAUNCH((conv_igemm_kernel<KS, TR, 2, CK, 1>), grid, dim3(256), 0, s, a);
            else SPLICE_LAUNCH((conv_igemm_kernel<KS, TR, 4, CK, 1>), grid, dim3(256), 0, s, a);
        }
    }
    if (ksplit_out) *ksplit_out = pol.ksplit;
    if (pol.ksplit > 1 && !a.defer_reduce) conv_splitk_reduce_launch(a, pol.ksplit, s);
}

static inline int conv_ck(const ConvArgs& a) { return a.ks == 3 ? (a.Cin >= 32 ? 8 : 4) : a.ks == 1 ? (a.Cin >= 64 ? 32 : 16) : 4; }

template <int KSA, bool TRA, int FNA, int CKA, int KSB, bool TRB, int FNB, int CKB, int NGB>
static void conv_pair_go(const ConvArgs& a, const ConvArgs& b, const ConvPolicy& pa, const ConvPolicy& pb, hipStream_t s) {
    const int na = pa.mt * pa.ny, nb = pb.mt * pb.ny;
    SPLICE_LAUNCH((conv_pair_kernel<KSA, TRA, FNA, CKA, 1, KSB, TRB, FNB, CKB, NGB>), dim3(na + nb, 1, a.N), dim3(256 * NGB), 0, s, a, b, na, pa.mt, pb.mt);
}
int conv_pair_launch(ConvArgs a, ConvArgs b, hipStream_t s, int* ksplit_a, int* ksplit_b) {
    static const int pair_on = getenv("SPLICE_CONV_PAIR") ? atoi(getenv("SPLICE_CONV_PAIR")) : 1;
    constexpr int pair_maxn = 4;
    const int cka = conv_ck(a), ckb = conv_ck(b);
    bool done = false;
    if (pair_on && a.N == b.N && a.N < pair_maxn && !a.reflect && !b.reflect && a.ks == 1 && a.stride == 1 && (b.stride == 1 || b.stride == 2) &&
        a.transposed == b.transposed && (size_t)a.Cin * a.in_cstride <= 0x7fffffffULL && (size_t)b.Cin * b.in_cstride <= 0x7fffffffULL) {
        const ConvPolicy pa = conv_policy(a, 1, cka), pb = conv_policy(b, b.ks, ckb);
        a.ksplit = pa.ksplit; b.ksplit = pb.ksplit;
#define PAIR(TR_, FNA_, CKA_, KSB_, FNB_, CKB_, NG_)                                                                                         \
    if (!done && a.transposed == (TR_ ? 1 : 0) && pa.ng == 1 && pa.fn_run == FNA_ && cka == CKA_ && b.ks == KSB_ && pb.fn_run == FNB_ && ckb == CKB_ && pb.ng == NG_) { \
        conv_pair_go<1, TR_, FNA_, CKA_, KSB_, TR_, FNB_, CKB_, NG_>(a, b, pa, pb, s);                                                       \
        done = true;                                                                                                                          \
    }
        PAIR(false, 1, 16, 3, 1, 4, 1) PAIR(false, 1, 16, 3, 2, 4, 1)
        PAIR(false, 1, 16, 3, 1, 8, 1) PAIR(false, 1, 16, 3, 2, 8, 1) PAIR(false, 1, 16, 3, 1, 8, 2) PAIR(false, 1, 16, 3, 2, 8, 2)
        PAIR(false, 1, 32, 3, 1, 8, 1) PAIR(false, 1, 32, 3, 2, 8, 1) PAIR(false, 1, 32, 3, 1, 8, 2) PAIR(false, 1, 32, 3, 2, 8, 2)
        PAIR(true, 1, 16, 1, 1, 16, 1) PAIR(true, 1, 16, 1, 2, 16, 1) PAIR(true, 2, 16, 1, 1, 16, 1) PAIR(true, 2, 16, 1, 2, 16, 1)
        PAIR(true, 1, 16, 1, 1, 32, 1) PAIR(true, 1, 16, 1, 2, 32, 1) PAIR(true, 2, 16, 1, 1, 32, 1) PAIR(true, 2, 16, 1, 2, 32, 1)
#undef PAIR
        if (done) {
            if (ksplit_a) *ksplit_a = pa.ksplit;
            if (ksplit_b) *ksplit_b = pb.ksplit;
            if (pa.ksplit > 1 && !a.defer_reduce) conv_splitk_reduce_launch(a, pa.ksplit, s);
            if (pb.ksplit > 1 && !b.defer_reduce) conv_splitk_reduce_launch(b, pb.ksplit, s);
            return SPLICE_OK;
        }
    }
    int rc = conv_launch(a, s, ksplit_a);
    if (rc != SPLICE_OK) return rc;
    return conv_launch(b, s, ksplit_b);
}

template <bool TRANSPOSED, int FN, int CK, int RW>
__global__ __launch_bounds__(256) void conv3x3_tile_kernel(ConvArgs a, int tiles_x) {
    constexpr int CT_TH = 4 * RW, CT_PH = CT_TH + 2, CT_PLANE = CT_PH * CT_PW, NF = 4 * RW;
    constexpr int KT = CK * 9, KSTEPS = KT / 4, LDW = KT + 2, BN = 16 * FN;
    constexpr int PE = CK * CT_PLANE;
    constexpr int NP = (PE + 255) / 256;
    constexpr int NW = (BN * KT + 255) / 256;
    __shared__ float Ps[PE];
    __shared__ float Ws[BN * LDW];
    const int tid = threadIdx.x, lane = tid & 63, wave = __builtin_amdgcn_readfirstlane(tid >> 6);
    const int img = blockIdx.z;
    const int x0 = (blockIdx.x % tiles_x) * CT_TW, y0 = (blockIdx.x / tiles_x) * CT_TH;
    const int n0 = blockIdx.y * BN;
    const float* in = a.in + (size_t)img * a.in_nstride;
    const float* wgt = a.w + conv_arena(a, img);
    const float* bias = a.bias ? a.bias + conv_arena(a, img) : nullptr;
    const int sy0 = TRANSPOSED ? y0 + a.pad - 2 : y0 - a.pad, sx0 = TRANSPOSED ? x0 + a.pad - 2 : x0 - a.pad;
    int p_vo[NP];
#pragma unroll
    for (int j = 0; j < NP; ++j) {
        const int e = tid + 256 * j;
        const int c = e / CT_PLANE, rem = e % CT_PLANE, r = rem / CT_PW, x = rem % CT_PW;
        int sy = sy0 + r, sx = sx0 + x;
        if (!TRANSPOSED && a.reflect) {
            sy = sy < 0 ? -sy : (sy >= a.Hi ? 2 * (a.Hi - 1) - sy : sy);
            sx = sx < 0 ? -sx : (sx >= a.Wi ? 2 * (a.Wi - 1) - sx : sx);
        }
        const bool ok = e < PE && sy >= 0 && sy < a.Hi && sx >= 0 && sx < a.Wi;
        p_vo[j] = ok ? (int)(c * a.in_cstride + (size_t)sy * a.Wi + sx) * 4 : (int)0x80000000;
    }
    int w_vo[NW], w_lds[NW];
#pragma unroll
    for (int t = 0; t < NW; ++t) {
        const int e = tid + 256 * t;
        const int j = e / KT, k = e % KT;
        const int cl = k / 9, tap = k % 9;
        const bool ok = e < BN * KT && (n0 + j) < a.Cout;
        w_vo[t] = ok ? (int)((size_t)(n0 + j) * a.w_jstride + (size_t)cl * a.w_cstride + tap) * 4 : (int)0x80000000;
        w_lds[t] = e < BN * KT ? j * LDW + k : -1;
    }
    int koff[KSTEPS];
#pragma unroll
    for (int kk = 0; kk < KSTEPS; ++kk) {
        const int k = kk * 4 + (lane >> 4);
        const int c = k / 9, tap = k % 9, ky = tap / 3, kx = tap % 3;
        koff[kk] = c * CT_PLANE + (TRANSPOSED ? 2 - ky : ky) * CT_PW + (TRANSPOSED ? 2 - kx : kx);
    }
    int a_rd = (RW * wave) * CT_PW + (lane & 15);
    int w_rd = (lane & 15) * LDW + (lane >> 4);
    const __amdgpu_buffer_rsrc_t rin = __builtin_amdgcn_make_buffer_rsrc(const_cast<float*>(in), 0, 0x7FFFFFFF, 0x00020000);
    const __amdgpu_buffer_rsrc_t rw = __builtin_amdgcn_make_buffer_rsrc(const_cast<float*>(wgt), 0, 0x7FFFFFFF, 0x00020000);
    const int Kc = a.Cin;
    float pv[NP], wv[NW];
    auto fetch = [&](int c0) __attribute__((always_inline)) {
        const int so_a = __builtin_amdgcn_readfirstlane(c0 * (int)a.in_cstride * 4), so_w = __builtin_amdgcn_readfirstlane(c0 * (int)a.w_cstride * 4);
        if (c0 + CK <= Kc) {
#pragma unroll
            for (int j = 0; j < NP; ++j) pv[j] = __builtin_bit_cast(float, __builtin_amdgcn_raw_buffer_load_b32(rin, p_vo[j], so_a, 0));
#pragma unroll
            for (int t = 0; t < NW; ++t) wv[t] = __builtin_bit_cast(float, __builtin_amdgcn_raw_buffer_load_b32(rw, w_vo[t], so_w, 0));
        } else {
#pragma unroll
            for (int j = 0; j < NP; ++j) {
                const bool cok = c0 + (tid + 256 * j) / CT_PLANE < Kc;
                pv[j] = __builtin_bit_cast(float, __builtin_amdgcn_raw_buffer_load_b32(rin, cok ? p_vo[j] : (int)0x80000000, so_a, 0));
            }
#pragma unroll
            for (int t = 0; t < NW; ++t) {
                const bool cok = c0 + ((tid + 256 * t) % KT) / 9 < Kc;
                wv[t] = __builtin_bit_cast(float, __builtin_amdgcn_raw_buffer_load_b32(rw, cok ? w_vo[t] : (int)0x80000000, so_w, 0));
            }
        }
    };
    const int fn_live = __builtin_amdgcn_readfirstlane(min(FN, (a.Cout - n0 + 15) / 16));
    f32x4 acc[NF][FN];
#pragma unroll
    for (int f = 0; f < NF; ++f)
#pragma unroll
        for (int j = 0; j < FN; ++j) acc[f][j] = f32x4{0.f, 0.f, 0.f, 0.f};
    fetch(0);
    for (int c0 = 0; c0 < Kc; c0 += CK) {
        asm volatile("" : "+v"(a_rd), "+v"(w_rd));
        __syncthreads();
#pragma unroll
        for (int j = 0; j < NP; ++j)
            if (tid + 256 * j < PE) Ps[tid + 256 * j] = pv[j];
#pragma unroll
        for (int t = 0; t < NW; ++t)
            if (w_lds[t] >= 0) Ws[w_lds[t]] = wv[t];
        __syncthreads();
        if (c0 + CK < Kc) fetch(c0 + CK);
        float af[2][NF], bf[2][FN];
        auto frag = [&](int buf, int kk) __attribute__((always_inline)) {
            const int ao = a_rd + koff[kk];
#pragma unroll
            for (int f = 0; f < NF; ++f) af[buf][f] = Ps[ao + (f >> 2) * CT_PW + (f & 3) * 16];
#pragma unroll
            for (int j = 0; j < FN; ++j) bf[buf][j] = Ws[w_rd + j * 16 * LDW + kk * 4];
        };
        frag(0, 0);
#pragma unroll
        for (int kk = 0; kk < KSTEPS; ++kk) {
            if (kk + 1 < KSTEPS) frag((kk + 1) & 1, kk + 1);
            __builtin_amdgcn_sched_barrier(0);
#pragma unroll
            for (int j = 0; j < FN; ++j) {
                if (j > 0 && j >= fn_live) continue;
#pragma unroll
                for (int f = 0; f < NF; ++f) acc[f][j] = mfma4(af[kk & 1][f], bf[kk & 1][j], acc[f][j]);
            }
            __builtin_amdgcn_sched_barrier(0);
        }
    }
    float* out = a.out + (size_t)img * a.out_nstride;
#pragma unroll
    for (int j = 0; j < FN; ++j) {
        const int n = n0 + j * 16 + (lane & 15);
        if (n >= a.Cout) continue;
        const float b = bias ? bias[n] : 0.f;
#pragma unroll
        for (int f = 0; f < NF; ++f) {
            const int row = y0 + RW * wave + (f >> 2), col = x0 + (f & 3) * 16 + (lane >> 4) * 4;
            if (row >= a.Ho || col >= a.Wo) continue;
            float* q = out + (size_t)n * a.out_cstride + (size_t)row * a.Wo + col;
            float v[4];
#pragma unroll
            for (int r = 0; r < 4; ++r) {
                v[r] = acc[f][j][r] + b;
            }
            if (a.accumulate) {
                float pr[4];
                ld_run(q, 0, a.Wo - col, pr);
#pragma unroll
                for (int r = 0; r < 4; ++r) v[r] = pr[r] + v[r];
            }
            st_run(q, 0, a.Wo - col, v);
        }
    }
}
static bool conv_tile_ok(const ConvArgs& a) {
    static const int on = getenv("SPLICE_CONV_TILE") ? atoi(getenv("SPLICE_CONV_TILE")) : 1;
    static const int min_px = getenv("SPLICE_CONV_TILE_MIN") ? atoi(getenv("SPLICE_CONV_TILE_MIN")) : 40000;
    return on && a.ks == 3 && a.stride == 1 && !a.act && a.Wo >= 64 && (long long)a.Ho * a.Wo > min_px && !(a.reflect && a.transposed) &&
           (size_t)a.Cin * a.in_cstride <= 0x1fffffffULL;
}
template <bool TR, int CK>
static void conv_tile_launch(const ConvArgs& a, hipStream_t s) {
    conv_note_work(a);
    constexpr int rw1_max = 0x7fffffff;
    const bool rw1 = (long long)a.Ho * a.Wo <= rw1_max;
    const int tiles_x = cdiv(a.Wo, CT_TW), tiles_y = cdiv(a.Ho, rw1 ? 4 : 8);
    if (rw1) {
        if (a.Cout <= 16) SPLICE_LAUNCH((conv3x3_tile_kernel<TR, 1, CK, 1>), dim3(tiles_x * tiles_y, 1, a.N), dim3(256), 0, s, a, tiles_x);
        else SPLICE_LAUNCH((conv3x3_tile_kernel<TR, 2, CK, 1>), dim3(tiles_x * tiles_y, cdiv(a.Cout, 32), a.N), dim3(256), 0, s, a, tiles_x);
        return;
    }
    if (a.Cout <= 16) SPLICE_LAUNCH((conv3x3_tile_kernel<TR, 1, CK, 2>), dim3(tiles_x * tiles_y, 1, a.N), dim3(256), 0, s, a, tiles_x);
    else SPLICE_LAUNCH((conv3x3_tile_kernel<TR, 2, CK, 2>), dim3(tiles_x * tiles_y, cdiv(a.Cout, 32), a.N), dim3(256), 0, s, a, tiles_x);
}

int conv_launch(const ConvArgs& a, hipStream_t s, int* ksplit_out) {
    if (a.ks != 1 && a.ks != 3 && a.ks != 5 && a.ks != 7) return SPLICE_ERR_ARG;
    if (a.reflect && a.transposed) return SPLICE_ERR_ARG;
    if (a.ks >= 5) {
        if (a.ks == 5) { if (a.transposed) conv_launch_fn<5, true, 4>(a, s, ksplit_out); else conv_launch_fn<5, false, 4>(a, s, ksplit_out); }
        else { if (a.transposed) conv_launch_fn<7, true, 4>(a, s, ksplit_out); else conv_launch_fn<7, false, 4>(a, s, ksplit_out); }
        return SPLICE_OK;
    }
    if (a.stride != 1 && a.stride != 2) return SPLICE_ERR_ARG;
    if ((size_t)a.Cin * a.in_cstride > 0x7fffffffULL) return SPLICE_ERR_ARG;
    if (conv_tile_ok(a)) {
        if (a.Cin >= 32) { if (a.transposed) conv_tile_launch<true, 8>(a, s); else conv_tile_launch<false, 8>(a, s); }
        else { if (a.transposed) conv_tile_launch<true, 4>(a, s); else conv_tile_launch<false, 4>(a, s); }
        if (ksplit_out) *ksplit_out = 1;
        return SPLICE_OK;
    }
    if (a.ks == 3) {
        if (a.Cin >= 32) { if (a.transposed) conv_launch_fn<3, true, 8>(a, s, ksplit_out); else conv_launch_fn<3, false, 8>(a, s, ksplit_out); }
        else { if (a.transposed) conv_launch_fn<3, true, 4>(a, s, ksplit_out); else conv_launch_fn<3, false, 4>(a, s, ksplit_out); }
    } else {
        if (a.Cin >= 64) { if (a.transposed) conv_launch_fn<1, true, 32>(a, s, ksplit_out); else conv_launch_fn<1, false, 32>(a, s, ksplit_out); }
        else { if (a.transposed) conv_launch_fn<1, true, 16>(a, s, ksplit_out); else conv_launch_fn<1, false, 16>(a, s, ksplit_out); }
    }
    return SPLICE_OK;
}

void conv_form_report(const ConvArgs& a, int* form) {
    const bool tile = a.ks == 3 && conv_tile_ok(a);
    const int CK = a.ks >= 5 ? 4 : conv_ck(a);
    const ConvPolicy pol = conv_policy(a, a.ks, CK);
    form[0] = tile ? 1 : 0;
    form[1] = CK;
    form[2] = tile ? (a.Cout <= 16 ? 1 : 2) : pol.fn_run;
    form[3] = tile ? 1 : pol.ng;
    form[4] = tile ? 1 : pol.ksplit;
}

__global__ __launch_bounds__(256) void reflect_fold_kernel(const float* __restrict__ dpad, float* __restrict__ dx, size_t dx_nstride, size_t dx_cstride,
                                                           int C, int H, int W, int p, int accumulate) {
    const int Hp = H + 2 * p, Wp = W + 2 * p;
    const int c = blockIdx.y, img = blockIdx.z;
    const float* src = dpad + ((size_t)img * C + c) * Hp * Wp;
    float* dst = dx + (size_t)img * dx_nstride + (size_t)c * dx_cstride;
    for (int i = blockIdx.x * 256 + threadIdx.x; i < H * W; i += gridDim.x * 256) {
        const int y = i / W, x = i % W;
        int ys[3], xs[3], ny = 0, nx = 0;
        ys[ny++] = y + p;
        if (y >= 1 && y <= p) ys[ny++] = p - y;
        if (y <= H - 2 && y >= H - 1 - p) ys[ny++] = p + 2 * (H - 1) - y;
        xs[nx++] = x + p;
        if (x >= 1 && x <= p) xs[nx++] = p - x;
        if (x <= W - 2 && x >= W - 1 - p) xs[nx++] = p + 2 * (W - 1) - x;
        float acc = 0.f;
        for (int a = 0; a < ny; ++a)
            for (int b = 0; b < nx; ++b) acc += src[(size_t)ys[a] * Wp + xs[b]];
        dst[i] = accumulate ? dst[i] + acc : acc;
    }
}
int conv_reflect_dgrad_launch(ConvArgs a, float* pad_scratch, hipStream_t s) {
    const int p = a.pad, Hp = a.Ho + 2 * p, Wp = a.Wo + 2 * p;
    float* out = a.out;
    const size_t out_ns = a.out_nstride, out_cs = a.out_cstride;
    const int acc = a.accumulate, H = a.Ho, W = a.Wo;
    a.out = pad_scratch; a.out_nstride = (size_t)a.Cout * Hp * Wp; a.out_cstride = (size_t)Hp * Wp;
    a.Ho = Hp; a.Wo = Wp; a.pad = 0; a.accumulate = 0; a.reflect = 0; a.transposed = 1; a.ws = nullptr;
    const int rc = conv_launch(a, s);
    if (rc != SPLICE_OK) return rc;
    int gx = cdiv(H * W, 256);
    if (gx > 64) gx = 64;
    SPLICE_LAUNCH(reflect_fold_kernel, dim3(gx, a.Cout, a.N), dim3(256), 0, s, pad_scratch, out, out_ns, out_cs, a.Cout, H, W, p, acc);
    return SPLICE_OK;
}
```

Measured before the change: 269.9.

## Stage attention outputs through LDS for coalesced stores; vectorize conv epilogue stores

Adds a runtime store-form mask that selects a new store path. In attention forward and backward, per-lane scattered 8-byte output writes become a swizzled LDS staging step followed by row-contiguous 16-byte global stores, reusing free ring slots in shared memory. Conv epilogues gain a float4 store/load path when four output pixels are in bounds. The default mask enables only the attention-backward staged path. A global s_nop is also appended after every 16-byte write-through store, which may add small overhead everywhere.

```diff
diff --git a/include/splice_hip.h b/include/splice_hip.h
--- a/include/splice_hip.h
+++ b/include/splice_hip.h
@@ -68,6 +68,7 @@
 int splice_attention_variant(int variant);
 int splice_attention_qfold(int on);
 int splice_attention_bwd_variant(int variant);
+int splice_store_form(int mask);
 
 int splice_layernorm_fwd(const float* x, const float* gamma, const float* beta, splice_bf16* y,
                          float* mean, float* rstd, int rows, int D, float eps, splice_stream_t stream);
diff --git a/splice_amd/_lib.py b/splice_amd/_lib.py
--- a/splice_amd/_lib.py
+++ b/splice_amd/_lib.py
@@ -126,6 +126,7 @@
     "splice_attention_variant": ([_i], _i),
     "splice_attention_qfold": ([_i], _i),
     "splice_attention_bwd_variant": ([_i], _i),
+    "splice_store_form": ([_i], _i),
     "splice_layernorm_fwd": ([_vp, _vp, _vp, _vp, _vp, _vp, _i, _i, _f, _vp], _i),
     "splice_layernorm_bwd": ([_vp, _vp, _vp, _vp, _vp, _vp, _vp, _vp, _i, _i, _vp], _i),
     "splice_attention_fwd": ([_vp, _vp, _i, _i, _i, _i, _i, _i, _f, _vp, _vp, _vp], _i),
diff --git a/splice_amd/csrc/attention.hip b/splice_amd/csrc/attention.hip
--- a/splice_amd/csrc/attention.hip
+++ b/splice_amd/csrc/attention.hip
@@ -646,6 +646,9 @@
 static int g_attn_qfold = 0;
 void attn_set_qfold(int on) { g_attn_qfold = on; }
 int attn_qfold_hook() { return g_attn_qfold; }
+static int g_store_form = SPLICE_STORE_ATTN_BWD;
+int store_form_mask() { return g_store_form; }
+int store_form_set(int mask) { const int prev = g_store_form; g_store_form = mask & SPLICE_STORE_ALL; return prev; }
 
 struct AttrOnce {
     bool done[64] = {};
@@ -657,12 +660,16 @@
     }
 };
 
+template <int NW, bool FOLD, bool STG>
+static void attn_fwd_x32_go2(const AttnArgs* a, hipStream_t s) {
+    static AttrOnce attr;
+    attr.set((const void*)attn_fwd_x32_kernel<NW, FOLD, STG>, X32<NW>::LDS_BYTES);
+    const int nx = cdiv(a->Tld, 32 * NW);
+    SPLICE_LAUNCH((attn_fwd_x32_kernel<NW, FOLD, STG>), dim3(nx * a->H * a->B), dim3(64 * NW), X32<NW>::LDS_BYTES, s, *a, nx);
+}
 template <int NW, bool FOLD>
 static void attn_fwd_x32_go(const AttnArgs* a, hipStream_t s) {
-    static AttrOnce attr;
-    attr.set((const void*)attn_fwd_x32_kernel<NW, FOLD>, X32<NW>::LDS_BYTES);
-    const int nx = cdiv(a->Tld, 32 * NW);
-    SPLICE_LAUNCH((attn_fwd_x32_kernel<NW, FOLD>), dim3(nx * a->H * a->B), dim3(64 * NW), X32<NW>::LDS_BYTES, s, *a, nx);
+    if (store_form_mask() & SPLICE_STORE_ATTN_FWD) attn_fwd_x32_go2<NW, FOLD, true>(a, s); else attn_fwd_x32_go2<NW, FOLD, false>(a, s);
 }
 
 int attn_fwd_launch(const AttnArgs* a, hipStream_t s) {
@@ -695,27 +702,32 @@
 static const int kAttnBwdMergeMaxX32 = 1400;
 static const int kAttnBwdMergeMax16 = 768;
 
+template <bool STG>
+static int attn_bwd_x32_go(const AttnArgs* a, hipStream_t s) {
+    static AttrOnce at_m, at_q, at_kv, at_m2;
+    at_m.set((const void*)attn_bwd_x32_kernel<4, STG>, BX_KV_LDS);
+    at_q.set((const void*)attn_bwd_q_x32_kernel<4, STG>, BX_Q_LDS);
+    at_kv.set((const void*)attn_bwd_kv_x32_kernel<4, STG>, BX_KV_LDS);
+    if (g_attn_bwd_variant == 4) {
+        at_m2.set((const void*)attn_bwd_x32_kernel<2, STG>, BX_KV_LDS);
+        const int nx2 = cdiv(a->Tld, 64), n2 = nx2 * a->H * a->B;
+        SPLICE_LAUNCH((attn_bwd_x32_kernel<2, STG>), dim3(2 * n2), dim3(128), BX_KV_LDS, s, *a, nx2);
+        return SPLICE_OK;
+    }
+    const int nx4 = cdiv(a->Tld, 128), n4 = nx4 * a->H * a->B;
+    if (g_attn_bwd_variant == 3 || (g_attn_bwd_variant != 2 && 2 * n4 > kAttnBwdMergeMaxX32)) {
+        SPLICE_LAUNCH((attn_bwd_q_x32_kernel<4, STG>), dim3(n4), dim3(256), BX_Q_LDS, s, *a, nx4);
+        SPLICE_LAUNCH((attn_bwd_kv_x32_kernel<4, STG>), dim3(n4), dim3(256), BX_KV_LDS, s, *a, nx4);
+    } else SPLICE_LAUNCH((attn_bwd_x32_kernel<4, STG>), dim3(2 * n4), dim3(256), BX_KV_LDS, s, *a, nx4);
+    return SPLICE_OK;
+}
+
 int attn_bwd_launch(const AttnArgs* a, hipStream_t s) {
     if (a->Tld % 32 || a->D % 64 || a->D / 64 != a->H) return SPLICE_ERR_ARG;
     const int nx = cdiv(a->Tld, 64);
     if (!a->delta_ready) SPLICE_LAUNCH(attn_delta_kernel, dim3(cdiv(a->B * a->Tld * a->H, 256)), dim3(256), 0, s, *a);
     if (a->qfold && g_attn_bwd_variant != 1) {
-        static AttrOnce at_m, at_q, at_kv, at_m2;
-        at_m.set((const void*)attn_bwd_x32_kernel<4>, BX_KV_LDS);
-        at_q.set((const void*)attn_bwd_q_x32_kernel<4>, BX_Q_LDS);
-        at_kv.set((const void*)attn_bwd_kv_x32_kernel<4>, BX_KV_LDS);
-        if (g_attn_bwd_variant == 4) {
-            at_m2.set((const void*)attn_bwd_x32_kernel<2>, BX_KV_LDS);
-            const int nx2 = cdiv(a->Tld, 64), n2 = nx2 * a->H * a->B;
-            SPLICE_LAUNCH((attn_bwd_x32_kernel<2>), dim3(2 * n2), dim3(128), BX_KV_LDS, s, *a, nx2);
-            return SPLICE_OK;
-        }
-        const int nx4 = cdiv(a->Tld, 128), n4 = nx4 * a->H * a->B;
-        if (g_attn_bwd_variant == 3 || (g_attn_bwd_variant != 2 && 2 * n4 > kAttnBwdMergeMaxX32)) {
-            SPLICE_LAUNCH((attn_bwd_q_x32_kernel<4>), dim3(n4), dim3(256), BX_Q_LDS, s, *a, nx4);
-            SPLICE_LAUNCH((attn_bwd_kv_x32_kernel<4>), dim3(n4), dim3(256), BX_KV_LDS, s, *a, nx4);
-        } else SPLICE_LAUNCH((attn_bwd_x32_kernel<4>), dim3(2 * n4), dim3(256), BX_KV_LDS, s, *a, nx4);
-        return SPLICE_OK;
+        return (store_form_mask() & SPLICE_STORE_ATTN_BWD) ? attn_bwd_x32_go<true>(a, s) : attn_bwd_x32_go<false>(a, s);
     }
     const int n = nx * a->H * a->B;
     if (2 * n <= kAttnBwdMergeMax16) {
diff --git a/splice_amd/csrc/attn_bwd_x32.h b/splice_amd/csrc/attn_bwd_x32.h
--- a/splice_amd/csrc/attn_bwd_x32.h
+++ b/splice_amd/csrc/attn_bwd_x32.h
@@ -63,9 +63,10 @@
     }
 };
 
-template <int NW, bool FOLD>
+template <int NW, bool FOLD, bool STG>
 __device__ __forceinline__ void attn_bwd_q_x32_body(const AttnArgs& a, int xb, int h, int b, bf16_t* bx_smem ) {
     constexpr int NL = 2 * (8 / NW);
+    static_assert(!STG || NW <= 4, "the staged tiles of all waves share one free ring slot");
     const int lane = threadIdx.x & 63, q32 = lane & 31, hi = lane >> 5;
     const int wave = __builtin_amdgcn_readfirstlane(threadIdx.x >> 6);
     const int ld = 3 * a.D;
@@ -187,6 +188,11 @@
         for (; t < nt; ++t) body(TAILT, t);
     }
     if (!active || qidx >= a.Tld) return;
+    if constexpr (STG) {
+        bf16_t* stg = bx_smem + ((nt + 1) & 3) * 8192 + wave * 2048;
+        x32_stage_store(stg, dq, a.scale, a.dqkv + ((size_t)b * a.Tld + qbase) * ld + h * 64, ld, lane);
+        return;
+    }
     bf16_t* op = a.dqkv + ((size_t)b * a.Tld + qidx) * ld + h * 64 + hi * 4;
 #pragma unroll
     for (int db = 0; db < 2; ++db)
@@ -196,10 +202,11 @@
                                                                     pack2bf(dq[db][4 * j + 2] * a.scale, dq[db][4 * j + 3] * a.scale)};
 }
 
-template <int NW>
+template <int NW, bool STG>
 __device__ __forceinline__ void attn_bwd_kv_x32_body(const AttnArgs& a, int xb, int h, int b, bf16_t* bx_smem ) {
     constexpr int SLOT = 2 * 4096 + 256;
     static_assert(NW >= 2, "waves 0 and 1 move the lse / delta rows");
+    static_assert(!STG || NW <= 4, "the staged tiles take the two free ring slots, one per wave pair");
     const int lane = threadIdx.x & 63, k32 = lane & 31, hi = lane >> 5;
     const int wave = __builtin_amdgcn_readfirstlane(threadIdx.x >> 6);
     const int ld = 3 * a.D;
@@ -353,6 +360,13 @@
     }
     if (!active || kidx >= a.Tld) return;
     const float sk = kidx < a.T ? -a.scale : 0.f, sv = kidx < a.T ? 1.0f : 0.f;
+    if constexpr (STG) {
+        bf16_t* stg = bx_smem + ((nt + 1 + (wave >> 1)) & 3) * SLOT + (wave & 1) * 4096;
+        bf16_t* row0 = a.dqkv + ((size_t)b * a.Tld + kbase) * ld + a.D + h * 64;
+        x32_stage_store(stg, dkn, sk, row0, ld, lane);
+        x32_stage_store(stg + 2048, dv, sv, row0 + a.D, ld, lane);
+        return;
+    }
     bf16_t* pk = a.dqkv + ((size_t)b * a.Tld + kidx) * ld + a.D + h * 64 + hi * 4;
     bf16_t* pv = a.dqkv + ((size_t)b * a.Tld + kidx) * ld + 2 * a.D + h * 64 + hi * 4;
 #pragma unroll
@@ -365,7 +379,7 @@
 }
 #undef BX_SB
 
-template <int NW>
+template <int NW, bool STG>
 __global__ __launch_bounds__(64 * NW) void attn_bwd_x32_kernel(AttnArgs a, int nx) {
     extern __shared__ __attribute__((aligned(16))) bf16_t bx_smem[];
     const int n = nx * a.H * a.B;
@@ -373,20 +387,20 @@
     const int pair = lid >> 1;
     const int xb = pair % nx, bh = pair / nx;
     const int h = bh % a.H, b = bh / a.H;
-    if (lid & 1) attn_bwd_kv_x32_body<NW>(a, xb, h, b, bx_smem);
-    else attn_bwd_q_x32_body<NW, true>(a, xb, h, b, bx_smem);
-}
-template <int NW>
+    if (lid & 1) attn_bwd_kv_x32_body<NW, STG>(a, xb, h, b, bx_smem);
+    else attn_bwd_q_x32_body<NW, true, STG>(a, xb, h, b, bx_smem);
+}
+template <int NW, bool STG>
 __global__ __launch_bounds__(64 * NW) void attn_bwd_q_x32_kernel(AttnArgs a, int nx) {
     extern __shared__ __attribute__((aligned(16))) bf16_t bx_smem[];
     int xb, h, b;
     attn_block_coords(nx, a.H, a.B, xb, h, b);
-    attn_bwd_q_x32_body<NW, true>(a, xb, h, b, bx_smem);
-}
-template <int NW>
+    attn_bwd_q_x32_body<NW, true, STG>(a, xb, h, b, bx_smem);
+}
+template <int NW, bool STG>
 __global__ __launch_bounds__(64 * NW) void attn_bwd_kv_x32_kernel(AttnArgs a, int nx) {
     extern __shared__ __attribute__((aligned(16))) bf16_t bx_smem[];
     int xb, h, b;
     attn_block_coords(nx, a.H, a.B, xb, h, b);
-    attn_bwd_kv_x32_body<NW>(a, xb, h, b, bx_smem);
-}
+    attn_bwd_kv_x32_body<NW, STG>(a, xb, h, b, bx_smem);
+}
diff --git a/splice_amd/csrc/attn_x32.h b/splice_amd/csrc/attn_x32.h
--- a/splice_amd/csrc/attn_x32.h
+++ b/splice_amd/csrc/attn_x32.h
@@ -82,7 +82,27 @@
     if (hi == 0 && qidx < a.Tld) a.lse[((size_t)b * a.H + h) * a.Tld + qidx] = mn + __builtin_amdgcn_logf(lt);
 }
 
-template <int NW, bool FOLD>
+__device__ __forceinline__ void x32_stage_store(bf16_t* stg, const f32x16_t (&t)[2], float s, bf16_t* row0, int ldo, int lane) {
+    const int r32 = lane & 31, hi = lane >> 5;
+#pragma unroll
+    for (int db = 0; db < 2; ++db)
+#pragma unroll
+        for (int j = 0; j < 4; ++j)
+            *reinterpret_cast<uint2*>(stg + r32 * 64 + (((db * 4 + j) ^ ((r32 >> 1) & 7)) << 3) + hi * 4) =
+                uint2{pack2bf(t[db][4 * j] * s, t[db][4 * j + 1] * s), pack2bf(t[db][4 * j + 2] * s, t[db][4 * j + 3] * s)};
+    __builtin_amdgcn_wave_barrier();
+    const int c = lane & 7;
+    u32x4 v[4];
+#pragma unroll
+    for (int i = 0; i < 4; ++i) {
+        const int r = i * 8 + (lane >> 3);
+        v[i] = *reinterpret_cast<const u32x4*>(stg + r * 64 + ((c ^ ((r >> 1) & 7)) << 3));
+    }
+#pragma unroll
+    for (int i = 0; i < 4; ++i) st_out(reinterpret_cast<u32x4*>(row0 + (size_t)(i * 8 + (lane >> 3)) * ldo + c * 8), v[i]);
+}
+
+template <int NW, bool FOLD, bool STG>
 __global__ __launch_bounds__(64 * NW) void attn_fwd_x32_kernel(AttnArgs a, int nx) {
     extern __shared__ __attribute__((aligned(16))) bf16_t x32_smem[];
     constexpr int PIECES = X32<NW>::PIECES, NL = X32<NW>::NL;
@@ -322,7 +342,13 @@
         x32_exact_rows(a, pbase, b, h, qidx, hi, FOLD ? 1.0f : c2);
         return;
     }
-    if (qidx < a.Tld) {
+    if constexpr (STG) {
+        const int pr = wave >> 1;
+        const int sl = (nt + (pr == 1 ? 1 : pr == 3 ? 2 : 0)) % 3;
+        bf16_t* stg = x32_smem + (pr < 2 ? 3 * 4096 : 0) + sl * 4096 + (wave & 1) * 2048;
+        x32_stage_store(stg, o, 1.0f / lt, a.out + ((size_t)b * a.Tld + qbase) * a.D + h * 64, a.D, lane);
+        if (hi == 0) a.lse[((size_t)b * a.H + h) * a.Tld + qidx] = m_ref + __builtin_amdgcn_logf(lt);
+    } else if (qidx < a.Tld) {
         const float inv = 1.0f / lt;
         bf16_t* op = a.out + ((size_t)b * a.Tld + qidx) * a.D + h * 64 + hi * 4;
 #pragma unroll
diff --git a/splice_amd/csrc/capi.hip b/splice_amd/csrc/capi.hip
--- a/splice_amd/csrc/capi.hip
+++ b/splice_amd/csrc/capi.hip
@@ -62,6 +62,7 @@
 int splice_attention_variant(int variant) { attn_set_variant(variant); return SPLICE_OK; }
 int splice_attention_qfold(int on) { attn_set_qfold(on); return SPLICE_OK; }
 int splice_attention_bwd_variant(int variant) { attn_set_bwd_variant(variant); return SPLICE_OK; }
+int splice_store_form(int mask) { return store_form_set(mask); }
 
 int splice_layernorm_fwd(const float* x, const float* gamma, const float* beta, splice_bf16* y, float* mean, float* rstd,
                          int rows, int D, float eps, splice_stream_t stream) {
diff --git a/splice_amd/csrc/common.h b/splice_amd/csrc/common.h
--- a/splice_amd/csrc/common.h
+++ b/splice_amd/csrc/common.h
@@ -64,11 +64,17 @@
 #ifndef WT_STORES
 #define WT_STORES 1
 #endif
+#define SPLICE_STORE_ATTN_FWD 1
+#define SPLICE_STORE_ATTN_BWD 2
+#define SPLICE_STORE_CONV 4
+#define SPLICE_STORE_ALL 7
+int store_form_mask();
+int store_form_set(int mask);
 template <class V>
 __device__ __forceinline__ void st_out(V* p, const V& v) {
     static_assert(sizeof(V) == 16 || sizeof(V) == 8 || sizeof(V) == 4, "4-, 8- or 16-byte values");
 #if WT_STORES
-    if constexpr (sizeof(V) == 16) asm volatile("global_store_dwordx4 %0, %1, off sc0 sc1" ::"v"(p), "v"(__builtin_bit_cast(u32x4, v)) : "memory");
+    if constexpr (sizeof(V) == 16) asm volatile("global_store_dwordx4 %0, %1, off sc0 sc1\n\ts_nop 1" ::"v"(p), "v"(__builtin_bit_cast(u32x4, v)) : "memory");
     else if constexpr (sizeof(V) == 8) asm volatile("global_store_dwordx2 %0, %1, off sc0 sc1" ::"v"(p), "v"(__builtin_bit_cast(u32x2, v)) : "memory");
     else asm volatile("global_store_dword %0, %1, off sc0 sc1" ::"v"(p), "v"(__builtin_bit_cast(unsigned int, v)) : "memory");
 #else
diff --git a/splice_amd/csrc/gen_conv.hip b/splice_amd/csrc/gen_conv.hip
--- a/splice_amd/csrc/gen_conv.hip
+++ b/splice_amd/csrc/gen_conv.hip
@@ -12,7 +12,7 @@
     static constexpr int A_FLOATS = KT * LDA, W_FLOATS = 16 * FN * LDW;
 };
 __device__ __forceinline__ size_t conv_arena(const ConvArgs& a, int img) { return (size_t)(a.p_group > 1 ? img / a.p_group : img) * a.p_nstride; }
-template <int KS, bool TRANSPOSED, int FN, int CK, int NG>
+template <int KS, bool TRANSPOSED, int FN, int CK, int NG, int SF>
 __device__ __forceinline__ void conv_igemm_body(const ConvArgs& a, int bx, int by, int bz, float* As, float* Ws) {
     constexpr int T = KS * KS;
     constexpr int KT = CK * T;
@@ -177,15 +177,22 @@
 #pragma unroll
             for (int r = 0; r < 4; ++r) acc[j][r] += As[(j * 4 + r) * 256 + tid];
     }
+    const int pp0 = m0 + pw * 16 + (lane >> 4) * 4;
+    const bool whole = SF != 0 && pp0 + 3 < HWo;
+    auto st4 = [&](float* q, const f32x4& v) __attribute__((always_inline)) {
+        f4u t; t.x = v[0]; t.y = v[1]; t.z = v[2]; t.w = v[3];
+        *(f4u*)q = t;
+    };
     if (ksplit > 1) {
         float* wsp = a.ws + (((size_t)kslice * a.N + img) * a.Cout) * HWo;
 #pragma unroll
         for (int j = 0; j < FN; ++j) {
             const int n = n0 + j * 16 + (lane & 15);
             if (n >= a.Cout) continue;
+            if (whole) { st4(wsp + (size_t)n * HWo + pp0, acc[j]); continue; }
 #pragma unroll
             for (int r = 0; r < 4; ++r) {
-                const int pp = m0 + pw * 16 + (lane >> 4) * 4 + r;
+                const int pp = pp0 + r;
                 if (pp < HWo) wsp[(size_t)n * HWo + pp] = acc[j][r];
             }
         }
@@ -198,8 +205,13 @@
         const int nc = min(n0 + j * 16 + (lane & 15), a.Cout - 1);
         bj[j] = bias ? bias[nc] : 0.f;
         if (a.accumulate) {
-#pragma unroll
-            for (int r = 0; r < 4; ++r) prev[j][r] = out[(size_t)nc * a.out_cstride + min(m0 + pw * 16 + (lane >> 4) * 4 + r, HWo - 1)];
+            if (whole) {
+                const f4u t = *(const f4u*)(out + (size_t)nc * a.out_cstride + pp0);
+                prev[j][0] = t.x; prev[j][1] = t.y; prev[j][2] = t.z; prev[j][3] = t.w;
+            } else {
+#pragma unroll
+                for (int r = 0; r < 4; ++r) prev[j][r] = out[(size_t)nc * a.out_cstride + min(pp0 + r, HWo - 1)];
+            }
         }
     }
 #pragma unroll
@@ -207,25 +219,27 @@
         const int n = n0 + j * 16 + (lane & 15);
         if (n >= a.Cout) continue;
         const float b = bj[j];
+        f32x4 o4;
 #pragma unroll
         for (int r = 0; r < 4; ++r) {
-            const int pp = m0 + pw * 16 + (lane >> 4) * 4 + r;
-            if (pp < HWo) {
-                float v = acc[j][r] + b;
-                if (a.act == 1) v = 1.0f / (1.0f + __expf(-v));
-                out[(size_t)n * a.out_cstride + pp] = a.accumulate ? prev[j][r] + v : v;
-            }
-        }
-    }
-}
-
-template <int KS, bool TRANSPOSED, int FN, int CK, int NG>
+            float v = acc[j][r] + b;
+            if (a.act == 1) v = 1.0f / (1.0f + __expf(-v));
+            o4[r] = a.accumulate ? prev[j][r] + v : v;
+        }
+        if (whole) { st4(out + (size_t)n * a.out_cstride + pp0, o4); continue; }
+#pragma unroll
+        for (int r = 0; r < 4; ++r)
+            if (pp0 + r < HWo) out[(size_t)n * a.out_cstride + pp0 + r] = o4[r];
+    }
+}
+
+template <int KS, bool TRANSPOSED, int FN, int CK, int NG, int SF>
 __global__ __launch_bounds__(256 * NG) void conv_igemm_kernel(ConvArgs a) {
     __shared__ float As[ConvTile<KS, FN, CK>::A_FLOATS];
     __shared__ float Ws[ConvTile<KS, FN, CK>::W_FLOATS];
-    conv_igemm_body<KS, TRANSPOSED, FN, CK, NG>(a, blockIdx.x, blockIdx.y, blockIdx.z, As, Ws);
-}
-template <int KSA, bool TRA, int FNA, int CKA, int NGA, int KSB, bool TRB, int FNB, int CKB, int NGB>
+    conv_igemm_body<KS, TRANSPOSED, FN, CK, NG, SF>(a, blockIdx.x, blockIdx.y, blockIdx.z, As, Ws);
+}
+template <int KSA, bool TRA, int FNA, int CKA, int NGA, int KSB, bool TRB, int FNB, int CKB, int NGB, int SF>
 __global__ __launch_bounds__(256 * (NGA > NGB ? NGA : NGB)) void conv_pair_kernel(ConvArgs a, ConvArgs b, int na, int gxa, int gxb) {
     using TA = ConvTile<KSA, FNA, CKA>;
     using TB = ConvTile<KSB, FNB, CKB>;
@@ -236,10 +250,10 @@
     const int bid = blockIdx.x;
     if (bid < na) {
         if (NGA < NGB && threadIdx.x >= 256 * NGA) return;
-        conv_igemm_body<KSA, TRA, FNA, CKA, NGA>(a, bid % gxa, bid / gxa, blockIdx.z, As, Ws);
+        conv_igemm_body<KSA, TRA, FNA, CKA, NGA, SF>(a, bid % gxa, bid / gxa, blockIdx.z, As, Ws);
     } else {
         if (NGB < NGA && threadIdx.x >= 256 * NGB) return;
-        conv_igemm_body<KSB, TRB, FNB, CKB, NGB>(b, (bid - na) % gxb, (bid - na) / gxb, blockIdx.z, As, Ws);
+        conv_igemm_body<KSB, TRB, FNB, CKB, NGB, SF>(b, (bid - na) % gxb, (bid - na) / gxb, blockIdx.z, As, Ws);
     }
 }
 
@@ -313,38 +327,48 @@
     const double outs = (double)a.N * a.Cout * a.Ho * a.Wo, red = (double)a.Cin * a.ks * a.ks;
     splice_prof_note(2.0 * outs * red, 4.0 * (outs + (double)a.N * a.Cin * a.Hi * a.Wi + (double)a.Cout * red * (a.p_nstride ? a.N / (a.p_group > 1 ? a.p_group : 1) : 1)));
 }
-template <int KS, bool TR, int CK>
-static void conv_launch_fn(ConvArgs a, hipStream_t s, int* ksplit_out) {
+static inline int conv_store_form() { return (store_form_mask() & SPLICE_STORE_CONV) ? 1 : 0; }
+template <int KS, bool TR, int CK, int SF>
+static void conv_launch_sf(ConvArgs a, hipStream_t s, int* ksplit_out) {
     const ConvPolicy pol = conv_policy(a, KS, CK);
     conv_note_work(a);
     a.ksplit = pol.ksplit;
     const dim3 grid(pol.mt, pol.ny, a.N);
     constexpr bool CAN8 = KS == 3 && CK == 8;
     if constexpr (KS >= 5) {
-        SPLICE_LAUNCH((conv_igemm_kernel<KS, TR, 1, CK, 1>), grid, dim3(256), 0, s, a);
+        SPLICE_LAUNCH((conv_igemm_kernel<KS, TR, 1, CK, 1, SF>), grid, dim3(256), 0, s, a);
     } else {
         if (pol.ng == 2) {
             if constexpr (CAN8) {
-                if (pol.fn_run == 1) SPLICE_LAUNCH((conv_igemm_kernel<KS, TR, 1, CK, 2>), grid, dim3(512), 0, s, a);
-                else if (pol.fn_run == 2) SPLICE_LAUNCH((conv_igemm_kernel<KS, TR, 2, CK, 2>), grid, dim3(512), 0, s, a);
-                else SPLICE_LAUNCH((conv_igemm_kernel<KS, TR, 4, CK, 2>), grid, dim3(512), 0, s, a);
+                if (pol.fn_run == 1) SPLICE_LAUNCH((conv_igemm_kernel<KS, TR, 1, CK, 2, SF>), grid, dim3(512), 0, s, a);
+                else if (pol.fn_run == 2) SPLICE_LAUNCH((conv_igemm_kernel<KS, TR, 2, CK, 2, SF>), grid, dim3(512), 0, s, a);
+                else SPLICE_LAUNCH((conv_igemm_kernel<KS, TR, 4, CK, 2, SF>), grid, dim3(512), 0, s, a);
             }
         } else {
-            if (pol.fn_run == 1) SPLICE_LAUNCH((conv_igemm_kernel<KS, TR, 1, CK, 1>), grid, dim3(256), 0, s, a);
-            else if (pol.fn_run == 2) SPLICE_LAUNCH((conv_igemm_kernel<KS, TR, 2, CK, 1>), grid, dim3(256), 0, s, a);
-            else SPLICE_LAUNCH((conv_igemm_kernel<KS, TR, 4, CK, 1>), grid, dim3(256), 0, s, a);
+            if (pol.fn_run == 1) SPLICE_LAUNCH((conv_igemm_kernel<KS, TR, 1, CK, 1, SF>), grid, dim3(256), 0, s, a);
+            else if (pol.fn_run == 2) SPLICE_LAUNCH((conv_igemm_kernel<KS, TR, 2, CK, 1, SF>), grid, dim3(256), 0, s, a);
+            else SPLICE_LAUNCH((conv_igemm_kernel<KS, TR, 4, CK, 1, SF>), grid, dim3(256), 0, s, a);
         }
     }
     if (ksplit_out) *ksplit_out = pol.ksplit;
     if (pol.ksplit > 1 && !a.defer_reduce) conv_splitk_reduce_launch(a, pol.ksplit, s);
 }
+template <int KS, bool TR, int CK>
+static void conv_launch_fn(const ConvArgs& a, hipStream_t s, int* ksplit_out) {
+    if (conv_store_form()) conv_launch_sf<KS, TR, CK, 1>(a, s, ksplit_out); else conv_launch_sf<KS, TR, CK, 0>(a, s, ksplit_out);
+}
 
 static inline int conv_ck(const ConvArgs& a) { return a.ks == 3 ? (a.Cin >= 32 ? 8 : 4) : a.ks == 1 ? (a.Cin >= 64 ? 32 : 16) : 4; }
 
+template <int KSA, bool TRA, int FNA, int CKA, int KSB, bool TRB, int FNB, int CKB, int NGB, int SF>
+static void conv_pair_go_sf(const ConvArgs& a, const ConvArgs& b, const ConvPolicy& pa, const ConvPolicy& pb, hipStream_t s) {
+    const int na = pa.mt * pa.ny, nb = pb.mt * pb.ny;
+    SPLICE_LAUNCH((conv_pair_kernel<KSA, TRA, FNA, CKA, 1, KSB, TRB, FNB, CKB, NGB, SF>), dim3(na + nb, 1, a.N), dim3(256 * NGB), 0, s, a, b, na, pa.mt, pb.mt);
+}
 template <int KSA, bool TRA, int FNA, int CKA, int KSB, bool TRB, int FNB, int CKB, int NGB>
 static void conv_pair_go(const ConvArgs& a, const ConvArgs& b, const ConvPolicy& pa, const ConvPolicy& pb, hipStream_t s) {
-    const int na = pa.mt * pa.ny, nb = pb.mt * pb.ny;
-    SPLICE_LAUNCH((conv_pair_kernel<KSA, TRA, FNA, CKA, 1, KSB, TRB, FNB, CKB, NGB>), dim3(na + nb, 1, a.N), dim3(256 * NGB), 0, s, a, b, na, pa.mt, pb.mt);
+    if (conv_store_form()) conv_pair_go_sf<KSA, TRA, FNA, CKA, KSB, TRB, FNB, CKB, NGB, 1>(a, b, pa, pb, s);
+    else conv_pair_go_sf<KSA, TRA, FNA, CKA, KSB, TRB, FNB, CKB, NGB, 0>(a, b, pa, pb, s);
 }
 int conv_pair_launch(ConvArgs a, ConvArgs b, hipStream_t s, int* ksplit_a, int* ksplit_b) {
     static const int pair_on = getenv("SPLICE_CONV_PAIR") ? atoi(getenv("SPLICE_CONV_PAIR")) : 1;
```

After: 271.9 (median of 6 runs). About the same (+0.7%).
